# szhan227/text2protein

Hardware: AMD Instinct MI355X
Metric: 6D backbone samples/sec (128-res, 1000-step) (higher is better)
Workload: dtype f16; 1 GPU; cfg2: test_config.yml L=128 N=1000 chains/GPU=32 C=5 text_tokens=512 condition=none; step = 1 PC step (2 score evals + SDE updates); sample = 1000 PC steps; finite=True

## Files before the change

include/t2p.h:

```cpp
#ifndef T2P_H_
#define T2P_H_

#include <stdint.h>

#ifdef __cplusplus
extern "C" {
#endif

#define T2P_DTYPE_F32 0
#define T2P_DTYPE_BF16 1
#define T2P_DTYPE_F16 2

#define T2P_SDE_VE 0
#define T2P_SDE_VP 1
#define T2P_SDE_SUBVP 2

typedef struct t2p_model_config {
  int32_t num_channels;
  int32_t max_res_num;
  int32_t nf;
  int32_t num_res_blocks;
  int32_t n_ch_mult;
  int32_t ch_mult[8];
  int32_t n_attn_resolutions;
// ... 6 lines not shown
  int32_t scale_by_sigma;
  int32_t compute_dtype;
} t2p_model_config;

typedef struct t2p_engine t2p_engine;
typedef struct t2p_sampler t2p_sampler;

const char* t2p_last_error(void);
int t2p_device_count(void);

int t2p_engine_create(const t2p_model_config* cfg, t2p_engine** out);
void t2p_engine_destroy(t2p_engine* e);
int t2p_engine_num_params(const t2p_engine* e);
int t2p_engine_param_info(const t2p_engine* e, int i, const char** name, int64_t shape[4], int* ndim);
int t2p_engine_load_param(t2p_engine* e, const char* name, const float* host_data, const int64_t* shape, int ndim);
int t2p_engine_finalize(t2p_engine* e);
int t2p_engine_set_context(t2p_engine* e, const float* context, int batch, int tokens, void* stream);
int t2p_engine_score(t2p_engine* e, const float* x, const int32_t* labels, float* out, int batch, void* stream);
int t2p_engine_score_ex(t2p_engine* e, const float* x, const int32_t* labels, const float* labels_f, float* out,
                        int batch, void* stream);
int64_t t2p_engine_device_bytes(const t2p_engine* e);
int t2p_engine_pool_reclaimed(const t2p_engine* e);

typedef struct t2p_sampler_config {
  int32_t sde;
  int32_t N;
  double sigma_min, sigma_max, beta_min, beta_max;
  double snr;
  int32_t n_steps_each;
  int32_t probability_flow;
  int32_t denoise;
  double eps;
  int32_t batch;
  int32_t global_batch;
  uint64_t seed;
} t2p_sampler_config;

int t2p_sampler_create(t2p_engine* e, const t2p_sampler_config* cfg, const float* g_table, const int32_t* label_table,
                       t2p_sampler** out);
void t2p_sampler_destroy(t2p_sampler* s);
int t2p_sampler_set_seed(t2p_sampler* s, uint64_t seed);
int t2p_sampler_set_vp_tables(t2p_sampler* s, const float* label_f, const float* score_scale, const float* x_coef, const float* corr_alpha);
typedef int (*t2p_allreduce_fn)(float* device_sums2, void* stream, void* user);
int t2p_sampler_set_norm_allreduce(t2p_sampler* s, float* device_sums2, t2p_allreduce_fn fn, void* user);
int t2p_sampler_set_condition(t2p_sampler* s, const uint8_t* mask, const float* x_initial);
int t2p_sampler_set_guidance(t2p_sampler* s, double w, int enabled);
int t2p_sampler_set_context(t2p_sampler* s, const float* context, int batch, int tokens, void* stream);
int t2p_sampler_reset(t2p_sampler* s, int step, void* stream);
int t2p_sampler_step(t2p_sampler* s, float* x, float* x_mean, const float* noise_corrector,
                     const float* noise_predictor, void* stream);
int t2p_sampler_step_graph(t2p_sampler* s, float* x, float* x_mean, void* stream);
int t2p_sampler_run(t2p_sampler* s, float* x, float* out, int prior_given, int n_steps, void* stream);
int t2p_sampler_count_dispatches(t2p_sampler* s, float* x, float* x_mean, void* stream, int* n_out);

typedef struct t2p_ddim_config {
  int32_t timesteps;
  int32_t sampling_steps;
  double eta;
  double w;
  int32_t clip;
  int32_t batch;
  uint64_t seed;
} t2p_ddim_config;
typedef struct t2p_ddim_step_row {
  int32_t t;
  float sqrt_recip, sqrt_recipm1, sqrt_an, c, sigma;
  int32_t last;
} t2p_ddim_step_row;
typedef struct t2p_ddim t2p_ddim;
int t2p_ddim_create(t2p_engine* e, const t2p_ddim_config* cfg, const t2p_ddim_step_row* table, t2p_ddim** out);
void t2p_ddim_destroy(t2p_ddim* d);
int t2p_ddim_set_seed(t2p_ddim* d, uint64_t seed);
int t2p_ddim_set_condition(t2p_ddim* d, const uint8_t* mask, const float* x_initial);
int t2p_ddim_set_context(t2p_ddim* d, const float* context, int batch, int tokens, void* stream);
int t2p_ddim_reset(t2p_ddim* d, int step, void* stream);
int t2p_ddim_step(t2p_ddim* d, float* x, float* x0_out, const float* noise, void* stream);
int t2p_ddim_run(t2p_ddim* d, float* x, float* out, int prior_given, int n_steps, void* stream);
int t2p_op_ddim_update(const float* x, const float* eps_c, const float* eps_u, const float* z, const uint8_t* mask,
                       const float* x_initial, float* x_out, float* x_out2, float* x0_out, int64_t n, float w, float w1,
                       float sqrt_recip, float sqrt_recipm1, float sqrt_an, float c, float sigma, int clip, int last,
                       uint64_t seed, uint64_t stream_id, void* stream);

typedef struct t2p_train_config {
  double lr, beta1, eps, weight_decay;
  double warmup;
  double grad_clip;
  double ema_rate;
  double dropout;
  double t_eps;
  int32_t cond_flags;
  uint64_t seed;
} t2p_train_config;

typedef struct t2p_train_batch {
  const float* coords_6d;
  const uint8_t* mask_pair;
  const uint8_t* mask_inpaint;
  const float* context;
  int32_t batch, tokens;
  const float* t;
  const float* z;
} t2p_train_batch;

typedef struct t2p_trainer t2p_trainer;
int t2p_train_create(const t2p_model_config* model, const t2p_train_config* train, t2p_trainer** out);
void t2p_train_destroy(t2p_trainer* t);
int t2p_train_num_params(const t2p_trainer* t);
int t2p_train_param_info(const t2p_trainer* t, int i, const char** name, int64_t shape[4], int* ndim);
int t2p_train_load_param(t2p_trainer* t, const char* name, const float* host_data, const int64_t* shape, int ndim);
int t2p_train_read(t2p_trainer* t, int which, const char* name, float* host_out);
int t2p_train_write(t2p_trainer* t, int which, const char* name, const float* host_in);
int t2p_train_set_step(t2p_trainer* t, int64_t step, int64_t adam_updates, int64_t ema_updates);
int t2p_train_get_step(const t2p_trainer* t, int64_t out3[3]);
int t2p_train_set_sde(t2p_trainer* t, int sde, double beta_min, double beta_max, const float* std_table);
int t2p_train_set_dropout_masks(t2p_trainer* t, const uint8_t* const* device_masks, int n);
int t2p_train_set_ss_blocks(t2p_trainer* t, const int32_t* host_blocks, int n, const uint8_t* host_drop, double p);
int t2p_train_set_inpaint_draw(t2p_trainer* t, const int32_t* host_len_lo_hi, int B, double random_p, double contiguous_p);
int t2p_train_loss(t2p_trainer* t, const t2p_train_batch* batch, int backward, float* loss_host, float* score_out, void* stream);
int t2p_train_step(t2p_trainer* t, const t2p_train_batch* batch, float* loss_host, void* stream);
int t2p_train_grad_buffer(t2p_trainer* t, float** device_ptr, int64_t* n);
int t2p_train_apply(t2p_trainer* t, void* stream);
int t2p_train_eval_loss(t2p_trainer* t, const t2p_train_batch* batch, float* loss_host, void* stream);
int64_t t2p_train_device_bytes(const t2p_trainer* t);
int t2p_op_tgemm(const float* A, int64_t sAm, int64_t sAk, const float* B, int64_t sBk, int64_t sBn, float* C, int64_t ldc, int M, int N,
                 int K, int nz, int64_t sAz, int64_t sBz, int64_t sCz, float alpha, float beta, const float* bias_n, int ksplit, int conv,
                 int H, int W, int conv_C, void* stream);
int t2p_op_tgemm16(int dtype, const float* A, int64_t sAm, int64_t sAk, const float* B, int64_t sBk, int64_t sBn, float* C, int64_t ldc,
                   int M, int N, int K, int nz, int64_t sAz, int64_t sBz, int64_t sCz, float alpha, float beta, const float* bias_n, int ksplit,
                   int conv, int H, int W, int conv_C, void* stream);
int t2p_op_ss_block_dropout(const float* x, float* out, int batch, int C, int L, const int32_t* host_blocks, int n,
                            const uint8_t* host_drop, double p, uint64_t seed, uint64_t stream_id, uint8_t* drop_out_device, void* stream);
int t2p_op_inpaint_mask_draw(const int32_t* host_len_lo_hi, int B, int L, double random_p, double contiguous_p, uint64_t seed, uint64_t stream_id,
                             int force_mode, uint8_t* flags_out, uint8_t* pair_out, int* mode_out_host, void* stream);
int t2p_op_groupnorm_backward(const float* x, const float* dy, const float* gamma, const float* beta, int silu, int batch, int HW, int C,
                              int groups, float eps, float* dx, float* dgamma, float* dbeta, void* stream);
int t2p_op_layernorm_backward(const float* x, const float* dy, const float* gamma, int64_t rows, int C, float eps, float* dx, float* dgamma,
                              float* dbeta, void* stream);
int t2p_op_groupnorm_backward_form(const float* x, const float* dy, const float* gamma, const float* beta, int silu, int batch, int HW,
                                   int C, int groups, float eps, float* dx, float* dgamma, float* dbeta, int fixed_order, void* stream);
int t2p_op_layernorm_backward_form(const float* x, const float* dy, const float* gamma, int64_t rows, int C, float eps, float* dx,
                                   float* dgamma, float* dbeta, int fixed_order, void* stream);
int t2p_op_colsum(const float* dy, int nz, int64_t rows_per_z, int N, int64_t ld, float* out, int64_t ld_out, int accumulate,
                  int fixed_order, void* stream);
int t2p_op_sumsq(const float* g, int64_t n, int fixed_order, double* result_host, void* stream);
int t2p_op_seed_scale(const float* x, int64_t n, float target, float* s2_host, void* stream);
int t2p_op_softmax_backward(const float* P, float* dP_inout, int64_t rows, int n, float scale, void* stream);
int t2p_op_geglu_backward(const float* u, const float* dy, float* du, int64_t rows, int inner, void* stream);

int t2p_op_gemm(int dtype, const void* A, int a_f32, const void* Bw, void* C, int c_f32, int M, int N, int K,
                int64_t lda, int64_t ldb, int64_t ldc, const float* bias_n, const float* residual, float alpha,
                void* stream);
int t2p_op_gemm_r16(int dtype, const void* A, int a_f32, const void* Bw, void* C, int c_f32, int M, int N, int K, int64_t lda,
                    int64_t ldb, int64_t ldc, const float* bias_n, const void* residual16, float alpha, void* stream);
int t2p_op_conv3x3(int dtype, const void* x, int a_f32, const void* w, const float* bias, float* out, int batch,
                   int H, int W, int Cin, int Cout, int upsample, void* stream);
int t2p_op_conv3x3_shortcut(int dtype, const void* a, const void* w, const float* bias, const void* x0, int CX0,
                            const void* x1, int CX1, float alpha, void* out, int c_f32, int batch, int H, int W, int C,
                            int Cout, void* stream);
int t2p_op_conv3x3_groupnorm(int dtype, const void* a, const void* w, const float* bias, const float* bias_bn, const void* residual,
                             float alpha, int upsample, int groups, const float* gamma, const float* beta, float eps, int silu,
                             void* out, int out_f32, void* normed, float* col_stats, int batch, int H, int W, int C, int Cout, void* stream);
int t2p_op_small_conv_groupnorm(int dtype, const void* a, const void* w, int64_t ldw, const void* x0, int CX0, const void* x1, int CX1,
                                const float* bias, const float* bias_bn, const void* residual, float alpha, void* out, int out_f32,
                                float* col_stats, void* normed, int groups, const float* gamma, const float* beta, float eps, int silu,
                                int batch, int H, int W, int C, int Cout, void* stream);
int t2p_op_st_entry(int dtype, const void* x, const float* col_stats, int groups, const float* gn_gamma, const float* gn_beta,
                    float gn_eps, const void* w_in, const float* b_in, const void* residual, const float* ln_gamma,
                    const float* ln_beta, float ln_eps, const void* w_2, int n2, const float* b_2, int geglu, void* t, void* out2,
                    const void* w_3, const float* b_3, const void* res3, void* y, float* y_stats, int batch, int n, int C,
                    void* stream);
int t2p_op_attn_proj(int dtype, const void* x, const float* col_stats, int groups, const float* gn_gamma, const float* gn_beta,
                     float gn_eps, const void* w_qk, const float* b_qk, const void* w_v, void* qk, void* vt, void* k_fm,
                     int64_t npad, int batch, int n, int C, void* stream);
int t2p_op_input_conv(const float* x, const float* w_tcn, const float* bias, void* out, int out_dtype, int batch, int C,
                      int H, int W, int nf, float* col_stats, void* stream);
int t2p_op_groupnorm(const float* x0, const float* x1, int C0, int C1, int batch, int H, int W, int groups,
                     const float* gamma, const float* beta, float eps, int silu, int down, void* out, int dtype,
                     void* stream);
int t2p_op_layernorm(const float* x, const float* gamma, const float* beta, void* out, int dtype, int64_t rows,
                     int C, float eps, void* stream);
int t2p_op_layernorm16(const void* x16, const float* gamma, const float* beta, void* out16, int dtype, int64_t rows, int C,
                       float eps, void* stream);
int t2p_op_softmax(const float* S, int64_t lds, void* P, int64_t ldp, int dtype, int64_t rows, int n, float scale,
                   void* stream);
int t2p_op_geglu(const float* u, void* out, int dtype, int64_t rows, int inner, void* stream);
int64_t t2p_op_attention_ws(int dtype, int batch, int heads, int nq, int nk);
int t2p_op_attention(int dtype, const void* q, int64_t ldq, const void* k, int64_t ldk, const void* vt,
                     int64_t ldvt, void* out, int batch, int heads, int nq, int nk, int d, float scale,
                     void* workspace, void* stream);
int t2p_op_attention_wide(int dtype, const void* q, int64_t ldq, const void* k, int64_t ldk, const void* vt, int64_t ldvt, void* out,
                          int out_f32, const float* bias, const void* residual, int residual_16bit, float alpha, float* col_stats,
                          int batch, int n, int d, float scale, void* stream);
int t2p_op_attention_wide_fm(int dtype, const void* q, int64_t ldq, const void* k_fm, const void* vt_fm, void* out, int out_f32,
                             const float* bias, const void* residual, int residual_16bit, float alpha, float* col_stats, int batch,
                             int n, int d, float scale, void* stream);
int t2p_op_gemm_frag_major(int dtype, const void* A, const void* Bw, void* C, void* c_frag, int M, int N, int K, int frag_col0,
                           int rows_per_batch, int batch, void* stream);
int t2p_op_attention_qkv(int dtype, const void* qkv, int64_t ld, void* out, int batch, int heads, int n, int d,
                         float scale, void* stream);
int t2p_op_langevin(const float* x, const float* grad, const float* noise, const uint8_t* mask,
                    const float* x_initial, float* x_out, float* x_mean_out, int batch, int64_t per_sample,
                    float snr, float alpha, float* sums_out , void* stream);
int t2p_op_langevin_norms(const float* grad, const float* noise, int batch, int64_t per_sample, float* workspace,
                          float* sums, void* stream);
int t2p_op_langevin_update(const float* x, const float* grad, const float* noise, const uint8_t* mask,
                           const float* x_initial, float* x_out, float* x_mean_out, int64_t n, const float* sums,
                           float batch_total, float snr, float alpha, void* stream);
int t2p_op_predictor(const float* x, const float* score, const float* noise, const uint8_t* mask,
                     const float* x_initial, float* x_out, float* x_mean_out, int64_t n, float G,
                     int probability_flow, void* stream);
int t2p_op_guided_langevin_norms(const float* o_c, const float* o_u, const float* noise, int batch, int64_t per_sample, float w, float w1,
                                 float scale, float* workspace, float* sums, void* stream);
int t2p_op_guided_langevin_update(const float* x, const float* o_c, const float* o_u, const float* noise, const uint8_t* mask,
                                  const float* x_initial, float* x_out, float* x_out2, float* x_mean_out, int64_t n, float w, float w1,
                                  float scale, const float* sums, float batch_total, float snr, float alpha, void* stream);
int t2p_op_guided_predictor(const float* x, const float* o_c, const float* o_u, const float* noise, const uint8_t* mask,
                            const float* x_initial, float* x_out, float* x_out2, float* x_mean_out, int64_t n, float w, float w1,
                            float scale, float G, float x_coef, int probability_flow, void* stream);
int t2p_op_philox_normal(float* out, int64_t n, uint64_t seed, uint64_t stream_id, void* stream);
int t2p_op_convert(const float* in, void* out, int dtype, int64_t n, void* stream);
int t2p_op_decode_6d(const float* x, int batch, int channels, int L, float* clipped, float* absval, int32_t* lengths, void* stream);
int t2p_op_encode_6d(const float* xyz, const int32_t* nres, const uint8_t* atom_ok, int batch, int channels, int L,
                     const int32_t* host_blocks, int n_blocks, float* coords_6d, uint8_t* mask_pair, void* stream);
int t2p_op_embedding_gather(const void* table, int table_dtype, const int32_t* ids, float* out, int64_t n_tokens, int dim, int vocab,
                            int32_t* bad_flag, void* stream);
int t2p_op_apply_mask(float* x, const uint8_t* mask, const float* x_initial, int64_t n, void* stream);

int t2p_profile_begin(void);
int t2p_debug_set(int key, int value);
int t2p_built_with_ablation(void);
int t2p_profile_end(double* out9);
int t2p_profile_dominant(double* out4, char* name, int name_len);
int t2p_profile_attention(double* out3);
int t2p_profile_shapes(char* buf, int len);
int t2p_debug_tap(int block_index, float* dst, int64_t capacity, int64_t* shape4);
int t2p_profile_layers_begin(void);
int t2p_profile_layers_end(char* buf, int len);

#ifdef __cplusplus
}
#endif
#endif
```

text2protein_amd/_lib.py:

```python
from __future__ import annotations

import ctypes as C

from . import build as _build

DT_F32, DT_BF16, DT_F16 = 0, 1, 2
DTYPE_NAMES = {"f32": DT_F32, "fp32": DT_F32, "float32": DT_F32, "bf16": DT_BF16, "bfloat16": DT_BF16,
               "f16": DT_F16, "fp16": DT_F16, "float16": DT_F16}
SDE_VE, SDE_VP, SDE_SUBVP = 0, 1, 2


class T2PError(RuntimeError):
    pass


class ModelConfig(C.Structure):
    _fields_ = [("num_channels", C.c_int32), ("max_res_num", C.c_int32), ("nf", C.c_int32),
                ("num_res_blocks", C.c_int32), ("n_ch_mult", C.c_int32), ("ch_mult", C.c_int32 * 8),
                ("n_attn_resolutions", C.c_int32), ("attn_resolutions", C.c_int32 * 8),
                ("n_heads", C.c_int32), ("context_dim", C.c_int32), ("num_scales", C.c_int32),
                ("sigma_min", C.c_double), ("sigma_max", C.c_double),
                ("skip_rescale", C.c_int32), ("scale_by_sigma", C.c_int32), ("compute_dtype", C.c_int32)]


class SamplerConfig(C.Structure):
    _fields_ = [("sde", C.c_int32), ("N", C.c_int32),
                ("sigma_min", C.c_double), ("sigma_max", C.c_double), ("beta_min", C.c_double), ("beta_max", C.c_double),
                ("snr", C.c_double), ("n_steps_each", C.c_int32), ("probability_flow", C.c_int32),
                ("denoise", C.c_int32), ("eps", C.c_double), ("batch", C.c_int32), ("global_batch", C.c_int32),
                ("seed", C.c_uint64)]


class DdimConfig(C.Structure):
    _fields_ = [("timesteps", C.c_int32), ("sampling_steps", C.c_int32), ("eta", C.c_double), ("w", C.c_double),
                ("clip", C.c_int32), ("batch", C.c_int32), ("seed", C.c_uint64)]


class DdimStepRow(C.Structure):
    _fields_ = [("t", C.c_int32), ("sqrt_recip", C.c_float), ("sqrt_recipm1", C.c_float), ("sqrt_an", C.c_float),
                ("c", C.c_float), ("sigma", C.c_float), ("last", C.c_int32)]


class TrainConfig(C.Structure):
    _fields_ = [("lr", C.c_double), ("beta1", C.c_double), ("eps", C.c_double), ("weight_decay", C.c_double),
                ("warmup", C.c_double), ("grad_clip", C.c_double), ("ema_rate", C.c_double), ("dropout", C.c_double),
                ("t_eps", C.c_double), ("cond_flags", C.c_int32), ("seed", C.c_uint64)]


class TrainBatch(C.Structure):
    _fields_ = [("coords_6d", C.c_void_p), ("mask_pair", C.c_void_p), ("mask_inpaint", C.c_void_p), ("context", C.c_void_p),
                ("batch", C.c_int32), ("tokens", C.c_int32), ("t", C.c_void_p), ("z", C.c_void_p)]


_vp, _i, _i64, _f, _u64 = C.c_void_p, C.c_int, C.c_int64, C.c_float, C.c_uint64

SIGNATURES = {
    "t2p_last_error": (C.c_char_p, []),
    "t2p_device_count": (_i, []),
    "t2p_engine_create": (_i, [C.POINTER(ModelConfig), C.POINTER(_vp)]),
    "t2p_engine_destroy": (None, [_vp]),
    "t2p_engine_num_params": (_i, [_vp]),
    "t2p_engine_param_info": (_i, [_vp, _i, C.POINTER(C.c_char_p), C.POINTER(_i64), C.POINTER(_i)]),
    "t2p_engine_load_param": (_i, [_vp, C.c_char_p, _vp, C.POINTER(_i64), _i]),
    "t2p_engine_finalize": (_i, [_vp]),
    "t2p_engine_set_context": (_i, [_vp, _vp, _i, _i, _vp]),
    "t2p_engine_score": (_i, [_vp, _vp, _vp, _vp, _i, _vp]),
    "t2p_engine_score_ex": (_i, [_vp, _vp, _vp, _vp, _vp, _i, _vp]),
    "t2p_engine_device_bytes": (_i64, [_vp]),
    "t2p_engine_pool_reclaimed": (_i, [_vp]),
    "t2p_sampler_create": (_i, [_vp, C.POINTER(SamplerConfig), _vp, _vp, C.POINTER(_vp)]),
    "t2p_sampler_set_seed": (_i, [_vp, _u64]),
    "t2p_sampler_set_norm_allreduce": (_i, [_vp, _vp, _vp, _vp]),
    "t2p_built_with_ablation": (_i, []),
    "t2p_sampler_destroy": (None, [_vp]),
    "t2p_sampler_set_condition": (_i, [_vp, _vp, _vp]),
    "t2p_sampler_reset": (_i, [_vp, _i, _vp]),
    "t2p_sampler_step": (_i, [_vp, _vp, _vp, _vp, _vp, _vp]),
    "t2p_sampler_step_graph": (_i, [_vp, _vp, _vp, _vp]),
    "t2p_sampler_run": (_i, [_vp, _vp, _vp, _i, _i, _vp]),
    "t2p_sampler_set_vp_tables": (_i, [_vp, _vp, _vp, _vp, _vp]),
    "t2p_sampler_count_dispatches": (_i, [_vp, _vp, _vp, _vp, C.POINTER(C.c_int)]),
    "t2p_sampler_set_guidance": (_i, [_vp, C.c_double, _i]),
    "t2p_sampler_set_context": (_i, [_vp, _vp, _i, _i, _vp]),
    "t2p_op_guided_langevin_norms": (_i, [_vp, _vp, _vp, _i, _i64, _f, _f, _f, _vp, _vp, _vp]),
    "t2p_op_guided_langevin_update": (_i, [_vp, _vp, _vp, _vp, _vp, _vp, _vp, _vp, _vp, _i64, _f, _f, _f, _vp, _f, _f, _f, _vp]),
    "t2p_op_guided_predictor": (_i, [_vp, _vp, _vp, _vp, _vp, _vp, _vp, _vp, _vp, _i64, _f, _f, _f, _f, _f, _i, _vp]),
    "t2p_ddim_create": (_i, [_vp, C.POINTER(DdimConfig), C.POINTER(DdimStepRow), C.POINTER(_vp)]),
    "t2p_ddim_destroy": (None, [_vp]),
    "t2p_ddim_set_seed": (_i, [_vp, _u64]),
    "t2p_ddim_set_condition": (_i, [_vp, _vp, _vp]),
    "t2p_ddim_set_context": (_i, [_vp, _vp, _i, _i, _vp]),
    "t2p_ddim_reset": (_i, [_vp, _i, _vp]),
    "t2p_ddim_step": (_i, [_vp, _vp, _vp, _vp, _vp]),
    "t2p_ddim_run": (_i, [_vp, _vp, _vp, _i, _i, _vp]),
    "t2p_op_ddim_update": (_i, [_vp, _vp, _vp, _vp, _vp, _vp, _vp, _vp, _vp, _i64, _f, _f, _f, _f, _f, _f, _f, _i, _i, _u64, _u64, _vp]),
    "t2p_op_gemm": (_i, [_i, _vp, _i, _vp, _vp, _i, _i, _i, _i, _i64, _i64, _i64, _vp, _vp, _f, _vp]),
    "t2p_op_conv3x3_shortcut": (_i, [_i, _vp, _vp, _vp, _vp, _i, _vp, _i, _f, _vp, _i, _i, _i, _i, _i, _i, _vp]),
    "t2p_op_conv3x3_groupnorm": (_i, [_i, _vp, _vp, _vp, _vp, _vp, C.c_float, _i, _i, _vp, _vp, C.c_float, _i, _vp, _i, _vp, _vp,
                                      _i, _i, _i, _i, _i, _vp]),
    "t2p_op_attention_wide": (_i, [_i, _vp, _i64, _vp, _i64, _vp, _i64, _vp, _i, _vp, _vp, _i, _f, _vp, _i, _i, _i, _f, _vp]),
    "t2p_op_attention_wide_fm": (_i, [_i, _vp, _i64, _vp, _vp, _vp, _i, _vp, _vp, _i, _f, _vp, _i, _i, _i, _f, _vp]),
    "t2p_op_gemm_frag_major": (_i, [_i, _vp, _vp, _vp, _vp, _i, _i, _i, _i, _i, _i, _vp]),
    "t2p_op_small_conv_groupnorm": (_i, [_i, _vp, _vp, _i64, _vp, _i, _vp, _i, _vp, _vp, _vp, _f, _vp, _i, _vp, _vp, _i, _vp, _vp, _f, _i,
                                         _i, _i, _i, _i, _i, _vp]),
    "t2p_op_attn_proj": (_i, [_i, _vp, _vp, _i, _vp, _vp, _f, _vp, _vp, _vp, _vp, _vp, _vp, _i64, _i, _i, _i, _vp]),
    "t2p_op_st_entry": (_i, [_i, _vp, _vp, _i, _vp, _vp, _f, _vp, _vp, _vp, _vp, _vp, _f, _vp, _i, _vp, _i, _vp, _vp, _vp, _vp, _vp, _vp, _vp,
                             _i, _i, _i, _vp]),
    "t2p_op_input_conv": (_i, [_vp, _vp, _vp, _vp, _i, _i, _i, _i, _i, _i, _vp, _vp]),
    "t2p_op_gemm_r16": (_i, [_i, _vp, _i, _vp, _vp, _i, _i, _i, _i, _i64, _i64, _i64, _vp, _vp, _f, _vp]),
    "t2p_op_conv3x3": (_i, [_i, _vp, _i, _vp, _vp, _vp, _i, _i, _i, _i, _i, _i, _vp]),
    "t2p_op_groupnorm": (_i, [_vp, _vp, _i, _i, _i, _i, _i, _i, _vp, _vp, _f, _i, _i, _vp, _i, _vp]),
    "t2p_op_layernorm": (_i, [_vp, _vp, _vp, _vp, _i, _i64, _i, _f, _vp]),
    "t2p_op_layernorm16": (_i, [_vp, _vp, _vp, _vp, _i, _i64, _i, _f, _vp]),
    "t2p_op_softmax": (_i, [_vp, _i64, _vp, _i64, _i, _i64, _i, _f, _vp]),
    "t2p_op_geglu": (_i, [_vp, _vp, _i, _i64, _i, _vp]),
    "t2p_op_attention_ws": (_i64, [_i, _i, _i, _i, _i]),
    "t2p_op_attention_qkv": (_i, [_i, _vp, _i64, _vp, _i, _i, _i, _i, _f, _vp]),
    "t2p_op_attention": (_i, [_i, _vp, _i64, _vp, _i64, _vp, _i64, _vp, _i, _i, _i, _i, _i, _f, _vp, _vp]),
    "t2p_op_langevin": (_i, [_vp, _vp, _vp, _vp, _vp, _vp, _vp, _i, _i64, _f, _f, _vp, _vp]),
    "t2p_op_langevin_norms": (_i, [_vp, _vp, _i, _i64, _vp, _vp, _vp]),
    "t2p_op_langevin_update": (_i, [_vp, _vp, _vp, _vp, _vp, _vp, _vp, _i64, _vp, _f, _f, _f, _vp]),
    "t2p_op_apply_mask": (_i, [_vp, _vp, _vp, _i64, _vp]),
    "t2p_op_predictor": (_i, [_vp, _vp, _vp, _vp, _vp, _vp, _vp, _i64, _f, _i, _vp]),
    "t2p_op_philox_normal": (_i, [_vp, _i64, _u64, _u64, _vp]),
    "t2p_profile_begin": (_i, []),
    "t2p_debug_set": (_i, [_i, _i]),
    "t2p_op_decode_6d": (_i, [_vp, _i, _i, _i, _vp, _vp, _vp, _vp]),
    "t2p_op_encode_6d": (_i, [_vp, _vp, _vp, _i, _i, _i, _vp, _i, _vp, _vp, _vp]),
    "t2p_op_embedding_gather": (_i, [_vp, _i, _vp, _vp, _i64, _i, _i, _vp, _vp]),
    "t2p_profile_end": (_i, [C.POINTER(C.c_double)]),
    "t2p_profile_dominant": (_i, [C.POINTER(C.c_double), C.c_char_p, C.c_int]),
    "t2p_profile_attention": (_i, [C.POINTER(C.c_double)]),
    "t2p_profile_shapes": (_i, [C.c_char_p, C.c_int]),
    "t2p_debug_tap": (_i, [_i, _vp, C.c_int64, C.POINTER(C.c_int64)]),
    "t2p_profile_layers_begin": (_i, []),
    "t2p_profile_layers_end": (_i, [C.c_char_p, C.c_int]),
    "t2p_op_convert": (_i, [_vp, _vp, _i, _i64, _vp]),
    "t2p_train_create": (_i, [C.POINTER(ModelConfig), C.POINTER(TrainConfig), C.POINTER(_vp)]),
    "t2p_train_destroy": (None, [_vp]),
    "t2p_train_num_params": (_i, [_vp]),
    "t2p_train_param_info": (_i, [_vp, _i, C.POINTER(C.c_char_p), C.POINTER(_i64), C.POINTER(_i)]),
    "t2p_train_load_param": (_i, [_vp, C.c_char_p, _vp, C.POINTER(_i64), _i]),
    "t2p_train_read": (_i, [_vp, _i, C.c_char_p, _vp]),
    "t2p_train_write": (_i, [_vp, _i, C.c_char_p, _vp]),
    "t2p_train_set_step": (_i, [_vp, _i64, _i64, _i64]),
    "t2p_train_get_step": (_i, [_vp, C.POINTER(_i64)]),
    "t2p_train_set_sde": (_i, [_vp, _i, C.c_double, C.c_double, _vp]),
    "t2p_train_set_dropout_masks": (_i, [_vp, C.POINTER(_vp), _i]),
    "t2p_train_set_ss_blocks": (_i, [_vp, _vp, _i, _vp, C.c_double]),
    "t2p_train_set_inpaint_draw": (_i, [_vp, _vp, _i, C.c_double, C.c_double]),
    "t2p_train_loss": (_i, [_vp, C.POINTER(TrainBatch), _i, C.POINTER(_f), _vp, _vp]),
    "t2p_train_step": (_i, [_vp, C.POINTER(TrainBatch), C.POINTER(_f), _vp]),
    "t2p_train_eval_loss": (_i, [_vp, C.POINTER(TrainBatch), C.POINTER(_f), _vp]),
    "t2p_train_apply": (_i, [_vp, _vp]),
    "t2p_train_grad_buffer": (_i, [_vp, C.POINTER(_vp), C.POINTER(_i64)]),
    "t2p_train_device_bytes": (_i64, [_vp]),
    "t2p_op_tgemm": (_i, [_vp, _i64, _i64, _vp, _i64, _i64, _vp, _i64, _i, _i, _i, _i, _i64, _i64, _i64, _f, _f, _vp, _i, _i, _i, _i, _i, _vp]),
    "t2p_op_tgemm16": (_i, [_i, _vp, _i64, _i64, _vp, _i64, _i64, _vp, _i64, _i, _i, _i, _i, _i64, _i64, _i64, _f, _f, _vp, _i, _i, _i, _i, _i,
                            _vp]),
    "t2p_op_ss_block_dropout": (_i, [_vp, _vp, _i, _i, _i, _vp, _i, _vp, C.c_double, _u64, _u64, _vp, _vp]),
    "t2p_op_inpaint_mask_draw": (_i, [_vp, _i, _i, C.c_double, C.c_double, _u64, _u64, _i, _vp, _vp, C.POINTER(_i), _vp]),
    "t2p_op_groupnorm_backward": (_i, [_vp, _vp, _vp, _vp, _i, _i, _i, _i, _i, _f, _vp, _vp, _vp, _vp]),
    "t2p_op_layernorm_backward": (_i, [_vp, _vp, _vp, _i64, _i, _f, _vp, _vp, _vp, _vp]),
    "t2p_op_groupnorm_backward_form": (_i, [_vp, _vp, _vp, _vp, _i, _i, _i, _i, _i, _f, _vp, _vp, _vp, _i, _vp]),
    "t2p_op_layernorm_backward_form": (_i, [_vp, _vp, _vp, _i64, _i, _f, _vp, _vp, _vp, _i, _vp]),
    "t2p_op_colsum": (_i, [_vp, _i, _i64, _i, _i64, _vp, _i64, _i, _i, _vp]),
    "t2p_op_sumsq": (_i, [_vp, _i64, _i, C.POINTER(C.c_double), _vp]),
    "t2p_op_seed_scale": (_i, [_vp, _i64, _f, C.POINTER(_f), _vp]),
    "t2p_op_softmax_backward": (_i, [_vp, _vp, _i64, _i, _f, _vp]),
    "t2p_op_geglu_backward": (_i, [_vp, _vp, _vp, _i64, _i, _vp]),
}

_lib = None


def lib_path() -> str:
    return _build.LIB


ALLREDUCE_FN = C.CFUNCTYPE(C.c_int, C.c_void_p, C.c_void_p, C.c_void_p)


def load_path(path):
    global _lib
    if _lib is not None:
        raise T2PError("load_path() must come before any other use of the library")
    lib = C.CDLL(path)
    for name, (res, args) in SIGNATURES.items():
        fn = getattr(lib, name, None)
        if fn is None:
            continue
        fn.restype = res
        fn.argtypes = args
    _lib = lib
    return lib


def load_ablation():
    global _lib
    if _lib is not None:
        raise T2PError("load_ablation() must come before any other use of the library")
    lib = C.CDLL(_build.build(verbose=False, ablation=True))
    for name, (res, args) in SIGNATURES.items():
        fn = getattr(lib, name)
        fn.restype = res
        fn.argtypes = args
    assert lib.t2p_built_with_ablation() == 1
    _lib = lib
    return lib


def load(build_if_missing: bool = True):
    global _lib
    if _lib is not None:
        return _lib
    path = lib_path()
    if _build.needs_build():
        if not build_if_missing:
            raise T2PError(f"{path} is missing or stale (built from other sources): run `python -m text2protein_amd.build`")
        try:
            _build.build(verbose=False)
        except Exception as e:
            raise T2PError(f"libt2p_hip.so is missing or stale and could not be rebuilt: {e}") from e
    lib = C.CDLL(path)
    for name, (res, args) in SIGNATURES.items():
        fn = getattr(lib, name)
        fn.restype = res
        fn.argtypes = args
    _lib = lib
    return lib


def set_plan_switches(spec: str):
    lib = load()
    for kv in filter(None, (spec or "").split(",")):
        k, v = kv.split("=")
        if lib.t2p_debug_set(int(k), int(v)) != 0:
            msg = lib.t2p_last_error()
            raise T2PError(f"bad plan switch {kv}: {msg.decode() if msg else '?'}")


def check(rc: int):
    if rc != 0:
        msg = load().t2p_last_error()
        raise T2PError(f"libt2p_hip call failed (status {rc}): {msg.decode() if msg else '?'}")


def ptr(t):
    return None if t is None else C.c_void_p(t.data_ptr())


def stream_ptr():
    import torch
    return C.c_void_p(torch.cuda.current_stream().cuda_stream)
```

text2protein_amd/build.py:

```python
from __future__ import annotations

import hashlib
import os
import re
import subprocess
import sys

CSRC = os.path.join(os.path.dirname(os.path.abspath(__file__)), "csrc")
LIB = os.path.join(CSRC, "libt2p_hip.so")
LIB_ABLATION = os.path.join(CSRC, "libt2p_hip_ablation.so")
SOURCES = ["gemm.hip", "kernels.hip", "attention.hip", "smallconv.hip", "stfuse.hip", "ddim.hip", "engine.cpp", "sampler.cpp", "capi.cpp",
           "train_kernels.hip", "train.cpp", "train_capi.cpp"]
GEMM_PARTS = 7
HEADERS = ["t2p_common.h", "t2p_kernels.h", "philox.h", "engine.h", "sampler.h", "ddim.h", "train_kernels.h", "train.h", os.path.join("..", "..", "include", "t2p.h")]
ARCH = "gfx950"


def _hipcc():
    for c in (os.environ.get("HIPCC"), "/opt/rocm/bin/hipcc", "hipcc"):
        if c and (os.path.isabs(c) and os.path.exists(c) or not os.path.isabs(c)):
            return c
    raise RuntimeError("hipcc not found")


STAMP = LIB + ".srchash"
FLAGS = ["-O3", "-std=c++17", "-fPIC", f"--offload-arch={ARCH}", "-Wall", "-Wno-unused-function"]
_COMPILER_ID = None


def compiler_id() -> str:
    global _COMPILER_ID
    if _COMPILER_ID is None:
        try:
            _COMPILER_ID = subprocess.run([_hipcc(), "--version"], capture_output=True, text=True, timeout=60).stdout.strip()
        except (OSError, RuntimeError, subprocess.SubprocessError):
            _COMPILER_ID = ""
    return _COMPILER_ID


def source_hash(ablation: bool = False) -> str:
    h = hashlib.sha256()
    h.update(" ".join(FLAGS + (["-DT2P_ABLATION"] if ablation else [])).encode())
    h.update(compiler_id().encode())
    for f in SOURCES + HEADERS:
        h.update(f.encode())
        with open(os.path.join(CSRC, f), "rb") as fh:
            h.update(fh.read())
    return h.hexdigest()


def unit_hash(src: str, flags) -> str:
    h = hashlib.sha256()
    h.update(" ".join(flags).encode())
    h.update(compiler_id().encode())
    seen, todo = [], [os.path.join(CSRC, src)]
    while todo:
        f = os.path.normpath(todo.pop())
        if f in seen or not os.path.exists(f):
            continue
        seen.append(f)
        with open(f, "rb") as fh:
            data = fh.read()
        h.update(os.path.relpath(f, CSRC).encode())
        h.update(data)
        for inc in re.findall(rb'^\s*#\s*include\s+"([^"]+)"', data, re.M):
            todo.append(os.path.join(os.path.dirname(f), inc.decode()))
    return h.hexdigest()


def _read(path) -> str:
    try:
        with open(path) as f:
            return f.read().strip()
    except OSError:
        return ""


def built_hash() -> str:
    return _read(STAMP)


def needs_build() -> bool:
    return not os.path.exists(LIB) or built_hash() != source_hash()


def scratch_users(remarks: str, kernel_prefix: str = "_kernel"):
    bad, name = [], None
    for line in remarks.splitlines():
        m = re.search(r"Function Name: (\S+)", line)
        if m:
            name = m.group(1)
        m = re.search(r"ScratchSize \[bytes/lane\]: (\d+)", line)
        if m and name and kernel_prefix in name and int(m.group(1)) > 0:
            bad.append((name, int(m.group(1))))
    return bad


def build(force: bool = False, verbose: bool = True, ablation: bool = False) -> str:
    lib, stamp = (LIB_ABLATION, LIB_ABLATION + ".srchash") if ablation else (LIB, STAMP)
    if not force and os.path.exists(lib) and _read(stamp) == source_hash(ablation):
        return lib
    import fcntl
    with open(lib + ".lock", "w") as lock:
        fcntl.flock(lock, fcntl.LOCK_EX)
        try:
            if not force and os.path.exists(lib) and _read(stamp) == source_hash(ablation):
                return lib
            return _build_locked(lib, stamp, verbose, ablation)
        finally:
            fcntl.flock(lock, fcntl.LOCK_UN)


def _build_locked(lib: str, stamp: str, verbose: bool, ablation: bool) -> str:
    hipcc = _hipcc()
    objs = []
    procs = []
    pending = {}
    flags = FLAGS + (["-DT2P_ABLATION"] if ablation else [])
    if os.path.exists(stamp):
        os.remove(stamp)
    units = [(src, None) for src in SOURCES if src != "gemm.hip"] + [("gemm.hip", k) for k in range(GEMM_PARTS)]
    for src, part in sorted(units, key=lambda u: u[1] is None):
        stem = os.path.splitext(src)[0] + ("" if part is None else f"_part{part}") + ("_abl" if ablation else "")
        obj = os.path.join(CSRC, stem + ".o")
        objs.append(obj)
        cmd = [hipcc, *flags, "-x", "hip", "-c", os.path.join(CSRC, src), "-o", obj]
        if part is not None:
            cmd[1:1] = ["-Rpass-analysis=kernel-resource-usage", f"-DT2P_GEMM_PART={part}"]
        uh = unit_hash(src, cmd[1:-4])
        if os.path.exists(obj) and _read(obj + ".hash") == uh:
            continue
        if os.path.exists(obj + ".hash"):
            os.remove(obj + ".hash")
        pending[obj] = uh
        if verbose:
            print(" ".join(cmd), flush=True)
        procs.append((src, obj, subprocess.Popen(cmd, stdout=subprocess.PIPE, stderr=subprocess.STDOUT, text=True)))
    for src, obj, p in procs:
        out, _ = p.communicate()
        if p.returncode != 0:
            raise RuntimeError(f"hipcc failed on {src}:\n{out}")
        if src == "gemm.hip":
            bad = scratch_users(out)
            if bad:
                raise RuntimeError("LDS-DMA GEMM kernels spill to scratch memory (accumulator loop left rolled?): "
                                   + ", ".join(f"{n} {b} B/lane" for n, b in bad[:4]))
            keep, skip = [], 0
            for l in out.splitlines():
                if "remark:" in l:
                    skip = 2
                elif skip and re.match(r"^\s*(\d+\s*)?\|", l):
                    skip -= 1
                else:
                    skip = 0
                    keep.append(l)
            out = "\n".join(keep)
        with open(obj + ".hash", "w") as f:
            f.write(pending[obj] + "\n")
        if verbose and out.strip():
            print(out)
    cmd = [hipcc, "-shared", "-fPIC", f"--offload-arch={ARCH}", "-o", lib, *objs]
    if verbose:
        print(" ".join(cmd), flush=True)
    subprocess.run(cmd, check=True)
    r = subprocess.run([sys.executable, "-c", f"import ctypes; ctypes.CDLL({lib!r})"], capture_output=True, text=True)
    if r.returncode != 0:
        raise RuntimeError(f"{lib} does not load:\n{r.stderr[-2000:]}")
    with open(stamp, "w") as f:
        f.write(source_hash(ablation) + "\n")
    return lib


if __name__ == "__main__":
    build(force="--force" in sys.argv, ablation="--ablation" in sys.argv)
    print(LIB)
```

text2protein_amd/csrc/capi.cpp:

```cpp
#include <new>

#include "ddim.h"
#include "engine.h"
#include "sampler.h"
#include "train.h"

using namespace t2p;

#define API_BEGIN try {
#define API_END                                        \
  }                                                    \
  catch (const std::bad_alloc&) {                      \
    set_last_error("out of host memory");              \
    return T2P_ERR_STATE;                              \
  }                                                    \
  catch (const std::exception& ex) {                   \
    set_last_error(std::string("exception: ") + ex.what()); \
    return T2P_ERR_STATE;                              \
  }

namespace t2p { extern bool g_pre_conv_mfma, g_gn_apply_cols; void layer_profile_begin(); int layer_profile_end(std::string* out);
void debug_tap_set(int index, float* dst, long capacity); void debug_tap_shape(long out[4]); }
extern "C" {

// ... 132 lines not shown
  return s->impl.set_guidance(w, enabled);
  API_END
}

int t2p_sampler_set_context(t2p_sampler* s, const float* context, int batch, int tokens, void* stream) {
  API_BEGIN
  T2P_REQUIRE(s, "null sampler");
  return s->impl.set_context(context, batch, tokens, (hipStream_t)stream);
  API_END
}

int t2p_sampler_reset(t2p_sampler* s, int step, void* stream) {
  API_BEGIN
  T2P_REQUIRE(s, "null sampler");
  return s->impl.reset(step, (hipStream_t)stream);
  API_END
}

int t2p_sampler_step(t2p_sampler* s, float* x, float* x_mean, const float* noise_corrector, const float* noise_predictor,
                     void* stream) {
  API_BEGIN
  T2P_REQUIRE(s, "null sampler");
  return s->impl.step(x, x_mean, noise_corrector, noise_predictor, (hipStream_t)stream);
  API_END
}

int t2p_sampler_step_graph(t2p_sampler* s, float* x, float* x_mean, void* stream) {
  API_BEGIN
  T2P_REQUIRE(s, "null sampler");
  return s->impl.step_graph(x, x_mean, (hipStream_t)stream);
  API_END
}

int t2p_sampler_count_dispatches(t2p_sampler* s, float* x, float* x_mean, void* stream, int* n_out) {
  API_BEGIN
  T2P_REQUIRE(s, "null sampler");
  return s->impl.count_dispatches(x, x_mean, (hipStream_t)stream, n_out);
  API_END
}

int t2p_sampler_run(t2p_sampler* s, float* x, float* out, int prior_given, int n_steps, void* stream) {
  API_BEGIN
  T2P_REQUIRE(s, "null sampler");
  return s->impl.run(x, out, prior_given, n_steps, (hipStream_t)stream);
  API_END
}

int t2p_ddim_create(t2p_engine* e, const t2p_ddim_config* cfg, const t2p_ddim_step_row* table, t2p_ddim** out) {
  API_BEGIN
  T2P_REQUIRE(e && cfg && out, "null argument");
  t2p_ddim* d = new t2p_ddim(&e->impl, *cfg);
  int rc = d->impl.init(table);
  if (rc != T2P_OK) {
    delete d;
    return rc;
  }
  *out = d;
  return T2P_OK;
  API_END
}

void t2p_ddim_destroy(t2p_ddim* d) { delete d; }

int t2p_ddim_set_seed(t2p_ddim* d, uint64_t seed) {
  API_BEGIN
  T2P_REQUIRE(d, "null ddim sampler");
  d->impl.set_seed(seed);
  return T2P_OK;
  API_END
}

int t2p_ddim_set_condition(t2p_ddim* d, const uint8_t* mask, const float* x_initial) {
  API_BEGIN
  T2P_REQUIRE(d, "null ddim sampler");
  T2P_REQUIRE((mask == nullptr) == (x_initial == nullptr), "mask and x_initial go together");
  return d->impl.set_condition(mask, x_initial);
  API_END
}

int t2p_ddim_set_context(t2p_ddim* d, const float* context, int batch, int tokens, void* stream) {
  API_BEGIN
  T2P_REQUIRE(d, "null ddim sampler");
  return d->impl.set_context(context, batch, tokens, (hipStream_t)stream);
  API_END
}

int t2p_ddim_reset(t2p_ddim* d, int step, void* stream) {
  API_BEGIN
  T2P_REQUIRE(d, "null ddim sampler");
  (void)stream;
  return d->impl.reset(step);
  API_END
}

int t2p_ddim_step(t2p_ddim* d, float* x, float* x0_out, const float* noise, void* stream) {
  API_BEGIN
  T2P_REQUIRE(d, "null ddim sampler");
  return d->impl.step(x, x0_out, noise, (hipStream_t)stream);
  API_END
}

int t2p_ddim_run(t2p_ddim* d, float* x, float* out, int prior_given, int n_steps, void* stream) {
  API_BEGIN
  T2P_REQUIRE(d, "null ddim sampler");
  return d->impl.run(x, out, prior_given, n_steps, (hipStream_t)stream);
  API_END
}

int t2p_op_ddim_update(const float* x, const float* eps_c, const float* eps_u, const float* z, const uint8_t* mask,
                       const float* x_initial, float* x_out, float* x_out2, float* x0_out, int64_t n, float w, float w1,
                       float sqrt_recip, float sqrt_recipm1, float sqrt_an, float c, float sigma, int clip, int last,
                       uint64_t seed, uint64_t stream_id, void* stream) {
  API_BEGIN
  DdimUpdateArgs a;
  a.x = x; a.eps_c = eps_c; a.eps_u = eps_u; a.z = z; a.mask = mask; a.x_initial = x_initial;
  a.x_out = x_out; a.x_out2 = x_out2; a.x0_out = x0_out; a.n = n; a.w = w; a.w1 = w1;
  a.sqrt_recip = sqrt_recip; a.sqrt_recipm1 = sqrt_recipm1; a.sqrt_an = sqrt_an; a.c = c; a.sigma = sigma;
  a.clip = clip; a.last = last; a.seed = seed; a.stream_id = stream_id;
  return launch_ddim_update(a, (hipStream_t)stream);
  API_END
}

int t2p_op_gemm(int dtype, const void* A, int a_f32, const void* Bw, void* C, int c_f32, int M, int N, int K, int64_t lda,
                int64_t ldb, int64_t ldc, const float* bias_n, const float* residual, float alpha, void* stream) {
  API_BEGIN
  GemmParams p;
  p.dtype = dtype; p.A0 = A; p.a_f32 = a_f32; p.C0 = K; p.lda0 = lda; p.Bw = Bw; p.ldb = ldb; p.M = M; p.N = N;
  p.bias_n = bias_n; p.R = residual; p.ldr = ldc; p.alpha = alpha; p.C = C; p.c_f32 = c_f32; p.ldc = ldc;
  return launch_gemm(p, (hipStream_t)stream);
  API_END
}

static void* g_op_ws = nullptr;
static size_t g_op_ws_bytes = 0, g_op_ws_alloc = 0;
static int attach_op_ws(GemmParams& p) {
  if (!g_op_ws_bytes) return T2P_OK;
  if (g_op_ws_alloc < g_op_ws_bytes) {
    if (g_op_ws) { T2P_HIP_CHECK(hipDeviceSynchronize()); T2P_HIP_CHECK(hipFree(g_op_ws)); g_op_ws = nullptr; g_op_ws_alloc = 0; }
    T2P_HIP_CHECK(hipMalloc(&g_op_ws, g_op_ws_bytes));
    g_op_ws_alloc = g_op_ws_bytes;
  }
  p.ws = g_op_ws; p.ws_bytes = g_op_ws_bytes;
  return T2P_OK;
}

int t2p_op_gemm_r16(int dtype, const void* A, int a_f32, const void* Bw, void* C, int c_f32, int M, int N, int K, int64_t lda,
                    int64_t ldb, int64_t ldc, const float* bias_n, const void* residual16, float alpha, void* stream) {
  API_BEGIN
  GemmParams p;
  p.dtype = dtype; p.A0 = A; p.a_f32 = a_f32; p.C0 = K; p.lda0 = lda; p.Bw = Bw; p.ldb = ldb; p.M = M; p.N = N;
  p.bias_n = bias_n; p.R = (const float*)residual16; p.r_lowp = 1; p.ldr = ldc; p.alpha = alpha; p.C = C; p.c_f32 = c_f32; p.ldc = ldc;
  T2P_TRY(attach_op_ws(p));
  return launch_gemm(p, (hipStream_t)stream);
  API_END
}

int t2p_op_conv3x3(int dtype, const void* x, int a_f32, const void* w, const float* bias, float* out, int batch, int H,
                   int W, int Cin, int Cout, int upsample, void* stream) {
  API_BEGIN
  GemmParams p;
  p.dtype = dtype; p.A0 = x; p.a_f32 = a_f32; p.C0 = Cin; p.lda0 = Cin; p.taps = 9; p.H = H; p.W = W; p.a_up = upsample;
  p.Bw = w; p.ldb = 9L * Cin; p.M = batch * H * W; p.N = Cout; p.bias_n = bias; p.rows_per_batch = H * W;
  p.C = out; p.c_f32 = 1; p.ldc = Cout;
  T2P_TRY(attach_op_ws(p));
  return launch_gemm(p, (hipStream_t)stream);
  API_END
}

int t2p_op_conv3x3_shortcut(int dtype, const void* a, const void* w, const float* bias, const void* x0, int CX0, const void* x1,
                            int CX1, float alpha, void* out, int c_f32, int batch, int H, int W, int C, int Cout, void* stream) {
  API_BEGIN
  GemmParams p;
  p.dtype = dtype; p.A0 = a; p.a_f32 = 0; p.C0 = C; p.lda0 = C; p.taps = 9; p.H = H; p.W = W;
  p.Bw = w; p.ldb = 9L * C + CX0 + CX1; p.M = batch * H * W; p.N = Cout; p.bias_n = bias; p.rows_per_batch = H * W;
  p.alpha = alpha; p.C = out; p.c_f32 = c_f32; p.ldc = Cout;
  T2P_TRY(attach_op_ws(p));
  T2P_REQUIRE(gemm_can_fuse_shortcut(p), "this convolution does not take the shortcut segment (LDS-DMA 3x3 convolutions only)");
  p.X0 = x0; p.CX0 = CX0; p.ldx0 = CX0; p.X1 = x1; p.CX1 = CX1; p.ldx1 = CX1;
  return launch_gemm(p, (hipStream_t)stream);
  API_END
}

int t2p_op_conv3x3_groupnorm(int dtype, const void* a, const void* w, const float* bias, const float* bias_bn, const void* residual,
                             float alpha, int upsample, int groups, const float* gamma, const float* beta, float eps, int silu,
                             void* out, int out_f32, void* normed, float* col_stats, int batch, int H, int W, int C, int Cout, void* stream) {
  API_BEGIN
  GemmParams p;
  p.dtype = dtype; p.A0 = a; p.a_f32 = 0; p.C0 = C; p.lda0 = C; p.taps = 9; p.H = H; p.W = W; p.a_up = upsample;
  p.Bw = w; p.ldb = 9L * C; p.M = batch * H * W; p.N = Cout; p.bias_n = bias; p.rows_per_batch = H * W;
  p.bias_bn = bias_bn; p.ld_bn = Cout;
  p.R = (const float*)residual; p.r_lowp = residual ? 1 : 0; p.ldr = Cout;
  p.alpha = alpha; p.C = out; p.c_f32 = out_f32; p.ldc = Cout; p.col_stats = col_stats;
  T2P_TRY(attach_op_ws(p));
  T2P_REQUIRE(gemm_fuses_post_gn(p, groups), "this convolution does not take the split-K plan whose second pass applies a GroupNorm");
  p.gn_gamma = gamma; p.gn_beta = beta; p.gn_groups = groups; p.gn_silu = silu; p.gn_eps = eps; p.gn_out = normed;
  return launch_gemm(p, (hipStream_t)stream);
  API_END
}

int t2p_op_small_conv_groupnorm(int dtype, const void* a, const void* w, int64_t ldw, const void* x0, int CX0, const void* x1, int CX1,
                                const float* bias, const float* bias_bn, const void* residual, float alpha, void* out, int out_f32,
                                float* col_stats, void* normed, int groups, const float* gamma, const float* beta, float eps, int silu,
                                int batch, int H, int W, int C, int Cout, void* stream) {
  API_BEGIN
  SmallConvArgs s;
  s.dtype = dtype; s.A = a; s.B = batch; s.H = H; s.W = W; s.C = C; s.N = Cout; s.Wt = w; s.ldw = ldw;
  s.X0 = x0; s.CX0 = CX0; s.X1 = x1; s.CX1 = CX1; s.bias = bias; s.bias_bn = bias_bn; s.ld_bn = Cout; s.R = residual; s.alpha = alpha;
  s.out = out; s.out_f32 = out_f32; s.col_stats = col_stats; s.normed = normed; s.gn_gamma = gamma; s.gn_beta = beta; s.groups = groups;
  s.gn_silu = silu; s.gn_eps = eps;
  return launch_small_conv_gn(s, (hipStream_t)stream);
  API_END
}

int t2p_op_st_entry(int dtype, const void* x, const float* col_stats, int groups, const float* gn_gamma, const float* gn_beta, float gn_eps,
                    const void* w_in, const float* b_in, const void* residual, const float* ln_gamma, const float* ln_beta, float ln_eps,
                    const void* w_qkv, int n2, const float* b2, int geglu, void* t, void* qkv, const void* w3, const float* b3,
                    const void* res3, void* y, float* y_stats, int batch, int n, int C, void* stream) {
  API_BEGIN
  StEntryArgs e;
  e.dtype = dtype; e.B = batch; e.n = n; e.C = C; e.x = x; e.cstats = col_stats; e.groups = groups; e.gn_gamma = gn_gamma;
  e.gn_beta = gn_beta; e.gn_eps = gn_eps; e.w_in = w_in; e.b_in = b_in; e.ln_gamma = ln_gamma; e.ln_beta = ln_beta; e.ln_eps = ln_eps;
  e.w_qkv = w_qkv; e.n2 = n2; e.b2 = b2; e.geglu = geglu; e.res = residual; e.t = t; e.qkv = qkv;
  e.w3 = w3; e.b3 = b3; e.res3 = res3; e.y = y; e.y_stats = y_stats;
  T2P_REQUIRE(st_entry_eligible(e), "st_entry: C = 256 (or 512 without geglu), n2 in {C, 3 C} (8 C with geglu), 16-bit dtype, n % 32 == 0 (64 with column sums), batch n <= 8192");
  void* fm = nullptr;
  T2P_HIP_CHECK(hipMalloc(&fm, ((size_t)C * C + (size_t)n2 * C + (w3 ? (size_t)5 * C * C : 0)) * 2));
  void* fm2 = (char*)fm + (size_t)C * C * 2;
  void* fm3 = (char*)fm2 + (size_t)n2 * C * 2;
  int rc = launch_sf_frag_major(dtype, w_in, fm, C, C, (hipStream_t)stream);
  if (rc == T2P_OK) rc = launch_sf_frag_major(dtype, w_qkv, fm2, n2, C, (hipStream_t)stream);
  if (rc == T2P_OK && w3) rc = launch_sf_frag_major(dtype, w3, fm3, C, 5 * C, (hipStream_t)stream);
  if (rc == T2P_OK && w3 && y_stats && hipMemsetAsync(y_stats, 0, (size_t)batch * n / 64 * C * 2 * 4, (hipStream_t)stream) != hipSuccess) rc = T2P_ERR_HIP;
  e.w_in = fm; e.w_qkv = fm2;
  if (w3) e.w3 = fm3;
  if (rc == T2P_OK) rc = launch_st_entry(e, (hipStream_t)stream);
  (void)hipStreamSynchronize((hipStream_t)stream);
  (void)hipFree(fm);
  return rc;
  API_END
}

int t2p_op_attn_proj(int dtype, const void* x, const float* col_stats, int groups, const float* gn_gamma, const float* gn_beta, float gn_eps,
                     const void* w_qk, const float* b_qk, const void* w_v, void* qk, void* vt, void* k_fm, int64_t npad, int batch, int n, int C,
                     void* stream) {
  API_BEGIN
  AttnProjArgs e;
  e.dtype = dtype; e.B = batch; e.n = n; e.C = C; e.npad = npad; e.x = x; e.cstats = col_stats; e.groups = groups; e.gn_gamma = gn_gamma;
  e.gn_beta = gn_beta; e.gn_eps = gn_eps; e.b_qk = b_qk; e.qk = qk; e.vt = vt; e.k_fm = k_fm;
  T2P_REQUIRE(attn_proj_eligible(e), "attn_proj: C = 256, 16-bit dtype, n % 32 == 0 (64 with column sums), batch n <= 8192, npad % 4 == 0");
  void* fm = nullptr;
  T2P_HIP_CHECK(hipMalloc(&fm, (size_t)3 * C * C * 2));
  void* fm2 = (char*)fm + (size_t)2 * C * C * 2;
  int rc = launch_sf_frag_major(dtype, w_qk, fm, 2 * C, C, (hipStream_t)stream);
  if (rc == T2P_OK) rc = launch_sf_frag_major(dtype, w_v, fm2, C, C, (hipStream_t)stream);
  e.w_qk = fm; e.w_v = fm2;
  if (rc == T2P_OK) rc = launch_attn_proj(e, (hipStream_t)stream);
  (void)hipStreamSynchronize((hipStream_t)stream);
  (void)hipFree(fm);
  return rc;
  API_END
}

int t2p_op_input_conv(const float* x, const float* w_tcn, const float* bias, void* out, int out_dtype, int batch, int C, int H, int W,
                      int nf, float* col_stats, void* stream) {
  API_BEGIN
  if (pre_conv_split_ok(out_dtype, C, H, W, nf) && (!col_stats || pre_conv_fuses_col_stats(W, nf))) {
    void* ws = nullptr;
    T2P_HIP_CHECK(hipMalloc(&ws, pre_conv_split_weight_bytes(C, nf)));
    int rc = launch_pre_conv_split_weights(w_tcn, ws, C, nf, (hipStream_t)stream);
    if (rc == T2P_OK) rc = launch_pre_conv_split(x, ws, bias, out, out_dtype, batch, C, H, W, nf, (hipStream_t)stream, col_stats);
    (void)hipStreamSynchronize((hipStream_t)stream);
    (void)hipFree(ws);
    return rc;
  }
  return launch_pre_conv(x, w_tcn, bias, out, out_dtype, batch, C, H, W, nf, (hipStream_t)stream, col_stats);
  API_END
}

int t2p_op_groupnorm(const float* x0, const float* x1, int C0, int C1, int batch, int H, int W, int groups,
                     const float* gamma, const float* beta, float eps, int silu, int down, void* out, int dtype,
                     void* stream) {
  API_BEGIN
  hipStream_t s = (hipStream_t)stream;
  GroupNormArgs a;
  a.x0 = x0; a.x1 = x1; a.C0 = C0; a.C1 = C1; a.B = batch; a.HW = H * W; a.G = groups; a.eps = eps;
  const int C = C0 + C1;
  {
    GroupNormApplyArgs g;
    g.x0 = x0; g.x1 = x1; g.C0 = C0; g.C1 = C1; g.B = batch; g.H = H; g.W = W; g.G = groups; g.gamma = gamma; g.beta = beta;
    g.silu = silu; g.down = down; g.out = out; g.dtype = dtype; g.eps = eps;
    if (g_gn_small && gn_small_eligible(g)) return launch_gn_small(g, s);
  }
  const int nparts = gn_num_chunks(a.HW) * ((C + 1023) / 1024);
  float* ws = nullptr;
  T2P_HIP_CHECK(hipMalloc((void**)&ws, ((size_t)batch * nparts * groups * 2 + (size_t)batch * groups * 2) * 4));
  a.partial = ws;
  a.stats = ws + (size_t)batch * nparts * groups * 2;
  int rc = launch_gn_stats(a, s);
  if (rc == T2P_OK) {
    GroupNormApplyArgs g;
    g.x0 = x0; g.x1 = x1; g.C0 = C0; g.C1 = C1; g.B = batch; g.H = H; g.W = W; g.G = groups; g.stats = a.stats;
    g.gamma = gamma; g.beta = beta; g.silu = silu; g.down = down; g.out = out; g.dtype = dtype;
    rc = launch_gn_apply(g, s);
  }
  (void)hipStreamSynchronize(s);
  (void)hipFree(ws);
// ... 149 lines not shown
                           float batch_total, float snr, float alpha, void* stream) {
  API_BEGIN
  SdeUpdateArgs a;
  a.x = x; a.score = grad; a.noise = noise; a.mask = mask; a.x_initial = x_initial; a.x_out = x_out;
  a.x_mean_out = x_mean_out; a.n = n;
  return launch_langevin_update(a, sums, batch_total, snr, alpha, (hipStream_t)stream);
  API_END
}

int t2p_op_predictor(const float* x, const float* score, const float* noise, const uint8_t* mask, const float* x_initial,
                     float* x_out, float* x_mean_out, int64_t n, float G, int probability_flow, void* stream) {
  API_BEGIN
  SdeUpdateArgs a;
  a.x = x; a.score = score; a.noise = noise; a.mask = mask; a.x_initial = x_initial; a.x_out = x_out;
  a.x_mean_out = x_mean_out; a.n = n;
  return launch_predictor_update(a, nullptr, nullptr, G, probability_flow, (hipStream_t)stream);
  API_END
}

int t2p_op_guided_langevin_norms(const float* o_c, const float* o_u, const float* noise, int batch, int64_t per_sample, float w, float w1,
                                 float scale, float* workspace, float* sums, void* stream) {
  API_BEGIN
  GuidedScore g;
  g.o_c = o_c; g.o_u = o_u; g.w = w; g.w1 = w1; g.scale = scale;
  return launch_guided_langevin_norms(g, noise, batch, per_sample, workspace, sums, (hipStream_t)stream);
  API_END
}

int t2p_op_guided_langevin_update(const float* x, const float* o_c, const float* o_u, const float* noise, const uint8_t* mask,
                                  const float* x_initial, float* x_out, float* x_out2, float* x_mean_out, int64_t n, float w, float w1,
                                  float scale, const float* sums, float batch_total, float snr, float alpha, void* stream) {
  API_BEGIN
  SdeUpdateArgs a;
  a.x = x; a.noise = noise; a.mask = mask; a.x_initial = x_initial; a.x_out = x_out; a.x_mean_out = x_mean_out; a.n = n;
  GuidedScore g;
  g.o_c = o_c; g.o_u = o_u; g.w = w; g.w1 = w1; g.scale = scale;
  return launch_guided_langevin_update(a, g, x_out2, sums, batch_total, snr, alpha, (hipStream_t)stream);
  API_END
}

int t2p_op_guided_predictor(const float* x, const float* o_c, const float* o_u, const float* noise, const uint8_t* mask,
                            const float* x_initial, float* x_out, float* x_out2, float* x_mean_out, int64_t n, float w, float w1,
                            float scale, float G, float x_coef, int probability_flow, void* stream) {
  API_BEGIN
  SdeUpdateArgs a;
  a.x = x; a.noise = noise; a.mask = mask; a.x_initial = x_initial; a.x_out = x_out; a.x_mean_out = x_mean_out; a.n = n;
  GuidedScore g;
  g.o_c = o_c; g.o_u = o_u; g.w = w; g.w1 = w1; g.scale = scale;
  return launch_guided_predictor_update(a, g, x_out2, nullptr, G, probability_flow, (hipStream_t)stream, nullptr, x_coef);
  API_END
}

int t2p_op_philox_normal(float* out, int64_t n, uint64_t seed, uint64_t stream_id, void* stream) {
  API_BEGIN
  return launch_philox_normal(out, n, seed, stream_id, nullptr, (hipStream_t)stream);
  API_END
}

int t2p_op_convert(const float* in, void* out, int dtype, int64_t n, void* stream) {
  API_BEGIN
  return launch_convert(in, out, dtype, n, (hipStream_t)stream);
  API_END
}

int t2p_op_decode_6d(const float* x, int batch, int channels, int L, float* clipped, float* absval, int32_t* lengths, void* stream) {
  API_BEGIN
  return launch_decode6d(x, batch, channels, L, clipped, absval, lengths, (hipStream_t)stream);
  API_END
}

int t2p_op_encode_6d(const float* xyz, const int32_t* nres, const uint8_t* atom_ok, int batch, int channels, int L,
                     const int32_t* host_blocks, int n_blocks, float* coords_6d, uint8_t* mask_pair, void* stream) {
  API_BEGIN
  T2P_REQUIRE(xyz && nres && coords_6d && mask_pair && batch > 0 && L > 0, "encode_6d arguments");
  T2P_REQUIRE(channels == 5 || channels == 8, "encode_6d: the channel count must be 5 or 8, not " + std::to_string(channels));
  T2P_REQUIRE(n_blocks >= 0 && (n_blocks == 0 || host_blocks), "encode_6d: block list arguments");
  T2P_REQUIRE(n_blocks == 0 || channels == 8, "encode_6d: secondary-structure blocks need the 8-channel layout");
  T2P_REQUIRE((long)L * L < (1L << 30) && batch <= 65535, "encode_6d: map or batch too large");
  hipStream_t s = (hipStream_t)stream;
  std::vector<int32_t> n((size_t)batch);
  T2P_HIP_CHECK(hipMemcpyAsync(n.data(), nres, (size_t)batch * 4, hipMemcpyDeviceToHost, s));
  T2P_HIP_CHECK(hipStreamSynchronize(s));
  for (int b = 0; b < batch; ++b)
    T2P_REQUIRE(n[b] >= 1 && n[b] <= L, "encode_6d: nres[" + std::to_string(b) + "] = " + std::to_string(n[b]) + " is outside [1, " + std::to_string(L) + "]");
  std::vector<std::vector<int32_t>> of_sample((size_t)batch);
  for (int k = 0; k < n_blocks; ++k) {
    const int32_t* q = host_blocks + 4 * (size_t)k;
    const std::string name = "encode_6d: block " + std::to_string(k);
    T2P_REQUIRE(q[0] >= 0 && q[0] < batch, name + " names a sample outside the batch");
    T2P_REQUIRE(q[1] <= q[2], name + " starts after its last residue");
    T2P_REQUIRE(q[1] >= 0 && q[2] < n[q[0]], name + " lies outside the " + std::to_string(n[q[0]]) + " residues of its sample");
    T2P_REQUIRE(q[3] == 0 || q[3] == 1, name + " is neither a helix (0) nor a strand (1)");
    of_sample[q[0]].push_back(k);
  }
  if (n_blocks == 0) return launch_encode6d(xyz, nres, atom_ok, batch, channels, L, nullptr, nullptr, 0, coords_6d, mask_pair, s);
  std::vector<int32_t> up(host_blocks, host_blocks + 4 * (size_t)n_blocks);
  for (const auto& ks : of_sample)
    for (int32_t k1 : ks)
      for (int32_t k2 : ks) { up.push_back(k1); up.push_back(k2); }
  const size_t npairs = (up.size() - 4 * (size_t)n_blocks) / 2;
  T2P_REQUIRE(npairs < (1u << 30), "encode_6d: too many block pairs");
  struct Scratch {
    int32_t* p = nullptr; hipStream_t s;
    ~Scratch() { if (p) { (void)hipStreamSynchronize(s); (void)hipFree(p); } }
  } dev;
  dev.s = s;
  T2P_HIP_CHECK(hipMalloc(&dev.p, up.size() * 4));
  T2P_HIP_CHECK(hipMemcpyAsync(dev.p, up.data(), up.size() * 4, hipMemcpyHostToDevice, s));
  return launch_encode6d(xyz, nres, atom_ok, batch, channels, L, dev.p, dev.p + 4 * (size_t)n_blocks, (int)npairs, coords_6d, mask_pair, s);
  API_END
}

int t2p_op_embedding_gather(const void* table, int table_dtype, const int32_t* ids, float* out, int64_t n_tokens, int dim, int vocab,
                            int32_t* bad_flag, void* stream) {
  API_BEGIN
  return launch_embedding_gather(table, table_dtype, ids, out, n_tokens, dim, vocab, bad_flag, (hipStream_t)stream);
  API_END
}

int t2p_op_apply_mask(float* x, const uint8_t* mask, const float* x_initial, int64_t n, void* stream) {
  API_BEGIN
  return launch_apply_mask(x, mask, x_initial, n, (hipStream_t)stream);
  API_END
}

int t2p_debug_set(int key, int value) {
  if (key == 10) { g_op_ws_bytes = (size_t)value << 20; return T2P_OK; }
  if (key == 11) { set_gemm_force_nsplit(value); return T2P_OK; }
  if (key == 12) { set_gemm_midsplit(value != 0); return T2P_OK; }
  if (key == 13) { g_gn_small = value != 0; return T2P_OK; }
  if (key == 14) { g_lowp_residual = value != 0; return T2P_OK; }
  if (key == 15) { set_gemm_thin_conv(value != 0); return T2P_OK; }
  if (key == 17) { g_gn_apply16 = value != 0; return T2P_OK; }
  if (key == 20) { g_layernorm16 = value != 0; return T2P_OK; }
  if (key == 21) { set_gemm_up4(value != 0); return T2P_OK; }
  if (key == 22) { set_gemm_deep_ring(value != 0); return T2P_OK; }
  if (key == 23) { set_gemm_fuse_shortcut(value != 0); return T2P_OK; }
  if (key == 25) { g_qkv_fused = value != 0; return T2P_OK; }
  if (key == 26) { t2p::g_pre_conv_mfma = value != 0; return T2P_OK; }
  if (key == 27) { t2p::g_gn_apply_cols = value != 0; return T2P_OK; }
  if (key == 28) { set_gemm_post_gn(value != 0); return T2P_OK; }
  if (key == 29) { t2p::g_attn_strip = value != 0; return T2P_OK; }
  if (key == 36) { t2p::g_small_conv = value != 0; return T2P_OK; }
  if (key == 38) { t2p::g_pre_conv_split = value != 0; return T2P_OK; }
  if (key == 39) { t2p::g_st_fuse = value != 0; return T2P_OK; }
  if (key == 40) { t2p::g_st_tail = value != 0; return T2P_OK; }
  if (key == 41) { t2p::g_small_conv_fm = value != 0; return T2P_OK; }
  if (key == 42) { t2p::g_st_ffpo = value != 0; return T2P_OK; }
  if (key == 43) { t2p::g_st_tail_rows = value; return T2P_OK; }
  if (key == 45) { t2p::g_attn_fm = value != 0; return T2P_OK; }
  if (key == 46) { t2p::g_attn_proj = value != 0; return T2P_OK; }
  if (key == 47) { set_gemm_dxs(value != 0); return T2P_OK; }
  if (key == 48) { t2p::g_train_plumbing16 = value != 0; return T2P_OK; }
  if (key == 34) { set_gemm_a_norm(value != 0); return T2P_OK; }
  if (key == 32) { g_attn_merged = value != 0; return T2P_OK; }
  if (key == 33) { g_ffpo_merged = value != 0; return T2P_OK; }
  if (key == 30) { set_gemm_split_consts(value, 0); return T2P_OK; }
  if (key == 31) { set_gemm_split_consts(0, value); return T2P_OK; }
  if (key == 0) set_gemm_dma(value != 0);
  else if (key == 1) {
#ifndef T2P_ABLATION
    if (value & ~(128 | 256 | 4096 | 8192)) {
      set_last_error("ablation bits that skip work exist only in a -DT2P_ABLATION build");
      return T2P_ERR_INVALID;
    }
#endif
    set_gemm_debug(value);
  }
  else if (key == 2) set_gemm_geom(value);
  else if (key == 3) set_gemm_splitk(value != 0);
  else if (key == 4) g_raw_copies = value != 0;
  else if (key == 5) g_flash_attention = value != 0;
  else if (key == 6) g_fuse_gn_stats = value != 0;
  else if (key == 7) g_fuse_geglu = value != 0;
  else if (key == 8) set_gemm_ring(value);
  else if (key == 9) g_lowp_h1 = value != 0;
  else return T2P_ERR_INVALID;
  return T2P_OK;
}

#ifdef T2P_ABLATION
extern "C" int t2p_ablation_dxs_stamps(unsigned long long* out, int n) { return t2p::dxs_stamps_read(out, n); }
#endif

int t2p_built_with_ablation(void) {
#ifdef T2P_ABLATION
  return 1;
#else
  return 0;
#endif
}

int t2p_profile_begin(void) {
  profile_begin();
  return T2P_OK;
}

int t2p_profile_end(double* out9) {
  API_BEGIN
  T2P_REQUIRE(out9, "null argument");
  double o[3][3];
  T2P_TRY(profile_end(o));
  for (int k = 0; k < 3; ++k)
    for (int j = 0; j < 3; ++j) out9[k * 3 + j] = o[k][j];
  return T2P_OK;
  API_END
}

int t2p_profile_attention(double* out3) {
  API_BEGIN
  T2P_REQUIRE(out3, "null argument");
  return profile_attention(out3);
  API_END
}

int t2p_profile_shapes(char* buf, int len) {
  API_BEGIN
  T2P_REQUIRE(buf && len > 0, "null argument");
  return profile_shapes(buf, len);
  API_END
}

int t2p_debug_tap(int block_index, float* dst, int64_t capacity, int64_t* shape4) {
  API_BEGIN
  if (shape4) {
    long sh[4];
    t2p::debug_tap_shape(sh);
    for (int i = 0; i < 4; ++i) shape4[i] = sh[i];
  }
  t2p::debug_tap_set(block_index, dst, (long)capacity);
  return T2P_OK;
  API_END
}

int t2p_profile_layers_begin(void) {
  t2p::layer_profile_begin();
  return T2P_OK;
}

int t2p_profile_layers_end(char* buf, int len) {
  API_BEGIN
  T2P_REQUIRE(buf && len > 0, "null argument");
  std::string out;
  T2P_TRY(t2p::layer_profile_end(&out));
  T2P_REQUIRE((size_t)len > out.size(), "the per-block timing table does not fit the buffer (" + std::to_string(out.size() + 1) + " bytes needed)");
  std::snprintf(buf, (size_t)len, "%s", out.c_str());
  return T2P_OK;
  API_END
}

int t2p_profile_dominant(double* out4, char* name, int name_len) {
  API_BEGIN
  T2P_REQUIRE(out4 && name && name_len > 0, "null argument");
  const char* n = nullptr;
  T2P_TRY(profile_dominant(out4, &n));
  std::snprintf(name, (size_t)name_len, "%s", n ? n : "");
  return T2P_OK;
  API_END
}

}
```

text2protein_amd/csrc/engine.cpp:

```cpp
#include "engine.h"

#include <algorithm>
#include <cmath>
#include <cstdio>
#include <cstring>
#include <map>
#include <mutex>
#include <thread>

namespace t2p {

bool g_fuse_gn_stats = true;
bool g_fuse_geglu = true;
bool g_lowp_h1 = true;
bool g_gn_small = true;
bool g_lowp_residual = true;
bool g_raw_copies = true;
bool g_flash_attention = true;
bool g_attn_merged = true;
bool g_ffpo_merged = true;
bool g_qkv_fused = true;
static thread_local std::string g_last_error;
void set_last_error(const std::string& msg) { g_last_error = msg; }
const char* get_last_error() { return g_last_error.c_str(); }
// ... 535 lines not shown
      T2P_TRY(upload_linear(p + ".NIN_3.W", p + ".NIN_3.b", ci, ci, &l.out, false, true));
      if (cfg_.compute_dtype != DT_F32) {
        const HostTensor* w2 = host(p + ".NIN_2.W", {ci, ci});
        const HostTensor* w3 = host(p + ".NIN_3.W", {ci, ci});
        const HostTensor* b2 = host(p + ".NIN_2.b", {ci});
        const HostTensor* b3 = host(p + ".NIN_3.b", {ci});
        if (!w2 || !w3 || !b2 || !b3) return T2P_ERR_STATE;
        HostTensor m;
        m.shape = {ci, ci};
        m.data = host_matmul(w2->data.data(), w3->data.data(), ci, ci, ci);
        std::vector<float> bb = host_matmul(b2->data.data(), w3->data.data(), 1, ci, ci);
        for (int i = 0; i < ci; ++i) bb[i] += b3->data[i];
        T2P_TRY(upload_matrix(pool_, to_nk(m, false, true), cfg_.compute_dtype, &l.v3.w));
        T2P_TRY(upload_f32(bb, &l.v3.b));
        l.v3.N = ci; l.v3.K = ci;
        if (ci == 256 && l.qk.w && l.qk.b) {
          l.fm_qk = pool_.persistent((size_t)2 * ci * ci * 2);
          l.fm_v3 = pool_.persistent((size_t)ci * ci * 2);
          if (!l.fm_qk || !l.fm_v3) return T2P_ERR_HIP;
          T2P_TRY(launch_sf_frag_major(cfg_.compute_dtype, l.qk.w, l.fm_qk, 2 * ci, ci, nullptr));
          T2P_TRY(launch_sf_frag_major(cfg_.compute_dtype, l.v3.w, l.fm_v3, ci, ci, nullptr));
          T2P_HIP_CHECK(hipStreamSynchronize(nullptr));
        }
      }
    } else {
      const std::string t = p + ".transformer_blocks.0";
      const int ctx = cfg_.context_dim;
      T2P_TRY(upload_norm(p + ".norm", ci, 32, &l.gn0));
      T2P_TRY(upload_linear(p + ".proj_in.weight", p + ".proj_in.bias", ci, ci, &l.proj_in));
      T2P_TRY(upload_linear(p + ".proj_out.weight", p + ".proj_out.bias", ci, ci, &l.proj_out));
      T2P_TRY(upload_stack2(t + ".attn1.to_q.weight", "", t + ".attn1.to_k.weight", "", ci, ci, false, false, &l.a1_qk));
      T2P_TRY(upload_linear(t + ".attn1.to_v.weight", "", ci, ci, &l.a1_v));
      if (cfg_.compute_dtype != DT_F32) {
        const HostTensor* wq = host(t + ".attn1.to_q.weight", {ci, ci});
        const HostTensor* wk = host(t + ".attn1.to_k.weight", {ci, ci});
        const HostTensor* wv = host(t + ".attn1.to_v.weight", {ci, ci});
        if (!wq || !wk || !wv) return T2P_ERR_STATE;
        std::vector<float> m = wq->data;
        m.insert(m.end(), wk->data.begin(), wk->data.end());
        m.insert(m.end(), wv->data.begin(), wv->data.end());
        T2P_TRY(upload_matrix(pool_, m, cfg_.compute_dtype, &l.a1_qkv.w));
        l.a1_qkv.N = 3 * ci; l.a1_qkv.K = ci; l.a1_qkv.b = nullptr;
      }
      T2P_TRY(upload_linear(t + ".attn1.to_out.0.weight", t + ".attn1.to_out.0.bias", ci, ci, &l.a1_out));
      T2P_TRY(upload_linear(t + ".attn2.to_q.weight", "", ci, ci, &l.a2_q));
      T2P_TRY(upload_linear(t + ".attn2.to_k.weight", "", ci, ctx, &l.a2_k));
      T2P_TRY(upload_linear(t + ".attn2.to_v.weight", "", ci, ctx, &l.a2_v));
      T2P_TRY(upload_linear(t + ".attn2.to_out.0.weight", t + ".attn2.to_out.0.bias", ci, ci, &l.a2_out));
      {
        const HostTensor* w = host(t + ".ff.net.0.proj.weight", {8 * ci, ci});
        const HostTensor* b = host(t + ".ff.net.0.proj.bias", {8 * ci});
        if (!w || !b) return T2P_ERR_STATE;
        const int inner = 4 * ci;
        std::vector<float> wi((size_t)8 * ci * ci), bi((size_t)8 * ci);
        for (int j = 0; j < inner; ++j) {
          std::copy(w->data.begin() + (size_t)j * ci, w->data.begin() + (size_t)(j + 1) * ci, wi.begin() + (size_t)(2 * j) * ci);
          std::copy(w->data.begin() + (size_t)(inner + j) * ci, w->data.begin() + (size_t)(inner + j + 1) * ci,
                    wi.begin() + (size_t)(2 * j + 1) * ci);
          bi[2 * j] = b->data[j];
          bi[2 * j + 1] = b->data[inner + j];
        }
        T2P_TRY(upload_matrix(pool_, wi, cfg_.compute_dtype, &l.ff1.w));
        T2P_TRY(upload_f32(bi, &l.ff1.b));
        l.ff1.N = 8 * ci;
        l.ff1.K = ci;
      }
      T2P_TRY(upload_linear(t + ".ff.net.2.weight", t + ".ff.net.2.bias", ci, 4 * ci, &l.ff2));
      if (cfg_.compute_dtype != DT_F32 && ci == 256 && l.a1_qkv.w) {
        auto fm = [&](const void* w, int N, void** out) -> int {
          *out = pool_.persistent((size_t)N * ci * 2);
          if (!*out) return T2P_ERR_HIP;
          return launch_sf_frag_major(cfg_.compute_dtype, w, *out, N, ci, nullptr);
        };
        T2P_TRY(fm(l.proj_in.w, ci, &l.fm_in));
        T2P_TRY(fm(l.a1_qkv.w, 3 * ci, &l.fm_qkv));
        T2P_TRY(fm(l.a1_out.w, ci, &l.fm_out1));
        T2P_TRY(fm(l.a2_q.w, ci, &l.fm_q2));
        if (ci == 256) {
          T2P_TRY(fm(l.a2_out.w, ci, &l.fm_out2));
          T2P_TRY(fm(l.ff1.w, 8 * ci, &l.fm_ff1));
        }
        T2P_HIP_CHECK(hipStreamSynchronize(nullptr));
      }
      if (cfg_.compute_dtype != DT_F32 && ci % 64 == 0) {
        const HostTensor* wpo = host(p + ".proj_out.weight", {ci, ci, 1, 1});
        const HostTensor* bpo = host(p + ".proj_out.bias", {ci});
        const HostTensor* wf = host(t + ".ff.net.2.weight", {ci, 4 * ci});
        const HostTensor* bf = host(t + ".ff.net.2.bias", {ci});
        if (!wpo || !bpo || !wf || !bf) return T2P_ERR_STATE;
        const std::vector<float> prod = host_matmul(wpo->data.data(), wf->data.data(), ci, ci, 4 * ci);
        std::vector<float> m((size_t)ci * 5 * ci), bb(ci);
        for (int n = 0; n < ci; ++n) {
          std::copy(prod.begin() + (size_t)n * 4 * ci, prod.begin() + (size_t)(n + 1) * 4 * ci, m.begin() + (size_t)n * 5 * ci);
          std::copy(wpo->data.begin() + (size_t)n * ci, wpo->data.begin() + (size_t)(n + 1) * ci, m.begin() + (size_t)n * 5 * ci + 4 * ci);
          double acc = bpo->data[n];
          for (int j = 0; j < ci; ++j) acc += (double)wpo->data[(size_t)n * ci + j] * bf->data[j];
          bb[n] = (float)acc;
        }
        T2P_TRY(upload_matrix(pool_, m, cfg_.compute_dtype, &l.ffpo.w));
        T2P_TRY(upload_f32(bb, &l.ffpo.b));
        l.ffpo.N = ci; l.ffpo.K = 5 * ci;
        if (ci == 256 && l.fm_in) {
          l.fm_ffpo = pool_.persistent((size_t)ci * 5 * ci * 2);
          if (!l.fm_ffpo) return T2P_ERR_HIP;
          T2P_TRY(launch_sf_frag_major(cfg_.compute_dtype, l.ffpo.w, l.fm_ffpo, ci, 5 * ci, nullptr));
          T2P_HIP_CHECK(hipStreamSynchronize(nullptr));
        }
      }
      T2P_TRY(upload_norm(t + ".norm1", ci, 1, &l.ln1));
      T2P_TRY(upload_norm(t + ".norm2", ci, 1, &l.ln2));
      T2P_TRY(upload_norm(t + ".norm3", ci, 1, &l.ln3));
    }
    return T2P_OK;
  }));
  void* dwp = nullptr;
  T2P_TRY(upload_matrix(pool_, dw, DT_F32, &dwp));
  dense_all_.w = dwp;
  dense_all_.N = arch_.temb_total;
  dense_all_.K = td;
  T2P_TRY(upload_f32(db, &dense_all_.b));
  T2P_TRY(upload_norm("out.0", arch_.final_ch, gn_groups(arch_.final_ch), &head_norm_));
  T2P_TRY(upload_linear("out.2.weight", "out.2.bias", cfg_.num_channels, 9 * arch_.final_ch, &head_conv_, true));

  const int N = cfg_.num_scales;
  std::vector<float> inv(N);
  const double a = std::log(cfg_.sigma_max), b = std::log(cfg_.sigma_min);
  for (int i = 0; i < N; ++i) {
    const double s = std::exp(a + (b - a) * (double)i / (double)(N - 1));
    inv[i] = (float)(1.0 / s);
  }
  T2P_TRY(upload_f32(inv, &inv_sigma_));
  T2P_TRY(upload_f32(std::vector<float>(N, 1.f), &unit_scale_));
  host_.clear();
  finalized_ = true;
  return T2P_OK;
}

int Engine::attach_ws(GemmParams& p) {
  if (!splitk_ws_) {
    splitk_ws_bytes_ = (size_t)256 << 20;
    splitk_ws_ = pool_.persistent(splitk_ws_bytes_);
    if (!splitk_ws_) return T2P_ERR_HIP;
  }
  p.ws = splitk_ws_;
  p.ws_bytes = splitk_ws_bytes_;
  return T2P_OK;
}

int Engine::gemm(GemmParams& p, hipStream_t s) {
  T2P_TRY(attach_ws(p));
  return launch_gemm(p, s);
}

int Engine::gemm_stats(GemmParams& p, float** cstats, hipStream_t s) {
  *cstats = nullptr;
  T2P_TRY(attach_ws(p));
  if (g_fuse_gn_stats && (gemm_fuses_col_stats(p) || gemm_fuses_col_stats_lowp(p))) {
    *cstats = (float*)pool_.get((size_t)(p.M / 64) * p.N * 2 * 4);
    if (!*cstats) return T2P_ERR_HIP;
    p.col_stats = *cstats;
  }
  return gemm(p, s);
}

int Engine::linear(const void* a, bool a_is_f32, const DevLinear& w, long rows, void* c, bool c_f32,
                   const float* residual, float alpha, hipStream_t s, bool use_bias, float** cstats, bool r_lowp) {
  GemmParams p;
  p.dtype = dtype();
  p.A0 = a; p.a_f32 = a_is_f32 || p.dtype == DT_F32; p.C0 = w.K; p.lda0 = w.K;
  p.Bw = w.w; p.ldb = w.K;
  p.M = (int)rows; p.N = w.N;
  p.bias_n = use_bias ? w.b : nullptr;
  p.R = residual; p.ldr = w.N; p.r_lowp = (residual && r_lowp) ? 1 : 0;
  p.alpha = alpha;
  p.C = c; p.c_f32 = c_f32; p.ldc = w.N;
  if (cstats) return gemm_stats(p, cstats, s);
  return gemm(p, s);
}

int Engine::group_norm(const Act& x, const Act* x1, const DevNorm& n, float eps, int silu, int down, int B, void** out,
                       hipStream_t s, void** raw_out) {
  const int C = x.C + (x1 ? x1->C : 0);
  T2P_REQUIRE(C == n.C, "GroupNorm channel mismatch");
  T2P_REQUIRE(!x1 || x1->lowp == x.lowp, "concatenated sources must share a storage type");
  T2P_REQUIRE(!x.lowp || dtype() != DT_F32, "16-bit activations exist in the 16-bit modes only");
  if (x.pre_norm && !x1 && x.pre_for == &n && x.pre_silu == silu && !down && !raw_out) {
    *out = x.pre_norm;
    x.pre_norm = nullptr;
    return T2P_OK;
  }
  {
    GroupNormApplyArgs g;
    g.x0 = (const float*)x.p; g.x1 = x1 ? (const float*)x1->p : nullptr; g.C0 = x.C; g.C1 = x1 ? x1->C : 0;
    g.B = B; g.H = x.H; g.W = x.W; g.G = n.G; g.gamma = n.gamma; g.beta = n.beta; g.silu = silu; g.down = down;
    g.dtype = dtype(); g.x0_lowp = x.lowp; g.eps = eps;
    if (g_gn_small && gn_small_eligible(g)) {
      const size_t bytes = (size_t)B * x.H * x.W * C * dtype_size(dtype());
      POOL_GET(o, void*, bytes);
      g.out = o;
      if (raw_out) {
        *raw_out = pool_.get(bytes);
        if (!*raw_out) return T2P_ERR_HIP;
        g.raw_out = *raw_out;
      }
      T2P_TRY(launch_gn_small(g, s));
      *out = o;
      return T2P_OK;
    }
  }
  GroupNormArgs a;
  a.x0 = x.p; a.x1 = x1 ? x1->p : nullptr; a.C0 = x.C; a.C1 = x1 ? x1->C : 0;
  a.B = B; a.HW = x.H * x.W; a.G = n.G; a.eps = eps;
  const bool have_cols = x.cstats && (!x1 || x1->cstats) && a.HW % 64 == 0;
  if (have_cols && !raw_out) {
    GroupNormApplyArgs g;
    g.x0 = a.x0; g.x1 = a.x1; g.C0 = a.C0; g.C1 = a.C1; g.B = B; g.H = x.H; g.W = x.W; g.G = n.G;
    g.gamma = n.gamma; g.beta = n.beta; g.silu = silu; g.down = down; g.dtype = dtype(); g.x0_lowp = x.lowp;
    g.cs0 = x.cstats; g.cs1 = x1 ? x1->cstats : nullptr; g.eps = eps;
    if (gn_apply_cols_eligible(g)) {
      POOL_GET(o, void*, (size_t)B * a.HW * C * dtype_size(dtype()));
      g.out = o;
      T2P_TRY(launch_gn_apply_cols(g, s));
      *out = o;
      return T2P_OK;
    }
  }
  const int nparts = gn_num_chunks(a.HW) * ((C + 1023) / 1024);
  POOL_GET(stats, float*, (size_t)B * n.G * 2 * 4);
  float* partial = nullptr;
  if (have_cols) {
    T2P_TRY(launch_gn_finalize_cols(x.cstats, x1 ? x1->cstats : nullptr, a.C0, a.C1, B, a.HW, n.G, eps, stats, s));
  } else {
    partial = (float*)pool_.get((size_t)B * nparts * n.G * 2 * 4);
    if (!partial) return T2P_ERR_HIP;
    a.partial = partial; a.stats = stats;
    a.lowp_dtype = x.lowp ? dtype() : DT_F32;
    T2P_TRY(launch_gn_stats(a, s));
  }
  GroupNormApplyArgs g;
  g.x0 = a.x0; g.x1 = a.x1; g.C0 = a.C0; g.C1 = a.C1; g.B = B; g.H = x.H; g.W = x.W; g.G = n.G;
  g.stats = stats; g.gamma = n.gamma; g.beta = n.beta; g.silu = silu; g.down = down; g.dtype = dtype();
  g.x0_lowp = x.lowp;
  const size_t opix = (size_t)B * (down ? x.H / 2 : x.H) * (down ? x.W / 2 : x.W);
  POOL_GET(o, void*, opix * C * dtype_size(dtype()));
  g.out = o;
  if (raw_out) {
    *raw_out = pool_.get(opix * C * dtype_size(dtype()));
    if (!*raw_out) return T2P_ERR_HIP;
    g.raw_out = *raw_out;
  }
  T2P_TRY(launch_gn_apply(g, s));
  pool_.put(partial);
  pool_.put(stats);
  *out = o;
  return T2P_OK;
}

int Engine::res_block(Layer& L, const Act& x, const Act* skip, Act* out, int B, hipStream_t s, NormHint hint) {
  const int Cin = x.C + (skip ? skip->C : 0), Cout = L.out_ch;
  T2P_REQUIRE(Cin == L.in_ch, "res block input channels");
  T2P_REQUIRE(!(L.down && skip), "down block with concat input");
  const int Ho = L.up ? x.H * 2 : (L.down ? x.H / 2 : x.H), Wo = L.up ? x.W * 2 : (L.down ? x.W / 2 : x.W);
  const long rows_out = (long)B * Ho * Wo;
  const int dt = dtype();
  void* a0 = nullptr;
  void* xraw = nullptr;
  const bool want_raw = g_raw_copies && L.has_conv2 && !L.down && dt != DT_F32 && !x.lowp;
  T2P_TRY(group_norm(x, skip, L.gn0, 1e-6f, 1, L.down, B, &a0, s, want_raw ? &xraw : nullptr));
  if (dt != DT_F32 && !L.up && (Ho * Wo == 16 || Ho * Wo == 64) && x.lowp && (!skip || skip->lowp) && (L.has_conv2 ? L.conv1x.w != nullptr : true)) {
    SmallConvArgs c0;
    c0.dtype = dt; c0.A = a0; c0.B = B; c0.H = Ho; c0.W = Wo; c0.C = Cin; c0.N = Cout; c0.Wt = L.conv0.w; c0.ldw = L.conv0.K;
    c0.bias = L.conv0.b; c0.bias_bn = tb_ + L.temb_off; c0.ld_bn = tb_ld_;
    c0.gn_gamma = L.gn1.gamma; c0.gn_beta = L.gn1.beta; c0.groups = L.gn1.G; c0.gn_silu = 1; c0.gn_eps = 1e-6f;
    SmallConvArgs c1;
    c1.dtype = dt; c1.B = B; c1.H = Ho; c1.W = Wo; c1.C = Cout; c1.N = Cout;
    c1.alpha = cfg_.skip_rescale ? 0.70710678118654752440f : 1.f;
    if (L.has_conv2) {
      c1.Wt = L.conv1x.w; c1.ldw = L.conv1x.K; c1.bias = L.conv1x.b;
      c1.CX0 = L.down ? Cin : x.C; c1.CX1 = (!L.down && skip) ? skip->C : 0;
    } else {
      c1.Wt = L.conv1.w; c1.ldw = L.conv1.K; c1.bias = L.conv1.b;
    }
    const bool olp = res_lowp();
    if (hint.norm && olp && hint.norm->C == Cout) { c1.groups = hint.norm->G; c1.gn_silu = hint.silu; }
    c0.normed = a0; c1.A = a0; c1.out = a0; c1.normed = c1.groups ? a0 : nullptr;
    c1.gn_gamma = c1.groups ? hint.norm->gamma : nullptr; c1.gn_beta = c1.groups ? hint.norm->beta : nullptr;
    if (L.has_conv2) { c1.X0 = a0; c1.X1 = c1.CX1 ? a0 : nullptr; } else { c1.R = a0; }
    if (small_conv_eligible(c0) && small_conv_eligible(c1)) {
      if (g_small_conv_fm && c0.ldw % 32 == 0 && c1.ldw % 32 == 0) {
        if (!L.fm_conv0) {
          hipStreamCaptureStatus cap = hipStreamCaptureStatusNone;
          if (s) (void)hipStreamIsCapturing(s, &cap);
          T2P_REQUIRE(cap == hipStreamCaptureStatusNone, "the first evaluation builds per-block weight copies: run one eager step before capturing");
          void* f0 = pool_.persistent((size_t)Cout * c0.ldw * 2);
          void* f1 = pool_.persistent((size_t)Cout * c1.ldw * 2);
          if (!f0 || !f1) return T2P_ERR_HIP;
          T2P_TRY(launch_sf_frag_major(dt, c0.Wt, f0, Cout, (int)c0.ldw, s));
          T2P_TRY(launch_sf_frag_major(dt, c1.Wt, f1, Cout, (int)c1.ldw, s));
          L.fm_conv0 = f0; L.fm_conv1 = f1;
        }
        c0.Wt = L.fm_conv0; c0.w_fm = 1; c1.Wt = L.fm_conv1; c1.w_fm = 1;
      }
      POOL_GET(a1s, void*, (size_t)rows_out * Cout * dtype_size(dt));
      c0.normed = a1s;
      T2P_TRY(launch_small_conv_gn(c0, s));
      pool_.put(a0);
      void* xpooled = nullptr;
      if (L.has_conv2) {
        if (L.down) {
          xpooled = pool_.get((size_t)rows_out * Cin * dtype_size(dt));
          if (!xpooled) return T2P_ERR_HIP;
          T2P_TRY(launch_pool2x2(x.p, xpooled, dt, B, x.H, x.W, Cin, s, x.lowp));
          c1.X0 = xpooled;
        } else {
          c1.X0 = x.p;
          c1.X1 = skip ? skip->p : nullptr;
        }
      } else {
        c1.R = x.p;
      }
      POOL_GET(o, float*, (size_t)rows_out * Cout * (olp ? dtype_size(dt) : 4));
      float* o_stats = nullptr;
      void* pre = nullptr;
      if (c1.groups) {
        pre = pool_.get((size_t)rows_out * Cout * dtype_size(dt));
        if (!pre) return T2P_ERR_HIP;
      }
      if (Ho * Wo == 64 && g_fuse_gn_stats) {
        o_stats = (float*)pool_.get((size_t)(rows_out / 64) * Cout * 2 * 4);
        if (!o_stats) return T2P_ERR_HIP;
// ... 27 lines not shown
      p.C = nullptr;
      T2P_TRY(gemm(p, s));
    } else {
    if (g_lowp_h1 && dt != DT_F32 && g_fuse_gn_stats && gemm_fuses_col_stats(p) && (Ho * Wo) % 64 == 0 &&
        !(g_gn_small && Ho * Wo <= 64)) {
      p.c_f32 = 0;
      h1_lowp = gemm_fuses_col_stats_lowp(p);
      if (!h1_lowp) p.c_f32 = 1;
    }
    T2P_TRY(gemm_stats(p, &h1_stats, s));
    if (h1_lowp && !h1_stats) return T2P_ERR_STATE;
    }
  }
  pool_.put(a0);
  Act h1a{h1, Cout, Ho, Wo, h1_stats, h1_lowp};
  void* a1 = a1_fused;
  if (!a1) T2P_TRY(group_norm(h1a, nullptr, L.gn1, 1e-6f, 1, 0, B, &a1, s));
  free_act(h1a);
  GemmParams pc;
  pc.dtype = dt; pc.A0 = a1; pc.a_f32 = dt == DT_F32; pc.C0 = Cout; pc.lda0 = Cout;
  pc.taps = 9; pc.H = Ho; pc.W = Wo;
  pc.Bw = L.conv1.w; pc.ldb = L.conv1.K; pc.M = (int)rows_out; pc.N = Cout;
  pc.bias_n = L.conv1.b; pc.rows_per_batch = Ho * Wo;
  pc.alpha = cfg_.skip_rescale ? 0.70710678118654752440f : 1.f;
  bool fused_shortcut = false;
  void* xpooled = nullptr;
  if (L.conv1x.w && (L.down || x.lowp || xraw) && x.C % 64 == 0 && (!skip || skip->C % 64 == 0) && gemm_can_fuse_shortcut(pc)) {
    fused_shortcut = true;
    pc.Bw = L.conv1x.w; pc.ldb = L.conv1x.K; pc.bias_n = L.conv1x.b;
    if (L.down) {
      xpooled = pool_.get((size_t)rows_out * Cin * dtype_size(dt));
      if (!xpooled) return T2P_ERR_HIP;
      T2P_TRY(launch_pool2x2(x.p, xpooled, dt, B, x.H, x.W, Cin, s, x.lowp));
      pc.X0 = xpooled; pc.CX0 = Cin; pc.ldx0 = Cin;
    } else if (xraw) {
      pc.X0 = xraw; pc.CX0 = Cin; pc.ldx0 = Cin;
    } else {
      pc.X0 = x.p; pc.CX0 = x.C; pc.ldx0 = x.C;
      if (skip) { pc.X1 = skip->p; pc.CX1 = skip->C; pc.ldx1 = skip->C; }
    }
  }
  const float* r = x.p;
  float* rbuf = nullptr;
  bool rbuf_lowp = false;
  int r_up = 0;
  if (fused_shortcut) {
    r = nullptr;
  } else if (L.has_conv2) {
    GemmParams p;
    p.dtype = dt; p.a_f32 = dt == DT_F32;
    void* pooled = nullptr;
    long rrows;
    if (L.down) {
      pooled = pool_.get((size_t)rows_out * Cin * dtype_size(dt));
      if (!pooled) return T2P_ERR_HIP;
      T2P_TRY(launch_pool2x2(x.p, pooled, dt, B, x.H, x.W, Cin, s, x.lowp));
      p.A0 = pooled; p.C0 = Cin; p.lda0 = Cin;
      rrows = rows_out;
    } else {
      if (xraw) {
        p.A0 = xraw; p.C0 = Cin; p.lda0 = Cin;
      } else {
        p.a_f32 = x.lowp ? 0 : 1;
        p.A0 = x.p; p.C0 = x.C; p.lda0 = x.C;
        if (skip) { p.A1 = skip->p; p.C1 = skip->C; p.lda1 = skip->C; }
      }
      rrows = (long)B * x.H * x.W;
      r_up = L.up;
    }
    rbuf_lowp = false;
    rbuf = (float*)pool_.get((size_t)rrows * Cout * (rbuf_lowp ? dtype_size(dt) : 4));
    if (!rbuf) return T2P_ERR_HIP;
    p.Bw = L.conv2.w; p.ldb = L.conv2.K; p.M = (int)rrows; p.N = Cout; p.bias_n = L.conv2.b;
    p.C = rbuf; p.c_f32 = rbuf_lowp ? 0 : 1; p.ldc = Cout;
    T2P_TRY(gemm(p, s));
    pool_.put(pooled);
    pool_.put(xraw);
    r = rbuf;
  } else {
    T2P_REQUIRE(!skip && Cin == Cout, "identity shortcut needs equal channels");
  }
  const bool olp = res_lowp();
  POOL_GET(o, float*, (size_t)rows_out * Cout * (olp ? dtype_size(dt) : 4));
  float* o_stats = nullptr;
  pc.R = r; pc.ldr = Cout; pc.r_up = r_up;
  pc.r_lowp = (r == x.p ? x.lowp : rbuf_lowp) ? 1 : 0;
  pc.C = o; pc.c_f32 = olp ? 0 : 1; pc.ldc = Cout;
  void* pre = nullptr;
  T2P_TRY(attach_ws(pc));
  if (hint.norm && olp && hint.norm->C == Cout && gemm_fuses_post_gn(pc, hint.norm->G)) {
    pre = pool_.get((size_t)rows_out * Cout * dtype_size(dt));
    if (!pre) return T2P_ERR_HIP;
    pc.gn_gamma = hint.norm->gamma; pc.gn_beta = hint.norm->beta; pc.gn_groups = hint.norm->G; pc.gn_silu = hint.silu; pc.gn_eps = 1e-6f;
    if ((Ho * Wo) % 64 == 0 && g_fuse_gn_stats) {
      o_stats = (float*)pool_.get((size_t)(rows_out / 64) * Cout * 2 * 4);
      if (!o_stats) return T2P_ERR_HIP;
      pc.col_stats = o_stats;
    }
    pc.gn_out = pre;
    T2P_TRY(gemm(pc, s));
  } else {
    T2P_TRY(gemm_stats(pc, &o_stats, s));
  }
  pool_.put(a1);
  pool_.put(rbuf);
  if (fused_shortcut) { pool_.put(xraw); pool_.put(xpooled); }
  *out = Act{o, Cout, Ho, Wo, o_stats, olp};
  out->pre_norm = pre; out->pre_for = hint.norm; out->pre_silu = hint.silu;
  return T2P_OK;
}

int Engine::attention(const void* q, long ldq, const void* k, long ldk, const void* vt, long ldvt, void* out, int B,
                      int heads, int nq, int nk, int d, float scale, hipStream_t s) {
  const int dt = dtype();
  if (g_flash_attention && attention_flash_eligible(dt, d, ldq, ldk, ldvt, (long)heads * d))
    return launch_attention_flash(dt, q, ldq, k, ldk, vt, ldvt, out, B, heads, nq, nk, d, scale, s);
  if (attention_strip_eligible(dt, heads, nq, nk, d, ldq, ldk, ldvt, d))
    return launch_attention_strip(dt, q, ldq, k, ldk, vt, ldvt, out, d, B, nq, d, scale, s);
  const long nkp = (long)round_up((size_t)nk, 8);
  const long rows = (long)B * heads * nq;
  POOL_GET(S, float*, (size_t)rows * nkp * 4);
  POOL_GET(P, void*, (size_t)rows * nkp * dtype_size(dt));
  GemmParams p;
  p.dtype = dt; p.a_f32 = dt == DT_F32;
  p.A0 = q; p.C0 = d; p.lda0 = ldq; p.M = nq; p.N = nk;
  p.Bw = k; p.ldb = ldk;
  p.nz0 = B; p.nz1 = heads;
  p.sA_z0 = (long)nq * ldq; p.sA_z1 = d; p.sB_z0 = (long)nk * ldk; p.sB_z1 = d;
  p.C = S; p.c_f32 = 1; p.ldc = nkp; p.sC_z0 = (long)heads * nq * nkp; p.sC_z1 = (long)nq * nkp;
  T2P_TRY(gemm(p, s));
  T2P_TRY(launch_softmax(S, nkp, P, nkp, dt, rows, nk, scale, s));
  GemmParams r;
  r.dtype = dt; r.a_f32 = dt == DT_F32;
  r.A0 = P; r.C0 = nk; r.lda0 = nkp; r.M = nq; r.N = d;
  r.Bw = vt; r.ldb = ldvt;
  r.nz0 = B; r.nz1 = heads;
  r.sA_z0 = (long)heads * nq * nkp; r.sA_z1 = (long)nq * nkp; r.sB_z0 = (long)heads * d * ldvt; r.sB_z1 = (long)d * ldvt;
  r.C = out; r.c_f32 = 0; r.ldc = (long)heads * d; r.sC_z0 = (long)nq * heads * d; r.sC_z1 = d;
  T2P_TRY(launch_gemm(r, s));
  pool_.put(S);
  pool_.put(P);
  return T2P_OK;
}

static int project_vt(int dt, const DevLinear& wv, const void* a, long lda, int B, int n, long npad, void* vt,
                      hipStream_t s) {
  GemmParams p;
  p.dtype = dt; p.a_f32 = dt == DT_F32;
  p.A0 = wv.w; p.C0 = wv.K; p.lda0 = wv.K; p.M = wv.N; p.N = n;
  p.Bw = a; p.ldb = lda;
  p.nz0 = B; p.sA_z0 = 0; p.sB_z0 = (long)n * lda;
  p.bias_m = wv.b;
  p.C = vt; p.c_f32 = 0; p.ldc = npad; p.sC_z0 = (long)wv.N * npad;
  return launch_gemm(p, s);
}

int Engine::attn_block(Layer& L, const Act& x, Act* out, int B, hipStream_t s) {
  const int C = x.C, n = x.H * x.W, dt = dtype();
  const size_t es = dtype_size(dt);
  const long rows = (long)B * n, npad = (long)round_up((size_t)n, 8);
  const bool olp = res_lowp();
  const bool merged = g_attn_merged && L.v3.w && attention_strip_eligible(dt, 1, n, n, C, 2 * C, 2 * C, npad, C) && (!x.lowp || olp);
  if (merged && x.lowp && L.fm_qk && g_attn_proj) {
    AttnProjArgs e;
    e.dtype = dt; e.B = B; e.n = n; e.C = C; e.npad = npad;
    const bool normed = x.pre_norm && x.pre_for == &L.gn0 && x.pre_silu == 0;
    e.x = normed ? x.pre_norm : (const void*)x.p;
    e.cstats = normed ? nullptr : x.cstats;
    e.gn_gamma = L.gn0.gamma; e.gn_beta = L.gn0.beta; e.groups = L.gn0.G; e.gn_eps = 1e-6f;
    e.w_qk = L.fm_qk; e.b_qk = L.qk.b; e.w_v = L.fm_v3;
    if ((normed || x.cstats) && attn_proj_eligible(e)) {
      POOL_GET(qk2, char*, (size_t)rows * 2 * C * es);
      POOL_GET(vt2, void*, (size_t)B * C * npad * es);
      e.qk = qk2; e.vt = vt2;
      void* kfm2 = nullptr;
      if (g_attn_fm && npad == n && attention_strip_frag_major_ok(dt, n, C)) {
        kfm2 = pool_.get((size_t)rows * C * es);
        if (!kfm2) return T2P_ERR_HIP;
        e.k_fm = kfm2;
      }
      T2P_TRY(launch_attn_proj(e, s));
      if (normed) { pool_.put(x.pre_norm); x.pre_norm = nullptr; }
      const float att_scale2 = 1.f / std::sqrt((float)C);
      POOL_GET(y, float*, (size_t)rows * C * (olp ? es : 4));
      float* y_stats = nullptr;
      if (g_fuse_gn_stats && n % 64 == 0) {
        y_stats = (float*)pool_.get((size_t)(rows / 64) * C * 2 * 4);
        if (!y_stats) return T2P_ERR_HIP;
      }
      StripEpilogue ep;
      ep.bias = L.v3.b; ep.residual = x.p; ep.r_lowp = 1; ep.ldr = C; ep.alpha = cfg_.skip_rescale ? 0.70710678118654752440f : 1.f;
      ep.out_f32 = olp ? 0 : 1; ep.col_stats = y_stats;
      ep.frag_major = kfm2 ? 1 : 0;
      if (kfm2) T2P_TRY(launch_attention_strip(dt, qk2, 2 * C, kfm2, C, vt2, npad, y, C, B, n, C, att_scale2, s, &ep));
      else T2P_TRY(launch_attention_strip(dt, qk2, 2 * C, qk2 + (size_t)C * es, 2 * C, vt2, npad, y, C, B, n, C, att_scale2, s, &ep));
      pool_.put(kfm2);
      pool_.put(qk2);
      pool_.put(vt2);
      *out = Act{y, C, x.H, x.W, y_stats, olp};
      return T2P_OK;
    }
  }
  void* a = nullptr;
  T2P_TRY(group_norm(x, nullptr, L.gn0, 1e-6f, 0, 0, B, &a, s));
  POOL_GET(qk, char*, (size_t)rows * 2 * C * es);
  GemmParams pq;
  pq.dtype = dt; pq.A0 = a; pq.a_f32 = dt == DT_F32; pq.C0 = C; pq.lda0 = C; pq.Bw = L.qk.w; pq.ldb = C; pq.M = (int)rows; pq.N = 2 * C;
  pq.bias_n = L.qk.b; pq.C = qk; pq.c_f32 = 0; pq.ldc = 2 * C;
  T2P_TRY(attach_ws(pq));
  void* kfm = nullptr;
  GemmParams pv;
  pv.dtype = dt; pv.a_f32 = dt == DT_F32; pv.A0 = L.v3.w; pv.C0 = C; pv.lda0 = C; pv.M = C; pv.N = n; pv.Bw = a; pv.ldb = C;
  pv.nz0 = B; pv.sA_z0 = 0; pv.sB_z0 = (long)n * C; pv.c_f32 = 0; pv.ldc = npad; pv.sC_z0 = (long)C * npad;
  T2P_TRY(attach_ws(pv));
  bool fm = false;
  if (merged && g_attn_fm && npad == n && attention_strip_frag_major_ok(dt, n, C)) {
    GemmParams tq = pq, tv = pv;
    tq.rows_per_batch = n; tq.frag_col0 = C; tq.frag_ns = C / 32; tq.frag_bstride = (long)n * C; tq.c_frag = qk;
    tv.frag_col0 = 0; tv.frag_ns = n / 32; tv.frag_bstride = (long)n * C; tv.c_frag = qk; tv.C = qk;
    fm = gemm_writes_frag_major(tq) && gemm_writes_frag_major(tv);
    if (fm) {
      kfm = pool_.get((size_t)rows * C * es);
      if (!kfm) return T2P_ERR_HIP;
      tq.c_frag = kfm;
      pq = tq;
      pv = tv;
    }
  }
  T2P_TRY(launch_gemm(pq, s));
  POOL_GET(vt, void*, (size_t)B * C * npad * es);
  const float att_scale = 1.f / std::sqrt((float)C);
  const float out_alpha = cfg_.skip_rescale ? 0.70710678118654752440f : 1.f;
  if (merged) {
    if (fm) {
      pv.C = vt; pv.c_frag = vt;
      T2P_TRY(launch_gemm(pv, s));
    } else {
      DevLinear nob = L.v3;
      nob.b = nullptr;
      T2P_TRY(project_vt(dt, nob, a, C, B, n, npad, vt, s));
    }
    pool_.put(a);
    POOL_GET(y, float*, (size_t)rows * C * (olp ? es : 4));
    float* y_stats = nullptr;
    if (g_fuse_gn_stats && n % 64 == 0) {
      y_stats = (float*)pool_.get((size_t)(rows / 64) * C * 2 * 4);
      if (!y_stats) return T2P_ERR_HIP;
    }
    StripEpilogue ep;
    ep.bias = L.v3.b; ep.residual = x.p; ep.r_lowp = x.lowp ? 1 : 0; ep.ldr = C; ep.alpha = out_alpha; ep.out_f32 = olp ? 0 : 1;
    ep.col_stats = y_stats;
    ep.frag_major = fm ? 1 : 0;
    if (fm) T2P_TRY(launch_attention_strip(dt, qk, 2 * C, kfm, C, vt, npad, y, C, B, n, C, att_scale, s, &ep));
    else T2P_TRY(launch_attention_strip(dt, qk, 2 * C, qk + (size_t)C * es, 2 * C, vt, npad, y, C, B, n, C, att_scale, s, &ep));
    pool_.put(kfm);
    pool_.put(qk);
    pool_.put(vt);
    *out = Act{y, C, x.H, x.W, y_stats, olp};
    return T2P_OK;
  }
  T2P_TRY(project_vt(dt, L.v, a, C, B, n, npad, vt, s));
  pool_.put(a);
  POOL_GET(o, void*, (size_t)rows * C * es);
  T2P_TRY(attention(qk, 2 * C, qk + (size_t)C * es, 2 * C, vt, npad, o, B, 1, n, n, C, att_scale, s));
  pool_.put(qk);
  pool_.put(vt);
  POOL_GET(y, float*, (size_t)rows * C * (olp ? es : 4));
  float* y_stats = nullptr;
  T2P_TRY(linear(o, false, L.out, rows, y, !olp, x.p, out_alpha, s, true, &y_stats, x.lowp));
  pool_.put(o);
  *out = Act{y, C, x.H, x.W, y_stats, olp};
  return T2P_OK;
}

bool g_st_tail = true;
int g_st_tail_rows = 4096;
bool g_attn_proj = true;
bool g_attn_fm = true;
bool g_st_ffpo = true;
bool g_small_conv_fm = true;
int Engine::st_block(Layer& L, const Act& x, Act* out, int B, hipStream_t s) {
  const int C = x.C, n = x.H * x.W, dt = dtype(), heads = cfg_.n_heads, d = C / heads;
  const size_t es = dtype_size(dt);
  const long rows = (long)B * n, npad = (long)round_up((size_t)n, 8);
  const float scale = 1.f / std::sqrt((float)d);
  T2P_REQUIRE(L.ctx_k && L.ctx_vt && ctx_B_ == B, "set_context must be called with the same batch before score");
  const bool tl = res_lowp();
  POOL_GET(t, float*, (size_t)rows * C * (tl ? es : 4));
  const bool qkv_flash = g_qkv_fused && L.a1_qkv.w && g_flash_attention && attention_flash_eligible(dt, d, 3 * C, 3 * C, 3 * C, C);
  char* qkv_pre = nullptr;
  const bool mega = tl && x.lowp && qkv_flash && g_st_tail && g_st_ffpo && g_ffpo_merged && L.fm_ffpo && L.fm_ff1 && rows >= g_st_tail_rows && n % 64 == 0 &&
                    g_fuse_geglu && L.a2_out.b && L.ff1.b;
  float* y2 = nullptr;
  float* y2_stats = nullptr;
  if (tl && x.lowp && qkv_flash) {
    StEntryArgs e;
    e.dtype = dt; e.B = B; e.n = n; e.C = C;
    const bool normed = x.pre_norm && x.pre_for == &L.gn0 && x.pre_silu == 0;
    e.x = normed ? x.pre_norm : (const void*)x.p;
    e.cstats = normed ? nullptr : x.cstats;
    e.gn_gamma = L.gn0.gamma; e.gn_beta = L.gn0.beta; e.groups = L.gn0.G; e.gn_eps = 1e-6f;
    e.w_in = L.fm_in; e.b_in = L.proj_in.b;
    e.ln_gamma = L.ln1.gamma; e.ln_beta = L.ln1.beta; e.ln_eps = 1e-5f;
    e.w_qkv = L.fm_qkv; e.n2 = 3 * C;
    void* a_small = nullptr;
    if (!normed && !x.cstats && L.proj_in.b && L.fm_in && g_st_fuse) {
      StEntryArgs probe = e;
      probe.x = x.p; probe.cstats = nullptr;
      if (st_entry_eligible(probe)) {
        T2P_TRY(group_norm(x, nullptr, L.gn0, 1e-6f, 0, 0, B, &a_small, s));
        e.x = a_small; e.cstats = nullptr;
      }
    }
    if ((normed || x.cstats || a_small) && L.proj_in.b && L.fm_in && st_entry_eligible(e)) {
      qkv_pre = (char*)pool_.get((size_t)rows * 3 * C * es);
      if (!qkv_pre) return T2P_ERR_HIP;
      if (mega) {
        y2 = (float*)pool_.get((size_t)rows * C * es);
        if (!y2) return T2P_ERR_HIP;
        if (g_fuse_gn_stats) {
          y2_stats = (float*)pool_.get((size_t)(rows / 64) * C * 2 * 4);
          if (!y2_stats) return T2P_ERR_HIP;
          e.zero = y2_stats; e.zero_n = (long)(rows / 64) * C * 2;
        }
      }
      e.t = t; e.qkv = qkv_pre;
      T2P_TRY(launch_st_entry(e, s));
      if (normed) { pool_.put(x.pre_norm); x.pre_norm = nullptr; }
    }
    pool_.put(a_small);
  }
  if (!qkv_pre) {
    void* a = nullptr;
    T2P_TRY(group_norm(x, nullptr, L.gn0, 1e-6f, 0, 0, B, &a, s));
    T2P_TRY(linear(a, false, L.proj_in, rows, t, !tl, nullptr, 1.f, s));
    pool_.put(a);
  }
  POOL_GET(ln, void*, (size_t)rows * C * es);
  POOL_GET(o, void*, (size_t)rows * C * es);
  if (!qkv_pre) T2P_TRY(launch_layernorm(t, L.ln1.gamma, L.ln1.beta, ln, dt, rows, C, 1e-5f, s, tl));
  if (qkv_flash) {
    char* qkv = qkv_pre;
    if (!qkv) {
      qkv = (char*)pool_.get((size_t)rows * 3 * C * es);
      if (!qkv) return T2P_ERR_HIP;
      T2P_TRY(linear(ln, false, L.a1_qkv, rows, qkv, false, nullptr, 1.f, s, false));
    }
    T2P_TRY(launch_attention_flash(dt, qkv, 3 * C, qkv + (size_t)C * es, 3 * C, qkv + (size_t)2 * C * es, 3 * C, o, B, heads, n, n, d, scale, s,
                                   true));
    pool_.put(qkv);
  } else {
    POOL_GET(qk, char*, (size_t)rows * 2 * C * es);
    T2P_TRY(linear(ln, false, L.a1_qk, rows, qk, false, nullptr, 1.f, s, false));
    POOL_GET(vt, void*, (size_t)B * C * npad * es);
    T2P_TRY(project_vt(dt, L.a1_v, ln, C, B, n, npad, vt, s));
    T2P_TRY(attention(qk, 2 * C, qk + (size_t)C * es, 2 * C, vt, npad, o, B, heads, n, n, d, scale, s));
    pool_.put(qk);
    pool_.put(vt);
  }
  {
    POOL_GET(q, void*, (size_t)rows * C * es);
    StEntryArgs e;
    e.dtype = dt; e.B = B; e.n = n; e.C = C; e.x = o; e.w_in = L.fm_out1; e.b_in = L.a1_out.b; e.res = t;
    e.ln_gamma = L.ln2.gamma; e.ln_beta = L.ln2.beta; e.ln_eps = 1e-5f; e.w_qkv = L.fm_q2; e.n2 = C; e.t = t; e.qkv = q;
    if (tl && qkv_pre && L.a1_out.b && !L.a2_q.b && st_entry_eligible(e)) {
      T2P_TRY(launch_st_entry(e, s));
    } else {
      T2P_TRY(linear(o, false, L.a1_out, rows, t, !tl, t, 1.f, s, true, nullptr, tl));
      T2P_TRY(launch_layernorm(t, L.ln2.gamma, L.ln2.beta, ln, dt, rows, C, 1e-5f, s, tl));
      T2P_TRY(linear(ln, false, L.a2_q, rows, q, false, nullptr, 1.f, s, false));
    }
    T2P_TRY(attention(q, C, L.ctx_k, C, L.ctx_vt, ctx_Tpad_, o, B, heads, n, ctx_T_, d, scale, s));
    pool_.put(q);
  }
  {
    POOL_GET(g, void*, (size_t)rows * 4 * C * es);
    GemmParams p;
    p.dtype = dt; p.A0 = ln; p.a_f32 = dt == DT_F32; p.C0 = C; p.lda0 = C;
    p.Bw = L.ff1.w; p.ldb = C; p.M = (int)rows; p.N = 8 * C; p.bias_n = L.ff1.b;
    p.C = g; p.c_f32 = 0; p.ldc = 4 * C; p.geglu = 1;
    T2P_TRY(attach_ws(p));
    StEntryArgs e;
    e.dtype = dt; e.B = B; e.n = n; e.C = C; e.x = o; e.w_in = L.fm_out2; e.b_in = L.a2_out.b; e.res = t;
    e.ln_gamma = L.ln3.gamma; e.ln_beta = L.ln3.beta; e.ln_eps = 1e-5f; e.w_qkv = L.fm_ff1; e.b2 = L.ff1.b; e.n2 = 8 * C; e.geglu = 1;
    e.t = t; e.qkv = g;
    const bool tail_chain = tl && qkv_pre && g_st_tail && (y2 || rows >= 2 * g_st_tail_rows) && L.fm_ff1 && g_fuse_geglu && gemm_fuses_geglu(p) && L.a2_out.b && L.ff1.b && st_entry_eligible(e);
    if (tail_chain && y2) {
      e.w3 = L.fm_ffpo; e.b3 = L.ffpo.b; e.res3 = x.p; e.y = y2; e.y_stats = y2_stats; e.qkv = nullptr;
      T2P_REQUIRE(st_entry_eligible(e), "row chain with the third product");
      T2P_TRY(launch_st_entry(e, s));
      pool_.put(g); pool_.put(o); pool_.put(ln); pool_.put(t);
      *out = Act{y2, C, x.H, x.W, y2_stats, true};
      return T2P_OK;
    }
    if (y2) { pool_.put(y2); pool_.put(y2_stats); y2 = nullptr; y2_stats = nullptr; }
    if (tail_chain) {
      T2P_TRY(launch_st_entry(e, s));
    } else {
      T2P_TRY(linear(o, false, L.a2_out, rows, t, !tl, t, 1.f, s, true, nullptr, tl));
      T2P_TRY(launch_layernorm(t, L.ln3.gamma, L.ln3.beta, ln, dt, rows, C, 1e-5f, s, tl));
    }
    if (tail_chain) {
    } else if (g_fuse_geglu && gemm_fuses_geglu(p)) {
      T2P_TRY(gemm(p, s));
    } else {
      POOL_GET(u, float*, (size_t)rows * 8 * C * 4);
      T2P_TRY(linear(ln, false, L.ff1, rows, u, true, nullptr, 1.f, s));
      T2P_TRY(launch_geglu(u, g, dt, rows, 4 * C, s, 1));
      pool_.put(u);
    }
    if (g_ffpo_merged && tl && L.ffpo.w) {
      pool_.put(o);
      const bool olp2 = res_lowp();
      POOL_GET(y2, float*, (size_t)rows * C * (olp2 ? es : 4));
      float* y2_stats = nullptr;
      GemmParams q;
      q.dtype = dt; q.a_f32 = 0; q.A0 = g; q.C0 = 4 * C; q.lda0 = 4 * C; q.A1 = t; q.C1 = C; q.lda1 = C;
      q.Bw = L.ffpo.w; q.ldb = L.ffpo.K; q.M = (int)rows; q.N = C; q.bias_n = L.ffpo.b;
      q.R = x.p; q.ldr = C; q.r_lowp = x.lowp ? 1 : 0;
      q.C = y2; q.c_f32 = olp2 ? 0 : 1; q.ldc = C; q.rows_per_batch = n;
      T2P_TRY(gemm_stats(q, &y2_stats, s));
      pool_.put(g);
      pool_.put(ln);
      pool_.put(t);
      *out = Act{y2, C, x.H, x.W, y2_stats, olp2};
      return T2P_OK;
    }
    T2P_TRY(linear(g, false, L.ff2, rows, t, !tl, t, 1.f, s, true, nullptr, tl));
    pool_.put(g);
  }
  pool_.put(o);
  const bool olp = res_lowp();
  POOL_GET(y, float*, (size_t)rows * C * (olp ? es : 4));
  float* y_stats = nullptr;
  if (tl) {
    T2P_TRY(linear(t, false, L.proj_out, rows, y, !olp, x.p, 1.f, s, true, &y_stats, x.lowp));
  } else if (dt != DT_F32 && g_raw_copies) {
    T2P_TRY(launch_convert(t, ln, dt, rows * C, s));
    T2P_TRY(linear(ln, false, L.proj_out, rows, y, !olp, x.p, 1.f, s, true, &y_stats, x.lowp));
  } else {
    T2P_TRY(linear(t, true, L.proj_out, rows, y, !olp, x.p, 1.f, s, true, &y_stats, x.lowp));
  }
  pool_.put(ln);
  pool_.put(t);
  *out = Act{y, C, x.H, x.W, y_stats, olp};
  return T2P_OK;
}

static NormHint first_norm_of(const Layer* l, bool concat_input) {
  NormHint h;
  if (!l || concat_input || l->down) return h;
  h.norm = &l->gn0;
  h.silu = l->kind == 0 ? 1 : 0;
  return h;
}

int Engine::run_stage(Stage& st, Act& h, const Act* skip, int B, hipStream_t s, const Layer* next_after) {
  Act cur = h;
  bool own = false;
  for (size_t i = 0; i < st.layers.size(); ++i) {
    Layer& L = st.layers[i];
    Act nxt;
    LayerScope scope(L.prefix + (L.kind == 0 ? (L.up ? ",res_up," : L.down ? ",res_down," : ",res,") : L.kind == 1 ? ",attn," : ",st,") +
                     std::to_string(cur.H) + "," + std::to_string(L.in_ch) + "," + std::to_string(L.out_ch), s);
    const Layer* nextL = i + 1 < st.layers.size() ? &st.layers[i + 1] : next_after;
    if (L.kind == 0) T2P_TRY(res_block(L, cur, i == 0 ? skip : nullptr, &nxt, B, s, res_lowp() ? first_norm_of(nextL, false) : NormHint()));
    else if (L.kind == 1) T2P_TRY(attn_block(L, cur, &nxt, B, s));
    else T2P_TRY(st_block(L, cur, &nxt, B, s));
    if (g_tap_index >= 0 && g_tap_counter++ == g_tap_index) {
      const long n = (long)B * nxt.H * nxt.W * nxt.C;
      g_tap_shape[0] = nxt.C; g_tap_shape[1] = nxt.H; g_tap_shape[2] = nxt.W; g_tap_shape[3] = nxt.lowp;
      float* dst = g_tap_dst;
      const long cap = g_tap_cap;
      g_tap_index = -1; g_tap_dst = nullptr; g_tap_cap = 0;
      T2P_REQUIRE(dst && n <= cap, "tap buffer too small");
      T2P_TRY(launch_widen(nxt.p, nxt.lowp ? dtype() : DT_F32, dst, n, s));
    }
    drop_pre_norm(cur);
    if (own) free_act(cur);
    cur = nxt;
    own = true;
  }
  h = cur;
  return T2P_OK;
}

int Engine::set_context(const float* ctx, int B, int T, hipStream_t s) {
  T2P_REQUIRE(finalized_, "finalize the engine first");
  T2P_REQUIRE(ctx && B > 0 && T > 0, "set_context arguments");
  const int dt = dtype(), D = cfg_.context_dim;
  const size_t es = dtype_size(dt);
  const long Tpad = (long)round_up((size_t)T, 8);
  const bool realloc = (B != ctx_B_ || T != ctx_T_);
  const void* cx = ctx;
  void* conv = nullptr;
  PoolLease lease(pool_);
  if (dt != DT_F32) {
    conv = pool_.get((size_t)B * T * D * es);
    if (!conv) return T2P_ERR_HIP;
    T2P_TRY(launch_convert(ctx, conv, dt, (long)B * T * D, s));
    cx = conv;
  }
  auto each = [&](Layer& l) -> int {
    if (l.kind != 2) return T2P_OK;
    const int C = l.in_ch;
    if (realloc || !l.ctx_k) {
      pool_.put(l.ctx_k);
      pool_.put(l.ctx_vt);
      l.ctx_k = pool_.get((size_t)B * T * C * es);
      l.ctx_vt = pool_.get((size_t)B * C * Tpad * es);
      pool_.keep(l.ctx_k);
      pool_.keep(l.ctx_vt);
      if (!l.ctx_k || !l.ctx_vt) return T2P_ERR_HIP;
    }
    T2P_TRY(linear(cx, false, l.a2_k, (long)B * T, l.ctx_k, false, nullptr, 1.f, s, false));
    T2P_TRY(project_vt(dt, l.a2_v, cx, D, B, T, Tpad, l.ctx_vt, s));
    return T2P_OK;
  };
  for (Stage& st : arch_.input_stages) for (Layer& l : st.layers) T2P_TRY(each(l));
  for (Layer& l : arch_.mid_stage.layers) T2P_TRY(each(l));
  for (Stage& st : arch_.out_stages) for (Layer& l : st.layers) T2P_TRY(each(l));
  pool_.put(conv);
  ctx_B_ = B; ctx_T_ = T; ctx_Tpad_ = (int)Tpad;
// ... 118 lines not shown
```

text2protein_amd/csrc/engine.h:

```cpp
#pragma once
#include <map>
#include <memory>
#include <string>
#include <unordered_map>
#include <unordered_set>
#include <vector>

#include "../../include/t2p.h"
#include "t2p_kernels.h"

namespace t2p {

class DevPool {
 public:
  ~DevPool();
  void* get(size_t bytes);
  void put(void* p);
  size_t held_bytes() const { return held_; }
  void* persistent(size_t bytes);
  void lease_begin();
  int lease_end();
  void keep(void* p) { leased_.erase(p); }
  int last_reclaimed() const { return last_reclaimed_; }
 private:
  std::multimap<size_t, void*> free_;
  std::unordered_map<void*, size_t> size_of_;
  std::vector<void*> all_;
  std::unordered_set<void*> leased_;
  int lease_depth_ = 0, last_reclaimed_ = 0;
  size_t held_ = 0;
};
struct PoolLease {
  explicit PoolLease(DevPool& p) : pool(p) { pool.lease_begin(); }
  ~PoolLease() { pool.lease_end(); }
  PoolLease(const PoolLease&) = delete;
  PoolLease& operator=(const PoolLease&) = delete;
  DevPool& pool;
};

struct HostTensor {
  std::vector<float> data;
  std::vector<int64_t> shape;
};

struct ParamInfo {
  std::string name;
  std::vector<int64_t> shape;
};

struct DevLinear {
  void* w = nullptr;
  float* b = nullptr;
  int N = 0, K = 0;
};
struct DevNorm {
  float* gamma = nullptr;
  float* beta = nullptr;
  int C = 0, G = 0;
};

struct Layer {
  int kind = 0;
  std::string prefix;
  int in_ch = 0, out_ch = 0, up = 0, down = 0;
  DevNorm gn0, gn1;
  DevLinear conv0, conv1, conv2;
  void* conv0_up4 = nullptr;
  DevLinear conv1x;
  void* fm_conv0 = nullptr; void* fm_conv1 = nullptr;
  bool has_conv2 = false;
  int temb_off = 0;
  DevLinear qk, v, out;
  DevLinear v3;
  void* fm_qk = nullptr; void* fm_v3 = nullptr;
  DevLinear a1_qkv;
  DevLinear proj_in, proj_out, a1_qk, a1_v, a1_out, a2_q, a2_k, a2_v, a2_out, ff1, ff2;
  DevLinear ffpo;
  void* fm_in = nullptr; void* fm_qkv = nullptr; void* fm_out1 = nullptr; void* fm_q2 = nullptr; void* fm_out2 = nullptr; void* fm_ff1 = nullptr; void* fm_ffpo = nullptr;
  DevNorm ln1, ln2, ln3;
  void* ctx_k = nullptr;
  void* ctx_vt = nullptr;
};

struct Stage {
  std::vector<Layer> layers;
  int skip_ch = 0;
};

struct NetArch {
  std::vector<Stage> input_stages, out_stages;
  Stage mid_stage;
  std::vector<ParamInfo> params;
  int nf = 0, temb_dim = 0, temb_total = 0, final_ch = 0;
  int build(const t2p_model_config& c);
};

struct Act {
  float* p = nullptr;
  int C = 0, H = 0, W = 0;
  float* cstats = nullptr;
  bool lowp = false;
  mutable void* pre_norm = nullptr;
  const DevNorm* pre_for = nullptr;
  int pre_silu = 0;
};
struct NormHint {
  const DevNorm* norm = nullptr;
  int silu = 0;
};

class Engine {
 public:
  explicit Engine(const t2p_model_config& cfg);
  ~Engine();
  int build();
  const std::vector<ParamInfo>& params() const { return arch_.params; }
  int load_param(const char* name, const float* data, const int64_t* shape, int ndim);
  int finalize();
  bool finalized() const { return finalized_; }
  int set_context(const float* ctx, int B, int T, hipStream_t s);
  int score(const float* x, const int* labels, const int* step_counter, float* out, int B, hipStream_t s,
            const float* labels_f = nullptr, const int* label_table = nullptr, const float* label_f_table = nullptr);
  int64_t device_bytes() const { return (int64_t)pool_.held_bytes(); }
  int pool_reclaimed() const { return pool_.last_reclaimed(); }
  const t2p_model_config& cfg() const { return cfg_; }
  DevPool& pool() { return pool_; }
  int dtype() const { return cfg_.compute_dtype; }

 private:
  int upload_linear(const std::string& wname, const std::string& bname, int N, int K, DevLinear* out,
                    bool conv3x3 = false, bool nin = false, int force_dtype = -1);
  int upload_stack2(const std::string& w0, const std::string& b0, const std::string& w1, const std::string& b1,
                    int N, int K, bool nin, bool has_bias, DevLinear* out);
  int upload_norm(const std::string& prefix, int C, int G, DevNorm* out);
  int upload_f32(const std::vector<float>& v, float** out);
  const HostTensor* host(const std::string& name, std::vector<int64_t> shape);

  int run_stage(Stage& st, Act& h, const Act* skip, int B, hipStream_t s, const Layer* next_after = nullptr);
  int res_block(Layer& L, const Act& x, const Act* skip, Act* out, int B, hipStream_t s, NormHint hint = NormHint());
  int attn_block(Layer& L, const Act& x, Act* out, int B, hipStream_t s);
  int st_block(Layer& L, const Act& x, Act* out, int B, hipStream_t s);
  int group_norm(const Act& x, const Act* x1, const DevNorm& n, float eps, int silu, int down, int B, void** out,
                 hipStream_t s, void** raw_out = nullptr);
  int gemm(GemmParams& p, hipStream_t s);
  int attach_ws(GemmParams& p);
  int gemm_stats(GemmParams& p, float** cstats, hipStream_t s);
  void free_act(Act& a) { pool_.put(a.p); pool_.put(a.cstats); pool_.put(a.pre_norm); a.p = nullptr; a.cstats = nullptr; a.pre_norm = nullptr; }
  void drop_pre_norm(const Act& a) { pool_.put(a.pre_norm); a.pre_norm = nullptr; }
  int attention(const void* q, long ldq, const void* k, long ldk, const void* vt, long ldvt, void* out, int B,
                int heads, int nq, int nk, int d, float scale, hipStream_t s);
  int linear(const void* a, bool a_is_f32, const DevLinear& w, long rows, void* c, bool c_f32, const float* residual,
             float alpha, hipStream_t s, bool use_bias = true, float** cstats = nullptr, bool r_lowp = false);
  bool res_lowp() const { return g_lowp_residual && cfg_.compute_dtype == DT_F16; }

  t2p_model_config cfg_;
  NetArch arch_;
  std::unordered_map<std::string, HostTensor> host_;
  bool finalized_ = false;
  DevPool pool_;

  int cpad_ = 8;
  DevLinear pre0_, pre1_, pre_conv_, head_conv_, dense_all_;
  DevNorm head_norm_;
  float* pre_conv_direct_ = nullptr;
  void* pre_conv_split_ = nullptr;
  float* inv_sigma_ = nullptr;
  float* unit_scale_ = nullptr;
  int ctx_B_ = 0, ctx_T_ = 0, ctx_Tpad_ = 0;
  void* splitk_ws_ = nullptr;
  size_t splitk_ws_bytes_ = 0;
  const float* tb_ = nullptr;
  long tb_ld_ = 0;
};

}

struct t2p_engine { t2p::Engine impl; explicit t2p_engine(const t2p_model_config& c) : impl(c) {} };
```

text2protein_amd/csrc/gemm.hip:

```cpp
#include <algorithm>
#include <array>
#include <cstdio>
#include <cstring>
#include <map>
#include <string>
#include <type_traits>
#include <vector>

#include "t2p_common.h"

namespace t2p {

typedef float f32x16 __attribute__((ext_vector_type(16)));
typedef __bf16 bf16x8_t __attribute__((ext_vector_type(8)));
typedef _Float16 f16x8_t __attribute__((ext_vector_type(8)));

[[maybe_unused]] static constexpr int ROWB = 144;

template <typename TC> struct VecInfo { static constexpr int VEC = 16 / (int)sizeof(TC); };

template <typename TC> __device__ inline uint4 pack16(const float* f);
template <> __device__ inline uint4 pack16<float>(const float* f) {
  uint4 r;
  r.x = __builtin_bit_cast(uint32_t, f[0]); r.y = __builtin_bit_cast(uint32_t, f[1]);
// ... 2195 lines not shown
      return launch_dma_geom<TC, MODE, 256, 256, 2, 4, 2>(p, stream);
    case 2: return launch_dma_geom<TC, MODE, 128, 128, 2, 2, 2>(p, stream);
    case 4: return launch_dma_geom<TC, MODE, 128, 128, 2, 2, 4>(p, stream);
    case 3:
      if (g_dma_ring == 2) return launch_dma_geom<TC, MODE, 512, 128, 4, 2, 2, 2, true>(p, stream);
      return launch_dma_geom<TC, MODE, 512, 128, 4, 2, 2>(p, stream);
    default: return launch_dma_geom<TC, MODE, 256, 128, 4, 2, 3>(p, stream);
  }
}

#endif

#if T2P_PART_HOST
template <typename TC>
static int launch_dma(const GemmParams& p, hipStream_t stream) {
  if (p.taps == 9) return p.a_up ? launch_dma_mode<TC, 2>(p, stream) : launch_dma_mode<TC, 1>(p, stream);
  return launch_dma_mode<TC, 0>(p, stream);
}

template <typename TC, bool AF32>
static int launch_tile(const GemmParams& p, hipStream_t stream) {
  const long tiles128 = (long)((p.M + 127) / 128) * ((p.N + 127) / 128) * p.nz0 * p.nz1;
  if (p.N <= 64 || p.M <= 64 || tiles128 < 128) return launch_t<TC, AF32, 64, 64>(p, stream);
  return launch_t<TC, AF32, 128, 128>(p, stream);
}

struct ThinConvArgs {
  const void* x; const void* w; const float* bias; const float* row_scale; float* out;
  int B, H, W, Cin, Cout;
  long ldw;
  const float* gn_stats; const float* gn_gamma; const float* gn_beta;
  int gn_groups, gn_silu;
};

template <typename TC, int CH>
__global__ __launch_bounds__(512) void thin_conv_kernel(const ThinConvArgs a) {
  constexpr int TH = 8, TW = 16, WP = TW + 2, NPIX = (TH + 2) * WP;
  constexpr int cb = CH * 2, nchunk = CH / 8;
  constexpr int wrow = 9 * cb + 16;
  constexpr int sw = (nchunk < 8 ? nchunk : 8) - 1;
  extern __shared__ __attribute__((aligned(16))) unsigned char smem[];
  __shared__ float nsc[256], nsh[256];
  unsigned char* halo = smem;
  unsigned char* wl = smem + NPIX * cb;
  const int tid = threadIdx.x;
  const int tiles_x = (a.W + TW - 1) / TW, tiles_y = (a.H + TH - 1) / TH;
  const int tx = blockIdx.x % tiles_x, ty = (blockIdx.x / tiles_x) % tiles_y, b = blockIdx.x / (tiles_x * tiles_y);
  const bool norm = a.gn_stats != nullptr;
  if (norm) {
    if (tid < a.Cin) {
      const int g = tid / (a.Cin / a.gn_groups);
      const float mean = a.gn_stats[2 * (b * a.gn_groups + g)], rstd = a.gn_stats[2 * (b * a.gn_groups + g) + 1];
      const float sc = rstd * a.gn_gamma[tid];
      nsc[tid] = sc;
      nsh[tid] = a.gn_beta[tid] - mean * sc;
    }
    __syncthreads();
  }
  const int x0 = tx * TW, y0 = ty * TH;
  const TC* xb = (const TC*)a.x + (long)b * a.H * a.W * a.Cin;
  const int wave = tid >> 6, lane = tid & 63, r = lane & 15, g = lane >> 4;
  const bool colv = r < a.Cout;
  f32x4_t acc = {0.f, 0.f, 0.f, 0.f};
  for (int c0 = 0; c0 < a.Cin; c0 += CH) {
    if (c0) __syncthreads();
    for (int i = tid; i < NPIX * nchunk; i += 512) {
      const int P = i / nchunk, j = i - P * nchunk;
      const int gy = y0 + P / WP - 1, gx = x0 + P % WP - 1;
      u32x4_t v = {0u, 0u, 0u, 0u};
      if (gy >= 0 && gy < a.H && gx >= 0 && gx < a.W) {
        v = *(const u32x4_t*)(xb + ((long)gy * a.W + gx) * a.Cin + c0 + j * 8);
        if (norm) {
          union { u32x4_t u; TC e[8]; } in, o;
          in.u = v;
#pragma unroll
          for (int e = 0; e < 8; ++e) {
            const int c = c0 + j * 8 + e;
            float y = to_f32(in.e[e]) * nsc[c] + nsh[c];
            if (a.gn_silu) y = y * __builtin_amdgcn_rcpf(1.f + __builtin_amdgcn_exp2f(y * -1.44269504088896341f));
            o.e[e] = from_f32<TC>(y);
          }
          v = o.u;
        }
      }
      *(u32x4_t*)(halo + P * cb + (((j & ~sw) | ((j ^ P) & sw)) << 4)) = v;
    }
    for (int i = tid; i < a.Cout * 9 * nchunk; i += 512) {
      const int co = i / (9 * nchunk), k = i - co * 9 * nchunk, tap = k / nchunk, j = k - tap * nchunk;
      *(u32x4_t*)(wl + co * wrow + k * 16) = *(const u32x4_t*)((const TC*)a.w + (long)co * a.ldw + (long)tap * a.Cin + c0 + j * 8);
    }
    __syncthreads();
#pragma unroll
    for (int tap = 0; tap < 9; ++tap) {
      const int dy = tap / 3, dx = tap % 3;
      const int P = (wave + dy) * WP + r + dx;
      u32x4_t af[CH / 32], bf[CH / 32];
#pragma unroll
      for (int kc = 0; kc < CH / 32; ++kc) {
        const int j = kc * 4 + g;
        af[kc] = *(const u32x4_t*)(halo + P * cb + (((j & ~sw) | ((j ^ P) & sw)) << 4));
        bf[kc] = (u32x4_t){0u, 0u, 0u, 0u};
        if (colv) bf[kc] = *(const u32x4_t*)(wl + r * wrow + (tap * nchunk + j) * 16);
      }
#pragma unroll
      for (int kc = 0; kc < CH / 32; ++kc) Mma16<TC>::run(af[kc], bf[kc], acc);
    }
  }
  if (!colv) return;
  const int y = y0 + wave;
  if (y >= a.H) return;
  const float bias = a.bias ? a.bias[r] : 0.f, sc = a.row_scale ? a.row_scale[b] : 1.f;
  float* o = a.out + (((long)b * a.Cout + r) * a.H + y) * a.W;
#pragma unroll
  for (int v = 0; v < 4; ++v) {
    const int x = x0 + g * 4 + v;
    if (x < a.W) o[x] = (acc[v] + bias) * sc;
  }
}

static bool g_thin_conv = true;
static bool g_a_norm = true;
void set_gemm_thin_conv(bool on) { g_thin_conv = on; }
void set_gemm_a_norm(bool on) { g_a_norm = on; }

static bool thin_conv_eligible(const GemmParams& p) {
  if (p.dtype == DT_F32 || p.a_f32 || p.taps != 9 || p.a_up || !p.c_nchw || !p.c_f32) return false;
  if (p.A1 || p.R || p.bias_m || p.bias_bn || p.nz0 * p.nz1 != 1 || p.alpha != 1.f || p.geglu) return false;
  if (p.N > 8 || (p.C0 != 32 && p.C0 != 64 && p.C0 != 128 && p.C0 != 256) || p.lda0 != p.C0) return false;
  return p.rows_per_batch == p.H * p.W && p.M % (p.H * p.W) == 0;
}

bool gemm_applies_a_norm(const GemmParams& p) { return g_thin_conv && g_a_norm && thin_conv_eligible(p) && p.C0 <= 256; }

template <typename TC, int CH>
static int launch_thin_conv_ch(const ThinConvArgs& a, hipStream_t stream) {
  constexpr int smem = 180 * CH * 2 + 8 * (9 * CH * 2 + 16);
  const int tiles = ((a.W + 15) / 16) * ((a.H + 7) / 8);
  hipLaunchKernelGGL((thin_conv_kernel<TC, CH>), dim3((unsigned)((long)a.B * tiles)), dim3(512), smem, stream, a);
  T2P_HIP_CHECK(hipGetLastError());
  return T2P_OK;
}

template <typename TC>
static int launch_thin_conv(const GemmParams& p, hipStream_t stream) {
  ThinConvArgs a;
  a.x = p.A0; a.w = p.Bw; a.bias = p.bias_n; a.row_scale = p.row_scale; a.out = (float*)p.C;
  a.B = p.M / (p.H * p.W); a.H = p.H; a.W = p.W; a.Cin = p.C0; a.Cout = p.N; a.ldw = p.ldb;
  a.gn_stats = p.an_stats; a.gn_gamma = p.an_gamma; a.gn_beta = p.an_beta; a.gn_groups = p.an_groups; a.gn_silu = p.an_silu;
  if (p.C0 == 32) return launch_thin_conv_ch<TC, 32>(a, stream);
  if (p.C0 == 64) return launch_thin_conv_ch<TC, 64>(a, stream);
  return launch_thin_conv_ch<TC, 128>(a, stream);
}

int launch_gemm(const GemmParams& p, hipStream_t stream) {
  const int vec = p.dtype == DT_F32 ? 4 : 8;
  const int Ctot = p.C0 + p.C1;
  T2P_REQUIRE(p.A0 && p.Bw && (p.C || p.gn_out), "null operand");
  if (p.gn_out) {
    GemmParams q = p;
    q.gn_out = nullptr; q.gn_gamma = q.gn_beta = nullptr;
    T2P_REQUIRE(p.gn_gamma && p.gn_beta && gemm_fuses_post_gn(q, p.gn_groups), "a following GroupNorm rides only on the split-K second pass (ask gemm_fuses_post_gn)");
  }
  T2P_REQUIRE(p.M > 0 && p.N > 0 && Ctot > 0, "empty problem");
  T2P_REQUIRE(p.taps == 1 || p.taps == 9, "taps must be 1 or 9");
  T2P_REQUIRE(p.dtype != DT_F32 || p.a_f32, "fp32 compute takes fp32 sources");
  T2P_REQUIRE(!p.r_lowp || (p.R && p.dtype != DT_F32), "a 16-bit residual needs a 16-bit compute dtype");
  T2P_REQUIRE(p.lda0 % vec == 0 && p.ldb % vec == 0, "row strides must be multiples of the 16-byte vector");
  T2P_REQUIRE(p.lda0 >= ((p.C0 + vec - 1) / vec) * vec, "lda0 too small");
  T2P_REQUIRE(p.ldb >= (long)(p.taps - 1) * Ctot + ((Ctot + vec - 1) / vec) * vec, "ldb too small");
  if (p.A1) {
    T2P_REQUIRE(p.C0 % vec == 0 && p.lda1 % vec == 0 && p.C1 % vec == 0, "concat sources must be vector aligned");
    T2P_REQUIRE(p.nz0 * p.nz1 == 1, "batched GEMM takes a single A source");
  } else {
    T2P_REQUIRE(p.C1 == 0, "C1 without A1");
  }
  if (p.taps == 9) T2P_REQUIRE(Ctot % vec == 0, "3x3 convolution needs channels % vector == 0");
  if (p.taps == 9 || p.a_up || p.r_up || p.c_nchw) {
    T2P_REQUIRE(p.H > 0 && p.W > 0 && p.M % (p.H * p.W) == 0, "spatial mode needs H, W with M = batch*H*W");
    T2P_REQUIRE(p.nz0 * p.nz1 == 1, "spatial modes are not batched");
  }
  if (p.a_up || p.r_up) T2P_REQUIRE(p.H % 2 == 0 && p.W % 2 == 0, "up-sampling needs even H, W");
  if (p.r_up || p.c_nchw) T2P_REQUIRE(p.rows_per_batch == p.H * p.W, "rows_per_batch must be H*W");
  T2P_REQUIRE(p.rows_per_batch > 0, "rows_per_batch");
  T2P_REQUIRE(!p.c_nchw || (p.row_scale && p.c_f32), "nchw store needs row_scale and fp32 output");
  T2P_REQUIRE(((uintptr_t)p.A0 % 16) == 0 && ((uintptr_t)p.Bw % 16) == 0 && ((uintptr_t)p.A1 % 16) == 0,
              "operands must be 16-byte aligned");
  T2P_REQUIRE((long)(p.M + 127) / 128 < 65536, "M too large for grid.y");
  if (p.X0 || p.X1 || p.CX0 || p.CX1) {
    GemmParams q = p;
    q.X0 = q.X1 = nullptr; q.CX0 = q.CX1 = 0;
    T2P_REQUIRE(p.X0 && p.CX0 > 0 && p.CX0 % 64 == 0 && p.CX1 % 64 == 0 && (p.X1 != nullptr) == (p.CX1 > 0), "shortcut segment: whole 64-channel K-tiles");
    T2P_REQUIRE(gemm_can_fuse_shortcut(q), "shortcut segment: only on the LDS-DMA 3x3 convolution (ask gemm_can_fuse_shortcut)");
    T2P_REQUIRE(((uintptr_t)p.X0 % 16) == 0 && ((uintptr_t)p.X1 % 16) == 0 && p.ldx0 % 8 == 0 && p.ldx1 % 8 == 0, "shortcut segment: 16-byte aligned rows");
    T2P_REQUIRE(((long)p.M + 512) * std::max(p.ldx0, p.ldx1) * 2 < (1L << 31) - 64 && std::max(p.ldx0, p.ldx1) * 2 < (1L << 24), "shortcut segment: 32-bit offsets");
    T2P_REQUIRE(p.ldb >= 9L * (p.C0 + p.C1) + p.CX0 + p.CX1, "shortcut segment: weight rows hold 9 (C0 + C1) + CX0 + CX1 columns");
  }
  if (p.an_stats) {
    GemmParams q = p;
    q.an_stats = nullptr;
    T2P_REQUIRE(p.an_gamma && p.an_beta && p.an_groups > 0 && p.C0 % p.an_groups == 0 && gemm_applies_a_norm(q),
                "a GroupNorm of the A operand rides only on the thin-output head convolution (ask gemm_applies_a_norm)");
  }
  if (g_thin_conv && thin_conv_eligible(p)) {
    ProfRec rec;
    if (g_prof_on) {
      T2P_HIP_CHECK(hipEventCreate(&rec.a));
      T2P_HIP_CHECK(hipEventCreate(&rec.b));
      prof_shape(rec, p);
    prof_shape(rec, p);
      rec.flops = 2.0 * p.M * p.N * 9.0 * p.C0; rec.kind = 2; rec.name = nullptr; rec.bytes = 0;
      T2P_HIP_CHECK(hipEventRecord(rec.a, stream));
    }
    const int rc = p.dtype == DT_BF16 ? launch_thin_conv<bf16_t>(p, stream) : launch_thin_conv<f16_t>(p, stream);
    if (g_prof_on) {
      T2P_HIP_CHECK(hipEventRecord(rec.b, stream));
      g_prof.push_back(rec);
    }
    return rc;
  }
  if (dma_eligible(p)) return p.dtype == DT_BF16 ? launch_dma<bf16_t>(p, stream) : launch_dma<f16_t>(p, stream);
  switch (p.dtype) {
    case DT_F32: return launch_tile<float, true>(p, stream);
    case DT_BF16: return p.a_f32 ? launch_tile<bf16_t, true>(p, stream) : launch_tile<bf16_t, false>(p, stream);
    case DT_F16: return p.a_f32 ? launch_tile<f16_t, true>(p, stream) : launch_tile<f16_t, false>(p, stream);
  }
  set_last_error("launch_gemm: unknown dtype");
  return T2P_ERR_INVALID;
}

#endif

#if T2P_GEMM_PART == -1 || T2P_GEMM_PART == 1
template int launch_dma_mode<f16_t, 0>(const GemmParams&, hipStream_t);
#endif
#if T2P_GEMM_PART == -1 || T2P_GEMM_PART == 2
template int launch_dma_mode<f16_t, 1>(const GemmParams&, hipStream_t);
#endif
#if T2P_GEMM_PART == -1 || T2P_GEMM_PART == 3
template int launch_dma_mode<f16_t, 2>(const GemmParams&, hipStream_t);
#endif
#if T2P_GEMM_PART == -1 || T2P_GEMM_PART == 4
template int launch_dma_mode<bf16_t, 0>(const GemmParams&, hipStream_t);
#endif
#if T2P_GEMM_PART == -1 || T2P_GEMM_PART == 5
template int launch_dma_mode<bf16_t, 1>(const GemmParams&, hipStream_t);
#endif
#if T2P_GEMM_PART == -1 || T2P_GEMM_PART == 6
template int launch_dma_mode<bf16_t, 2>(const GemmParams&, hipStream_t);
#endif

}
```

text2protein_amd/csrc/t2p_common.h:

```cpp
#pragma once
#include <hip/hip_runtime.h>
#include <stdint.h>
#include <string>

namespace t2p {

enum DType : int { DT_F32 = 0, DT_BF16 = 1, DT_F16 = 2 };

inline size_t dtype_size(int dt) { return dt == DT_F32 ? 4 : 2; }

struct bf16_t { uint16_t v; };
struct f16_t { _Float16 v; };

template <typename T> struct dtype_of;
template <> struct dtype_of<float> { static constexpr int value = DT_F32; };
template <> struct dtype_of<bf16_t> { static constexpr int value = DT_BF16; };
template <> struct dtype_of<f16_t> { static constexpr int value = DT_F16; };

__host__ __device__ inline uint16_t f32_to_bf16_bits(float f) {
#if defined(__HIP_DEVICE_COMPILE__)
  return __builtin_bit_cast(uint16_t, (__bf16)f);
#endif
  uint32_t u = __builtin_bit_cast(uint32_t, f);
  if ((u & 0x7fffffffu) > 0x7f800000u) return (uint16_t)((u >> 16) | 0x40);
  u += 0x7fffu + ((u >> 16) & 1u);
  return (uint16_t)(u >> 16);
}
__host__ __device__ inline float bf16_bits_to_f32(uint16_t b) {
  uint32_t u = ((uint32_t)b) << 16;
  return __builtin_bit_cast(float, u);
}

template <typename T> __host__ __device__ inline T from_f32(float f);
template <> __host__ __device__ inline float from_f32<float>(float f) { return f; }
template <> __host__ __device__ inline bf16_t from_f32<bf16_t>(float f) { return bf16_t{f32_to_bf16_bits(f)}; }
template <> __host__ __device__ inline f16_t from_f32<f16_t>(float f) { return f16_t{(_Float16)f}; }

__host__ __device__ inline float to_f32(float f) { return f; }
__host__ __device__ inline float to_f32(bf16_t b) { return bf16_bits_to_f32(b.v); }
__host__ __device__ inline float to_f32(f16_t h) { return (float)h.v; }

void set_last_error(const std::string& msg);
const char* get_last_error();

#define T2P_OK 0
#define T2P_ERR_INVALID 1
#define T2P_ERR_HIP 2
#define T2P_ERR_STATE 3

#define T2P_HIP_CHECK(expr)                                                                   \
  do {                                                                                        \
    hipError_t _e = (expr);                                                                   \
    if (_e != hipSuccess) {                                                                   \
      ::t2p::set_last_error(std::string(#expr) + ": " + hipGetErrorString(_e) + " at " +      \
                            __FILE__ + ":" + std::to_string(__LINE__));                       \
      return T2P_ERR_HIP;                                                                     \
    }                                                                                         \
  } while (0)

#define T2P_REQUIRE(cond, msg)                                                                \
  do {                                                                                        \
    if (!(cond)) {                                                                            \
      ::t2p::set_last_error(std::string("requirement failed: ") + #cond + " -- " + (msg) +    \
                            " at " + __FILE__ + ":" + std::to_string(__LINE__));              \
      return T2P_ERR_INVALID;                                                                 \
    }                                                                                         \
  } while (0)

#define T2P_TRY(expr)                                                                         \
  do {                                                                                        \
    int _rc = (expr);                                                                         \
    if (_rc != T2P_OK) return _rc;                                                            \
  } while (0)

int ensure_dynamic_lds(const void* kernel, int bytes);

struct GemmParams {
  const void* A0 = nullptr;
  const void* A1 = nullptr;
  int a_f32 = 0;
  int C0 = 0, C1 = 0;
  long lda0 = 0, lda1 = 0;
  int taps = 1;
  int H = 0, W = 0;
  int a_up = 0;
  const void* Bw = nullptr;
  long ldb = 0;
  const void* Bw4 = nullptr;
  long ldb4 = 0;
  int up_phase = 0;
  const void* X0 = nullptr;
  const void* X1 = nullptr;
  int CX0 = 0, CX1 = 0;
  long ldx0 = 0, ldx1 = 0;
  int M = 0, N = 0;
  int nz0 = 1, nz1 = 1;
  long sA_z0 = 0, sA_z1 = 0, sB_z0 = 0, sB_z1 = 0, sC_z0 = 0, sC_z1 = 0, sR_z0 = 0, sR_z1 = 0;
  const float* bias_n = nullptr;
  const float* bias_m = nullptr;
  const float* bias_bn = nullptr;
  int rows_per_batch = 1;
  long ld_bn = 0;
  const float* R = nullptr;
  int r_lowp = 0;
  long ldr = 0;
  int r_up = 0;
  float alpha = 1.f;
  void* C = nullptr;
  int c_f32 = 1;
  long ldc = 0;
  int c_nchw = 0;
  const float* row_scale = nullptr;
  int dtype = DT_F32;
  int geglu = 0;
  float* col_stats = nullptr;
  void* ws = nullptr;
  size_t ws_bytes = 0;
  const float* gn_gamma = nullptr;
  const float* gn_beta = nullptr;
  int gn_groups = 0, gn_silu = 0;
  float gn_eps = 1e-6f;
  void* gn_out = nullptr;
  const float* an_stats = nullptr;
  const float* an_gamma = nullptr;
  const float* an_beta = nullptr;
  int an_groups = 0, an_silu = 0;
  void* c_frag = nullptr;
  int frag_col0 = 0, frag_ns = 0;
  long frag_bstride = 0;
};
bool gemm_writes_frag_major(const GemmParams& p);

int launch_gemm(const GemmParams& p, hipStream_t stream);
bool gemm_fuses_col_stats(const GemmParams& p);
bool gemm_can_fuse_shortcut(const GemmParams& p);
bool gemm_fuses_geglu(const GemmParams& p);
bool gemm_fuses_col_stats_lowp(const GemmParams& p);
bool gemm_fuses_post_gn(const GemmParams& p, int groups);
void set_gemm_post_gn(bool on);
bool gemm_applies_a_norm(const GemmParams& p);
void set_gemm_split_consts(int tiles, int target);
void set_gemm_dma(bool on);
void set_gemm_debug(int v);
void set_gemm_geom(int v);
void set_gemm_ring(int v);
void set_gemm_splitk(bool on);
void set_gemm_force_nsplit(int v);
void set_gemm_midsplit(bool on);
void set_gemm_thin_conv(bool on);
void set_gemm_a_norm(bool on);
void set_gemm_up4(bool on);
void set_gemm_deep_ring(bool on);
void set_gemm_fuse_shortcut(bool on);
void set_gemm_dxs(bool on);
#ifdef T2P_ABLATION
int dxs_stamps_read(unsigned long long* out, int n);
#endif
extern bool g_qkv_fused;
extern bool g_attn_merged, g_ffpo_merged;
extern bool g_flash_attention;
extern bool g_lowp_h1;
extern bool g_lowp_residual;
extern bool g_layernorm16;
extern bool g_gn_apply16;
extern bool g_gn_small;
extern bool g_fuse_geglu;
extern bool g_fuse_gn_stats;
extern bool g_raw_copies;
void profile_begin();
int profile_end(double out[3][3]);
int profile_dominant(double out[4], const char** name);
int profile_shapes(char* buf, int len);
bool prof_on();
void prof_attention(hipEvent_t a, hipEvent_t b, double flops);
int profile_attention(double out[3]);

}
```

Baseline: 0.6483 samples/s.

## Add K-split GEMM kernel for small products with optional fused A-side LayerNorm

Adds a new 64x64-tile GEMM kernel that splits K (512 or 1024) across four waves, each running MFMA 16x16x32 on its K slice, then reduces the partials through LDS before the bias/residual epilogue. Small GEMMs whose tile count fits a threshold are routed to it through linear, the attention projections and the value transpose, with the aim of filling more of the GPU than the existing tiled GEMM does on low-tile-count shapes. An optional path folds the LayerNorm of the A rows into the kernel for K=512, removing a separate layernorm launch and its round trip through memory. That path is off by default. The cost is an extra LDS reduction and a second GEMM code path with strict eligibility rules.

```diff
diff --git a/include/t2p.h b/include/t2p.h
--- a/include/t2p.h
+++ b/include/t2p.h
@@ -182,6 +182,12 @@
                 void* stream);
 int t2p_op_gemm_r16(int dtype, const void* A, int a_f32, const void* Bw, void* C, int c_f32, int M, int N, int K, int64_t lda,
                     int64_t ldb, int64_t ldc, const float* bias_n, const void* residual16, float alpha, void* stream);
+int t2p_op_gemm_ksplit(int dtype, const void* A, int a_f32, const void* Bw, void* C, int c_f32, int M, int N, int K, int64_t lda,
+                       int64_t ldb, int64_t ldc, const float* bias_n, const void* residual, int r_lowp, float alpha, int geglu, int nz,
+                       int64_t sA, int64_t sB, int64_t sC, void* stream);
+int t2p_op_gemm_ksplit_ln(int dtype, const void* A, const float* ln_gamma, const float* ln_beta, float ln_eps, const void* Bw, void* C,
+                          int c_f32, int M, int N, int K, int64_t lda, int64_t ldb, int64_t ldc, const float* bias_n, const void* residual,
+                          int r_lowp, float alpha, void* stream);
 int t2p_op_conv3x3(int dtype, const void* x, int a_f32, const void* w, const float* bias, float* out, int batch,
                    int H, int W, int Cin, int Cout, int upsample, void* stream);
 int t2p_op_conv3x3_shortcut(int dtype, const void* a, const void* w, const float* bias, const void* x0, int CX0,
diff --git a/text2protein_amd/_lib.py b/text2protein_amd/_lib.py
--- a/text2protein_amd/_lib.py
+++ b/text2protein_amd/_lib.py
@@ -108,6 +108,8 @@
                              _i, _i, _i, _vp]),
     "t2p_op_input_conv": (_i, [_vp, _vp, _vp, _vp, _i, _i, _i, _i, _i, _i, _vp, _vp]),
     "t2p_op_gemm_r16": (_i, [_i, _vp, _i, _vp, _vp, _i, _i, _i, _i, _i64, _i64, _i64, _vp, _vp, _f, _vp]),
+    "t2p_op_gemm_ksplit": (_i, [_i, _vp, _i, _vp, _vp, _i, _i, _i, _i, _i64, _i64, _i64, _vp, _vp, _i, _f, _i, _i, _i64, _i64, _i64, _vp]),
+    "t2p_op_gemm_ksplit_ln": (_i, [_i, _vp, _vp, _vp, _f, _vp, _vp, _i, _i, _i, _i, _i64, _i64, _i64, _vp, _vp, _i, _f, _vp]),
     "t2p_op_conv3x3": (_i, [_i, _vp, _i, _vp, _vp, _vp, _i, _i, _i, _i, _i, _i, _vp]),
     "t2p_op_groupnorm": (_i, [_vp, _vp, _i, _i, _i, _i, _i, _i, _vp, _vp, _f, _i, _i, _vp, _i, _vp]),
     "t2p_op_layernorm": (_i, [_vp, _vp, _vp, _vp, _i, _i64, _i, _f, _vp]),
diff --git a/text2protein_amd/build.py b/text2protein_amd/build.py
--- a/text2protein_amd/build.py
+++ b/text2protein_amd/build.py
@@ -9,8 +9,9 @@
 CSRC = os.path.join(os.path.dirname(os.path.abspath(__file__)), "csrc")
 LIB = os.path.join(CSRC, "libt2p_hip.so")
 LIB_ABLATION = os.path.join(CSRC, "libt2p_hip_ablation.so")
-SOURCES = ["gemm.hip", "kernels.hip", "attention.hip", "smallconv.hip", "stfuse.hip", "ddim.hip", "engine.cpp", "sampler.cpp", "capi.cpp",
+SOURCES = ["gemm.hip", "gemm_ksplit.hip", "kernels.hip", "attention.hip", "smallconv.hip", "stfuse.hip", "ddim.hip", "engine.cpp", "sampler.cpp", "capi.cpp",
            "train_kernels.hip", "train.cpp", "train_capi.cpp"]
+SCRATCH_CHECKED = ("gemm.hip", "gemm_ksplit.hip")
 GEMM_PARTS = 7
 HEADERS = ["t2p_common.h", "t2p_kernels.h", "philox.h", "engine.h", "sampler.h", "ddim.h", "train_kernels.h", "train.h", os.path.join("..", "..", "include", "t2p.h")]
 ARCH = "gfx950"
@@ -127,6 +128,8 @@
         cmd = [hipcc, *flags, "-x", "hip", "-c", os.path.join(CSRC, src), "-o", obj]
         if part is not None:
             cmd[1:1] = ["-Rpass-analysis=kernel-resource-usage", f"-DT2P_GEMM_PART={part}"]
+        elif src in SCRATCH_CHECKED:
+            cmd[1:1] = ["-Rpass-analysis=kernel-resource-usage"]
         uh = unit_hash(src, cmd[1:-4])
         if os.path.exists(obj) and _read(obj + ".hash") == uh:
             continue
@@ -140,10 +143,10 @@
         out, _ = p.communicate()
         if p.returncode != 0:
             raise RuntimeError(f"hipcc failed on {src}:\n{out}")
-        if src == "gemm.hip":
+        if src in SCRATCH_CHECKED:
             bad = scratch_users(out)
             if bad:
-                raise RuntimeError("LDS-DMA GEMM kernels spill to scratch memory (accumulator loop left rolled?): "
+                raise RuntimeError(f"{src}: GEMM kernels spill to scratch memory (accumulator loop left rolled?): "
                                    + ", ".join(f"{n} {b} B/lane" for n, b in bad[:4]))
             keep, skip = [], 0
             for l in out.splitlines():
diff --git a/text2protein_amd/csrc/capi.cpp b/text2protein_amd/csrc/capi.cpp
--- a/text2protein_amd/csrc/capi.cpp
+++ b/text2protein_amd/csrc/capi.cpp
@@ -308,6 +308,37 @@
   p.bias_n = bias_n; p.R = (const float*)residual16; p.r_lowp = 1; p.ldr = ldc; p.alpha = alpha; p.C = C; p.c_f32 = c_f32; p.ldc = ldc;
   T2P_TRY(attach_op_ws(p));
   return launch_gemm(p, (hipStream_t)stream);
+  API_END
+}
+
+static int op_gemm_ksplit(int dtype, const void* A, int a_f32, const void* Bw, void* C, int c_f32, int M, int N, int K, int64_t lda, int64_t ldb,
+                          int64_t ldc, const float* bias_n, const void* residual, int r_lowp, float alpha, int geglu, int nz, int64_t sA, int64_t sB,
+                          int64_t sC, const float* ln_gamma, const float* ln_beta, float ln_eps, void* stream) {
+  GemmParams p;
+  p.dtype = dtype; p.A0 = A; p.a_f32 = a_f32; p.C0 = K; p.lda0 = lda; p.Bw = Bw; p.ldb = ldb; p.M = M; p.N = N;
+  p.bias_n = bias_n; p.R = (const float*)residual; p.r_lowp = (residual && r_lowp) ? 1 : 0; p.ldr = ldc; p.alpha = alpha;
+  p.C = C; p.c_f32 = c_f32; p.ldc = ldc; p.geglu = geglu;
+  p.nz0 = nz; p.sA_z0 = sA; p.sB_z0 = sB; p.sC_z0 = sC; p.sR_z0 = sC;
+  p.aln_gamma = ln_gamma; p.aln_beta = ln_beta; p.aln_eps = ln_eps;
+  return launch_gemm_ksplit(p, (hipStream_t)stream);
+}
+
+int t2p_op_gemm_ksplit(int dtype, const void* A, int a_f32, const void* Bw, void* C, int c_f32, int M, int N, int K, int64_t lda,
+                       int64_t ldb, int64_t ldc, const float* bias_n, const void* residual, int r_lowp, float alpha, int geglu, int nz,
+                       int64_t sA, int64_t sB, int64_t sC, void* stream) {
+  API_BEGIN
+  return op_gemm_ksplit(dtype, A, a_f32, Bw, C, c_f32, M, N, K, lda, ldb, ldc, bias_n, residual, r_lowp, alpha, geglu, nz, sA, sB, sC, nullptr,
+                        nullptr, 1e-5f, stream);
+  API_END
+}
+
+int t2p_op_gemm_ksplit_ln(int dtype, const void* A, const float* ln_gamma, const float* ln_beta, float ln_eps, const void* Bw, void* C, int c_f32,
+                          int M, int N, int K, int64_t lda, int64_t ldb, int64_t ldc, const float* bias_n, const void* residual, int r_lowp,
+                          float alpha, void* stream) {
+  API_BEGIN
+  T2P_REQUIRE(ln_gamma && ln_beta, "t2p_op_gemm_ksplit_ln takes gamma and beta");
+  return op_gemm_ksplit(dtype, A, 0, Bw, C, c_f32, M, N, K, lda, ldb, ldc, bias_n, residual, r_lowp, alpha, 0, 1, 0, 0, 0, ln_gamma, ln_beta,
+                        ln_eps, stream);
   API_END
 }
 
@@ -763,6 +794,9 @@
   if (key == 46) { t2p::g_attn_proj = value != 0; return T2P_OK; }
   if (key == 47) { set_gemm_dxs(value != 0); return T2P_OK; }
   if (key == 48) { t2p::g_train_plumbing16 = value != 0; return T2P_OK; }
+  if (key == 49) { t2p::g_gemm_ksplit = value != 0; return T2P_OK; }
+  if (key == 50) { t2p::g_ksplit_aln = value != 0; return T2P_OK; }
+  if (key == 51) { if (value > 0) t2p::g_ksplit_max_tiles = value; return T2P_OK; }
   if (key == 34) { set_gemm_a_norm(value != 0); return T2P_OK; }
   if (key == 32) { g_attn_merged = value != 0; return T2P_OK; }
   if (key == 33) { g_ffpo_merged = value != 0; return T2P_OK; }
diff --git a/text2protein_amd/csrc/engine.cpp b/text2protein_amd/csrc/engine.cpp
--- a/text2protein_amd/csrc/engine.cpp
+++ b/text2protein_amd/csrc/engine.cpp
@@ -711,6 +711,9 @@
   return launch_gemm(p, s);
 }
 
+bool g_ksplit_aln = false;
+static int gemm_small(const GemmParams& p, hipStream_t s) { return gemm_ksplit_routed(p) ? launch_gemm_ksplit(p, s) : launch_gemm(p, s); }
+
 int Engine::gemm_stats(GemmParams& p, float** cstats, hipStream_t s) {
   *cstats = nullptr;
   T2P_TRY(attach_ws(p));
@@ -723,7 +726,7 @@
 }
 
 int Engine::linear(const void* a, bool a_is_f32, const DevLinear& w, long rows, void* c, bool c_f32,
-                   const float* residual, float alpha, hipStream_t s, bool use_bias, float** cstats, bool r_lowp) {
+                   const float* residual, float alpha, hipStream_t s, bool use_bias, float** cstats, bool r_lowp, const DevNorm* ln) {
   GemmParams p;
   p.dtype = dtype();
   p.A0 = a; p.a_f32 = a_is_f32 || p.dtype == DT_F32; p.C0 = w.K; p.lda0 = w.K;
@@ -733,8 +736,25 @@
   p.R = residual; p.ldr = w.N; p.r_lowp = (residual && r_lowp) ? 1 : 0;
   p.alpha = alpha;
   p.C = c; p.c_f32 = c_f32; p.ldc = w.N;
+  if (ln) {
+    T2P_REQUIRE(!cstats && gemm_applies_a_layernorm(p), "LayerNorm on the A side: only where the K-split kernel takes the product");
+    p.aln_gamma = ln->gamma; p.aln_beta = ln->beta; p.aln_eps = 1e-5f;
+    T2P_REQUIRE(gemm_ksplit_routed(p), "LayerNorm on the A side: ask linear_takes_layernorm first");
+    return launch_gemm_ksplit(p, s);
+  }
   if (cstats) return gemm_stats(p, cstats, s);
-  return gemm(p, s);
+  T2P_TRY(attach_ws(p));
+  return gemm_small(p, s);
+}
+
+bool Engine::linear_takes_layernorm(const DevLinear& w, long rows) const {
+  if (!g_ksplit_aln) return false;
+  GemmParams p;
+  p.dtype = cfg_.compute_dtype;
+  p.A0 = p.Bw = (const void*)(uintptr_t)256; p.C = (void*)(uintptr_t)256;
+  p.a_f32 = p.dtype == DT_F32; p.C0 = w.K; p.lda0 = w.K; p.ldb = w.K; p.M = (int)rows; p.N = w.N; p.c_f32 = 0; p.ldc = w.N;
+  p.aln_gamma = p.aln_beta = (const float*)(uintptr_t)256;
+  return gemm_ksplit_routed(p);
 }
 
 int Engine::group_norm(const Act& x, const Act* x1, const DevNorm& n, float eps, int silu, int down, int B, void** out,
@@ -1068,7 +1088,7 @@
   p.nz0 = B; p.sA_z0 = 0; p.sB_z0 = (long)n * lda;
   p.bias_m = wv.b;
   p.C = vt; p.c_f32 = 0; p.ldc = npad; p.sC_z0 = (long)wv.N * npad;
-  return launch_gemm(p, s);
+  return gemm_small(p, s);
 }
 
 int Engine::attn_block(Layer& L, const Act& x, Act* out, int B, hipStream_t s) {
@@ -1143,7 +1163,7 @@
       pv = tv;
     }
   }
-  T2P_TRY(launch_gemm(pq, s));
+  T2P_TRY(gemm_small(pq, s));
   POOL_GET(vt, void*, (size_t)B * C * npad * es);
   const float att_scale = 1.f / std::sqrt((float)C);
   const float out_alpha = cfg_.skip_rescale ? 0.70710678118654752440f : 1.f;
@@ -1254,13 +1274,15 @@
   }
   POOL_GET(ln, void*, (size_t)rows * C * es);
   POOL_GET(o, void*, (size_t)rows * C * es);
-  if (!qkv_pre) T2P_TRY(launch_layernorm(t, L.ln1.gamma, L.ln1.beta, ln, dt, rows, C, 1e-5f, s, tl));
+  const bool ln1_fused = !qkv_pre && qkv_flash && tl && linear_takes_layernorm(L.a1_qkv, rows);
+  if (!qkv_pre && !ln1_fused) T2P_TRY(launch_layernorm(t, L.ln1.gamma, L.ln1.beta, ln, dt, rows, C, 1e-5f, s, tl));
   if (qkv_flash) {
     char* qkv = qkv_pre;
     if (!qkv) {
       qkv = (char*)pool_.get((size_t)rows * 3 * C * es);
       if (!qkv) return T2P_ERR_HIP;
-      T2P_TRY(linear(ln, false, L.a1_qkv, rows, qkv, false, nullptr, 1.f, s, false));
+      if (ln1_fused) T2P_TRY(linear(t, false, L.a1_qkv, rows, qkv, false, nullptr, 1.f, s, false, nullptr, false, &L.ln1));
+      else T2P_TRY(linear(ln, false, L.a1_qkv, rows, qkv, false, nullptr, 1.f, s, false));
     }
     T2P_TRY(launch_attention_flash(dt, qkv, 3 * C, qkv + (size_t)C * es, 3 * C, qkv + (size_t)2 * C * es, 3 * C, o, B, heads, n, n, d, scale, s,
                                    true));
@@ -1283,8 +1305,12 @@
       T2P_TRY(launch_st_entry(e, s));
     } else {
       T2P_TRY(linear(o, false, L.a1_out, rows, t, !tl, t, 1.f, s, true, nullptr, tl));
-      T2P_TRY(launch_layernorm(t, L.ln2.gamma, L.ln2.beta, ln, dt, rows, C, 1e-5f, s, tl));
-      T2P_TRY(linear(ln, false, L.a2_q, rows, q, false, nullptr, 1.f, s, false));
+      if (tl && linear_takes_layernorm(L.a2_q, rows)) {
+        T2P_TRY(linear(t, false, L.a2_q, rows, q, false, nullptr, 1.f, s, false, nullptr, false, &L.ln2));
+      } else {
+        T2P_TRY(launch_layernorm(t, L.ln2.gamma, L.ln2.beta, ln, dt, rows, C, 1e-5f, s, tl));
+        T2P_TRY(linear(ln, false, L.a2_q, rows, q, false, nullptr, 1.f, s, false));
+      }
     }
     T2P_TRY(attention(q, C, L.ctx_k, C, L.ctx_vt, ctx_Tpad_, o, B, heads, n, ctx_T_, d, scale, s));
     pool_.put(q);
diff --git a/text2protein_amd/csrc/engine.h b/text2protein_amd/csrc/engine.h
--- a/text2protein_amd/csrc/engine.h
+++ b/text2protein_amd/csrc/engine.h
@@ -150,7 +150,8 @@
   int attention(const void* q, long ldq, const void* k, long ldk, const void* vt, long ldvt, void* out, int B,
                 int heads, int nq, int nk, int d, float scale, hipStream_t s);
   int linear(const void* a, bool a_is_f32, const DevLinear& w, long rows, void* c, bool c_f32, const float* residual,
-             float alpha, hipStream_t s, bool use_bias = true, float** cstats = nullptr, bool r_lowp = false);
+             float alpha, hipStream_t s, bool use_bias = true, float** cstats = nullptr, bool r_lowp = false, const DevNorm* ln = nullptr);
+  bool linear_takes_layernorm(const DevLinear& w, long rows) const;
   bool res_lowp() const { return g_lowp_residual && cfg_.compute_dtype == DT_F16; }
 
   t2p_model_config cfg_;
diff --git a/text2protein_amd/csrc/gemm.hip b/text2protein_amd/csrc/gemm.hip
--- a/text2protein_amd/csrc/gemm.hip
+++ b/text2protein_amd/csrc/gemm.hip
@@ -2371,10 +2371,32 @@
   return launch_thin_conv_ch<TC, 128>(a, stream);
 }
 
+int prof_gemm_begin(const GemmParams& p, const char* name, hipStream_t stream, int* slot) {
+  *slot = -1;
+  if (!g_prof_on) return T2P_OK;
+  ProfRec rec;
+  T2P_HIP_CHECK(hipEventCreate(&rec.a));
+  T2P_HIP_CHECK(hipEventCreate(&rec.b));
+  prof_shape(rec, p);
+  const double z = (double)p.nz0 * p.nz1;
+  rec.flops = 2.0 * p.M * p.N * (double)p.C0 * z;
+  rec.kind = 1; rec.name = name;
+  rec.bytes = z * ((double)p.M * p.C0 * 2 + (double)p.N * p.C0 * 2 + (double)p.M * p.N * (p.c_f32 ? 4 : 2) + (p.R ? (double)p.M * p.N * (p.r_lowp ? 2 : 4) : 0.0));
+  T2P_HIP_CHECK(hipEventRecord(rec.a, stream));
+  g_prof.push_back(rec);
+  *slot = (int)g_prof.size() - 1;
+  return T2P_OK;
+}
+int prof_gemm_end(int slot, hipStream_t stream) {
+  if (slot >= 0 && slot < (int)g_prof.size()) T2P_HIP_CHECK(hipEventRecord(g_prof[slot].b, stream));
+  return T2P_OK;
+}
+
 int launch_gemm(const GemmParams& p, hipStream_t stream) {
   const int vec = p.dtype == DT_F32 ? 4 : 8;
   const int Ctot = p.C0 + p.C1;
   T2P_REQUIRE(p.A0 && p.Bw && (p.C || p.gn_out), "null operand");
+  T2P_REQUIRE(!p.aln_gamma && !p.aln_beta, "a LayerNorm of the A operand rides only on launch_gemm_ksplit (ask gemm_applies_a_layernorm)");
   if (p.gn_out) {
     GemmParams q = p;
     q.gn_out = nullptr; q.gn_gamma = q.gn_beta = nullptr;
diff --git a/text2protein_amd/csrc/gemm_ksplit.hip b/text2protein_amd/csrc/gemm_ksplit.hip
--- /dev/null
+++ b/text2protein_amd/csrc/gemm_ksplit.hip
@@ -0,0 +1,265 @@
+#include <hip/hip_runtime.h>
+
+#include <string>
+
+#include "t2p_common.h"
+#include "t2p_kernels.h"
+
+namespace t2p {
+
+namespace {
+
+typedef unsigned ks_u32x4_t __attribute__((ext_vector_type(4)));
+typedef unsigned ks_u32x2_t __attribute__((ext_vector_type(2)));
+typedef float ks_f32x4_t __attribute__((ext_vector_type(4)));
+typedef __bf16 ks_bf16x8_t __attribute__((ext_vector_type(8)));
+typedef _Float16 ks_f16x8_t __attribute__((ext_vector_type(8)));
+
+template <typename TC> struct KsMma;
+template <> struct KsMma<bf16_t> {
+  __device__ static inline void run(const ks_u32x4_t& a, const ks_u32x4_t& b, ks_f32x4_t& c) {
+    c = __builtin_amdgcn_mfma_f32_16x16x32_bf16(__builtin_bit_cast(ks_bf16x8_t, a), __builtin_bit_cast(ks_bf16x8_t, b), c, 0, 0, 0);
+  }
+};
+template <> struct KsMma<f16_t> {
+  __device__ static inline void run(const ks_u32x4_t& a, const ks_u32x4_t& b, ks_f32x4_t& c) {
+    c = __builtin_amdgcn_mfma_f32_16x16x32_f16(__builtin_bit_cast(ks_f16x8_t, a), __builtin_bit_cast(ks_f16x8_t, b), c, 0, 0, 0);
+  }
+};
+
+template <typename TC> __device__ inline float ks_lo(unsigned u) { return to_f32(__builtin_bit_cast(TC, (uint16_t)(u & 0xffffu))); }
+template <typename TC> __device__ inline float ks_hi(unsigned u) { return to_f32(__builtin_bit_cast(TC, (uint16_t)(u >> 16))); }
+template <typename TC> __device__ inline unsigned ks_pack2(float a, float b) {
+  const TC x = from_f32<TC>(a), y = from_f32<TC>(b);
+  return (unsigned)__builtin_bit_cast(uint16_t, x) | ((unsigned)__builtin_bit_cast(uint16_t, y) << 16);
+}
+
+constexpr int KS_NW = 4;
+constexpr int KS_BM = 64, KS_BN = 64;
+
+}
+
+template <typename TC, int KSTEPS, bool ALN>
+__global__ __launch_bounds__(KS_NW * 64) void gemm_ksplit_kernel(const GemmParams p) {
+  constexpr int TM = KS_BM / 16, TN = KS_BN / 16, TT = TM * TN, TQ = TT / KS_NW;
+  constexpr int K = KS_NW * KSTEPS * 32;
+  static_assert(KSTEPS % 2 == 0 && TT % KS_NW == 0, "tile split");
+  extern __shared__ __attribute__((aligned(16))) unsigned char ks_smem[];
+  ks_f32x4_t* part = (ks_f32x4_t*)ks_smem;
+  float* red = (float*)(ks_smem + (size_t)KS_NW * TT * 64 * 16);
+
+  const int lane = threadIdx.x & 63, wave = threadIdx.x >> 6;
+  const int l16 = lane & 15, g = lane >> 4;
+  const int z0 = (int)blockIdx.z / p.nz1, z1 = (int)blockIdx.z % p.nz1;
+  const long m0 = (long)blockIdx.y * KS_BM;
+  const int n0 = (int)blockIdx.x * KS_BN;
+  const int kl = wave * (KSTEPS * 32) + g * 16;
+  const TC* A = (const TC*)p.A0 + z0 * p.sA_z0 + z1 * p.sA_z1 + m0 * p.lda0 + kl;
+  const TC* W = (const TC*)p.Bw + z0 * p.sB_z0 + z1 * p.sB_z1 + (long)n0 * p.ldb + kl;
+
+  ks_u32x4_t af[TM][KSTEPS], wf[TN][KSTEPS];
+#pragma unroll
+  for (int pp = 0; pp < KSTEPS / 2; ++pp) {
+#pragma unroll
+    for (int i = 0; i < TM; ++i) {
+      const TC* ap = A + (long)(i * 16 + l16) * p.lda0 + pp * 64;
+      af[i][2 * pp] = *(const ks_u32x4_t*)ap;
+      af[i][2 * pp + 1] = *(const ks_u32x4_t*)(ap + 8);
+    }
+#pragma unroll
+    for (int j = 0; j < TN; ++j) {
+      const TC* wp = W + (long)(j * 16 + l16) * p.ldb + pp * 64;
+      wf[j][2 * pp] = *(const ks_u32x4_t*)wp;
+      wf[j][2 * pp + 1] = *(const ks_u32x4_t*)(wp + 8);
+    }
+  }
+  __builtin_amdgcn_sched_barrier(0);
+
+  if constexpr (ALN) {
+    float mean[TM], rstd[TM];
+#pragma unroll
+    for (int i = 0; i < TM; ++i) {
+      float s = 0.f;
+#pragma unroll
+      for (int st = 0; st < KSTEPS; ++st) {
+        const ks_u32x4_t u = af[i][st];
+        s += ((ks_lo<TC>(u.x) + ks_hi<TC>(u.x)) + (ks_lo<TC>(u.y) + ks_hi<TC>(u.y))) + ((ks_lo<TC>(u.z) + ks_hi<TC>(u.z)) + (ks_lo<TC>(u.w) + ks_hi<TC>(u.w)));
+      }
+      s += __shfl_xor(s, 16);
+      s += __shfl_xor(s, 32);
+      if (g == 0) red[wave * KS_BM + i * 16 + l16] = s;
+    }
+    __syncthreads();
+#pragma unroll
+    for (int i = 0; i < TM; ++i) {
+      const int r = i * 16 + l16;
+      mean[i] = (((red[r] + red[KS_BM + r]) + red[2 * KS_BM + r]) + red[3 * KS_BM + r]) * (1.f / K);
+    }
+    float* red2 = red + KS_NW * KS_BM;
+#pragma unroll
+    for (int i = 0; i < TM; ++i) {
+      float q = 0.f;
+      const float mu = mean[i];
+#pragma unroll
+      for (int st = 0; st < KSTEPS; ++st) {
+        const ks_u32x4_t u = af[i][st];
+        const float d0 = ks_lo<TC>(u.x) - mu, d1 = ks_hi<TC>(u.x) - mu, d2 = ks_lo<TC>(u.y) - mu, d3 = ks_hi<TC>(u.y) - mu;
+        const float d4 = ks_lo<TC>(u.z) - mu, d5 = ks_hi<TC>(u.z) - mu, d6 = ks_lo<TC>(u.w) - mu, d7 = ks_hi<TC>(u.w) - mu;
+        q += ((d0 * d0 + d1 * d1) + (d2 * d2 + d3 * d3)) + ((d4 * d4 + d5 * d5) + (d6 * d6 + d7 * d7));
+      }
+      q += __shfl_xor(q, 16);
+      q += __shfl_xor(q, 32);
+      if (g == 0) red2[wave * KS_BM + i * 16 + l16] = q;
+    }
+    __syncthreads();
+#pragma unroll
+    for (int i = 0; i < TM; ++i) {
+      const int r = i * 16 + l16;
+      const float var = (((red2[r] + red2[KS_BM + r]) + red2[2 * KS_BM + r]) + red2[3 * KS_BM + r]) * (1.f / K);
+      rstd[i] = 1.f / sqrtf(var + p.aln_eps);
+    }
+#pragma unroll
+    for (int st = 0; st < KSTEPS; ++st) {
+      const int k = kl + (st >> 1) * 64 + (st & 1) * 8;
+      const float4 g0 = *(const float4*)(p.aln_gamma + k), g1 = *(const float4*)(p.aln_gamma + k + 4);
+      const float4 b0 = *(const float4*)(p.aln_beta + k), b1 = *(const float4*)(p.aln_beta + k + 4);
+#pragma unroll
+      for (int i = 0; i < TM; ++i) {
+        const ks_u32x4_t u = af[i][st];
+        const float mu = mean[i], rs = rstd[i];
+        ks_u32x4_t o;
+        o.x = ks_pack2<TC>((ks_lo<TC>(u.x) - mu) * rs * g0.x + b0.x, (ks_hi<TC>(u.x) - mu) * rs * g0.y + b0.y);
+        o.y = ks_pack2<TC>((ks_lo<TC>(u.y) - mu) * rs * g0.z + b0.z, (ks_hi<TC>(u.y) - mu) * rs * g0.w + b0.w);
+        o.z = ks_pack2<TC>((ks_lo<TC>(u.z) - mu) * rs * g1.x + b1.x, (ks_hi<TC>(u.z) - mu) * rs * g1.y + b1.y);
+        o.w = ks_pack2<TC>((ks_lo<TC>(u.w) - mu) * rs * g1.z + b1.z, (ks_hi<TC>(u.w) - mu) * rs * g1.w + b1.w);
+        af[i][st] = o;
+      }
+    }
+  }
+
+  ks_f32x4_t acc[TM][TN];
+#pragma unroll
+  for (int i = 0; i < TM; ++i)
+#pragma unroll
+    for (int j = 0; j < TN; ++j) acc[i][j] = ks_f32x4_t{0.f, 0.f, 0.f, 0.f};
+#pragma unroll
+  for (int s = 0; s < KSTEPS; ++s)
+#pragma unroll
+    for (int i = 0; i < TM; ++i)
+#pragma unroll
+      for (int j = 0; j < TN; ++j) KsMma<TC>::run(wf[j][s], af[i][s], acc[i][j]);
+
+#pragma unroll
+  for (int i = 0; i < TM; ++i)
+#pragma unroll
+    for (int j = 0; j < TN; ++j) part[(wave * TT + i * TN + j) * 64 + lane] = acc[i][j];
+  __syncthreads();
+
+  const long zc = z0 * p.sC_z0 + z1 * p.sC_z1, zr = z0 * p.sR_z0 + z1 * p.sR_z1;
+#pragma unroll
+  for (int q = 0; q < TQ; ++q) {
+    const int t = wave * TQ + q, i = t / TN, j = t % TN;
+    ks_f32x4_t v = part[t * 64 + lane];
+#pragma unroll
+    for (int w = 1; w < KS_NW; ++w) v += part[(w * TT + t) * 64 + lane];
+    const long m = m0 + i * 16 + l16;
+    const int n = n0 + j * 16 + g * 4;
+    if (p.bias_n) {
+      const float4 b = *(const float4*)(p.bias_n + n);
+      v.x += b.x; v.y += b.y; v.z += b.z; v.w += b.w;
+    }
+    if (p.R) {
+      if (p.r_lowp) {
+        const ks_u32x2_t r = *(const ks_u32x2_t*)((const TC*)p.R + zr + m * p.ldr + n);
+        v.x += ks_lo<TC>(r.x); v.y += ks_hi<TC>(r.x); v.z += ks_lo<TC>(r.y); v.w += ks_hi<TC>(r.y);
+      } else {
+        const float4 r = *(const float4*)(p.R + zr + m * p.ldr + n);
+        v.x += r.x; v.y += r.y; v.z += r.z; v.w += r.w;
+      }
+    }
+    v *= p.alpha;
+    if (p.c_f32) {
+      *(float4*)((float*)p.C + zc + m * p.ldc + n) = make_float4(v.x, v.y, v.z, v.w);
+    } else {
+      ks_u32x2_t o;
+      o.x = ks_pack2<TC>(v.x, v.y);
+      o.y = ks_pack2<TC>(v.z, v.w);
+      *(ks_u32x2_t*)((TC*)p.C + zc + m * p.ldc + n) = o;
+    }
+  }
+}
+
+namespace {
+
+template <typename TC, int KSTEPS, bool ALN>
+int launch_ksplit_t(const GemmParams& p, hipStream_t stream) {
+  constexpr int smem = KS_NW * (KS_BM / 16) * (KS_BN / 16) * 64 * 16 + 2 * KS_NW * KS_BM * 4;
+  void (*kern)(const GemmParams) = gemm_ksplit_kernel<TC, KSTEPS, ALN>;
+  T2P_TRY(ensure_dynamic_lds((const void*)kern, smem));
+  const dim3 grid((unsigned)(p.N / KS_BN), (unsigned)(p.M / KS_BM), (unsigned)(p.nz0 * p.nz1));
+  static const std::string kname = std::string("gemm_ksplit_kernel<") + (dtype_of<TC>::value == DT_F16 ? "f16_t" : "bf16_t") + ", " +
+                                   std::to_string(KSTEPS) + ", " + (ALN ? "true" : "false") + ">";
+  int slot = -1;
+  T2P_TRY(prof_gemm_begin(p, kname.c_str(), stream, &slot));
+  hipLaunchKernelGGL(kern, grid, dim3(KS_NW * 64), smem, stream, p);
+  T2P_TRY(prof_gemm_end(slot, stream));
+  T2P_HIP_CHECK(hipGetLastError());
+  return T2P_OK;
+}
+
+template <typename TC>
+int launch_ksplit_dt(const GemmParams& p, hipStream_t stream) {
+  const bool aln = p.aln_gamma != nullptr;
+  if (p.C0 == 512) return aln ? launch_ksplit_t<TC, 4, true>(p, stream) : launch_ksplit_t<TC, 4, false>(p, stream);
+  return launch_ksplit_t<TC, 8, false>(p, stream);
+}
+
+const char* ksplit_refusal(const GemmParams& p) {
+  if (p.dtype != DT_F16 && p.dtype != DT_BF16) return "the compute dtype must be f16 or bf16";
+  if (p.a_f32) return "A must be stored in the 16-bit compute dtype";
+  if (p.taps != 1 || p.A1 || p.C1 || p.a_up || p.r_up) return "plain products of one A source only";
+  if (p.C0 != 512 && p.C0 != 1024) return "K must be 512 or 1024";
+  if (p.M <= 0 || p.N <= 0 || p.M % KS_BM != 0 || p.N % KS_BN != 0) return "M and N must be multiples of the 64 x 64 tile";
+  if (p.geglu || p.col_stats || p.c_frag || p.c_nchw || p.bias_m || p.bias_bn || p.gn_out || p.X0 || p.X1 || p.CX0 || p.CX1 || p.an_stats ||
+      p.Bw4 || p.row_scale)
+    return "epilogue or operand option the K-split kernel does not have";
+  if (!p.A0 || !p.Bw || !p.C) return "null operand";
+  if (p.nz0 < 1 || p.nz1 < 1 || (long)p.nz0 * p.nz1 > 65535 || p.M / KS_BM > 65535) return "grid too large";
+  if (p.lda0 < p.C0 || p.ldb < p.C0 || p.ldc < p.N || (p.R && p.ldr < p.N)) return "row strides shorter than the rows";
+  if (p.lda0 % 8 || p.ldb % 8 || p.sA_z0 % 8 || p.sA_z1 % 8 || p.sB_z0 % 8 || p.sB_z1 % 8 || (uintptr_t)p.A0 % 16 || (uintptr_t)p.Bw % 16)
+    return "A and W rows must be 16-byte aligned";
+  if (p.ldc % 4 || p.sC_z0 % 4 || p.sC_z1 % 4 || (uintptr_t)p.C % 16) return "C rows must be aligned to four elements";
+  if (p.R && (p.ldr % 4 || p.sR_z0 % 4 || p.sR_z1 % 4 || (uintptr_t)p.R % 16)) return "residual rows must be aligned to four elements";
+  if (p.bias_n && (uintptr_t)p.bias_n % 16) return "bias must be 16-byte aligned";
+  if (p.aln_gamma || p.aln_beta) {
+    if (!p.aln_gamma || !p.aln_beta || (uintptr_t)p.aln_gamma % 16 || (uintptr_t)p.aln_beta % 16) return "LayerNorm needs 16-byte aligned gamma and beta";
+    if (!(p.aln_eps > 0.f)) return "LayerNorm needs eps > 0";
+    if (p.C0 != 512) return "LayerNorm of the A rows at K = 512 only";
+  }
+  return nullptr;
+}
+
+}
+
+bool g_gemm_ksplit = true;
+int g_ksplit_max_tiles = 256;
+
+bool gemm_ksplit_eligible(const GemmParams& p) { return ksplit_refusal(p) == nullptr; }
+bool gemm_applies_a_layernorm(const GemmParams& p) {
+  GemmParams q = p;
+  q.aln_gamma = q.aln_beta = nullptr;
+  return gemm_ksplit_eligible(q);
+}
+bool gemm_ksplit_routed(const GemmParams& p) {
+  return g_gemm_ksplit && (long)(p.M / KS_BM) * (p.N / KS_BN) * p.nz0 * p.nz1 <= g_ksplit_max_tiles && gemm_ksplit_eligible(p);
+}
+
+int launch_gemm_ksplit(const GemmParams& p, hipStream_t stream) {
+  if (const char* why = ksplit_refusal(p)) {
+    set_last_error(std::string("gemm_ksplit: ") + why);
+    return T2P_ERR_INVALID;
+  }
+  return p.dtype == DT_BF16 ? launch_ksplit_dt<bf16_t>(p, stream) : launch_ksplit_dt<f16_t>(p, stream);
+}
+
+}
diff --git a/text2protein_amd/csrc/t2p_common.h b/text2protein_amd/csrc/t2p_common.h
--- a/text2protein_amd/csrc/t2p_common.h
+++ b/text2protein_amd/csrc/t2p_common.h
@@ -80,6 +80,7 @@
   const void* A1 = nullptr;
   int a_f32 = 0;
   int C0 = 0, C1 = 0;
+  int up_phase = 0;
   long lda0 = 0, lda1 = 0;
   int taps = 1;
   int H = 0, W = 0;
@@ -88,7 +89,6 @@
   long ldb = 0;
   const void* Bw4 = nullptr;
   long ldb4 = 0;
-  int up_phase = 0;
   const void* X0 = nullptr;
   const void* X1 = nullptr;
   int CX0 = 0, CX1 = 0;
@@ -100,16 +100,16 @@
   const float* bias_m = nullptr;
   const float* bias_bn = nullptr;
   int rows_per_batch = 1;
+  int r_lowp = 0;
   long ld_bn = 0;
   const float* R = nullptr;
-  int r_lowp = 0;
   long ldr = 0;
   int r_up = 0;
   float alpha = 1.f;
   void* C = nullptr;
   int c_f32 = 1;
+  int c_nchw = 0;
   long ldc = 0;
-  int c_nchw = 0;
   const float* row_scale = nullptr;
   int dtype = DT_F32;
   int geglu = 0;
@@ -120,6 +120,7 @@
   const float* gn_beta = nullptr;
   int gn_groups = 0, gn_silu = 0;
   float gn_eps = 1e-6f;
+  float aln_eps = 1e-5f;
   void* gn_out = nullptr;
   const float* an_stats = nullptr;
   const float* an_gamma = nullptr;
@@ -128,10 +129,21 @@
   void* c_frag = nullptr;
   int frag_col0 = 0, frag_ns = 0;
   long frag_bstride = 0;
+  const float* aln_gamma = nullptr;
+  const float* aln_beta = nullptr;
 };
 bool gemm_writes_frag_major(const GemmParams& p);
 
 int launch_gemm(const GemmParams& p, hipStream_t stream);
+bool gemm_ksplit_eligible(const GemmParams& p);
+bool gemm_ksplit_routed(const GemmParams& p);
+bool gemm_applies_a_layernorm(const GemmParams& p);
+int launch_gemm_ksplit(const GemmParams& p, hipStream_t stream);
+extern bool g_gemm_ksplit;
+extern bool g_ksplit_aln;
+extern int g_ksplit_max_tiles;
+int prof_gemm_begin(const GemmParams& p, const char* name, hipStream_t stream, int* slot);
+int prof_gemm_end(int slot, hipStream_t stream);
 bool gemm_fuses_col_stats(const GemmParams& p);
 bool gemm_can_fuse_shortcut(const GemmParams& p);
 bool gemm_fuses_geglu(const GemmParams& p);
```

After: 0.6509 samples/s (median of 6 runs). No clear change (+0.4%).
